# alanqrwang/keymorph

Hardware: AMD Instinct MI355X
Metric: volume-pairs/sec (fwd+bwd) at 256^3, 512 kp, TPS (higher is better)
Workload: dtype f32

## Files before the change

include/keymorph_hip.h:

```cpp
#ifndef KEYMORPH_HIP_H
#define KEYMORPH_HIP_H
#include <stddef.h>
#include <stdint.h>
#ifdef __cplusplus
extern "C" {
#endif

#define KMH_EINVAL (-22)
#define KMH_ABI_VERSION 1
int kmh_abi_version(void);

int kmh_grid_sample3d_fwd(const float* x, const float* grid, float* out, int N, int C, int D, int H,
                          int W, int Do, int Ho, int Wo, int mode, void* stream);
int kmh_grid_sample3d_bwd_grid(const float* x, const float* grid, const float* gout, float* dgrid,
                               int N, int C, int D, int H, int W, int Do, int Ho, int Wo, void* stream);
int kmh_grid_sample3d_bwd_input(const float* grid, const float* gout, float* dx, int N, int C, int D,
                                int H, int W, int Do, int Ho, int Wo, void* stream);

size_t kmh_reduce_ws_bytes(void);
int kmh_mse_fwd(const float* a, const float* b, long long n, float* out, void* ws, void* stream);
int kmh_mse_bwd(const float* a, const float* b, const float* gscale, long long n, float* da, void* stream);
int kmh_warp_mse_fwd(const float* x, const float* grid, const float* fixed, float* out, float* out_loss,
                     int N, int C, int D, int H, int W, int Do, int Ho, int Wo, void* ws, void* stream);
int kmh_warp_mse_fwd_grad(const float* x, const float* grid, const float* fixed, float* out, float* out_loss,
                          float* dgrid, int N, int C, int D, int H, int W, int Do, int Ho, int Wo, void* ws,
                          void* stream);
int kmh_scale_unless_one(float* a, long long n, const float* g, void* stream);

int kmh_dice_sums(const float* pred, const float* target, int R, long long V, float* sums, void* ws,
                  void* stream);
int kmh_rows_axpby(const float* t, const float* p, const float* ca, const float* cb, int R, long long V,
                   float* out, void* stream);
int kmh_warp_dice_ok(int N, int C, int D, int H, int W);
int kmh_warp_dice_sums(const float* x, const float* grid, const float* fixed, float* sums, int N, int C, int D, int H,
                       int W, int Do, int Ho, int Wo, const unsigned char* lab_x, const unsigned char* lab_fixed,
                       const int* gate, void* ws, void* stream);
int kmh_warp_dice_bwd_grid(const float* x, const float* grid, const float* fixed, const float* ca, const float* cb,
                           float* dgrid, int N, int C, int D, int H, int W, int Do, int Ho, int Wo,
                           const unsigned char* lab_x, const unsigned char* lab_fixed, const int* gate, void* stream);
int kmh_onehot_to_labels(const float* x, int N, int C, long long V, unsigned char* lab, int* ok, void* stream);
int kmh_argmax_onehot(const float* pred, int N, int C, long long V, float* out, void* stream);
int kmh_jacobian_det(const float* disp, long long cstride, long long vstride, int D, int H, int W, float* jd,
                     double* stats, void* ws, void* stream);

int kmh_label_presence(const long long* seg, long long n, int nflags, int* flags, void* stream);
int kmh_one_hot_select(const long long* seg, int N, long long V, const long long* labels, int C, void* out,
                       int out_i64, void* stream);

size_t kmh_hausdorff3d_ws_bytes(int D, int H, int W);
int kmh_hausdorff3d(const void* a, const void* b, int dtype_a, int dtype_b, long long sstride_a, long long sstride_b, int N,
                    int D, int H, int W, double sz, double sy, double sx, void* ws, double* out_sq, void* stream);
size_t kmh_edt3d_sq_ws_bytes(int D, int H, int W);
int kmh_edt3d_sq(const void* a, int dtype, int D, int H, int W, double sz, double sy, double sx, void* ws, double* out,
                 void* stream);
int kmh_label_counts(const void* x, const void* y, int dtype, int N, int C, long long V, unsigned long long* counts,
                     void* stream);

size_t kmh_lc2_ws_bytes(int num_patches, int num_radii);
int kmh_lc2_fwd(const float* us, const float* mr, int N, int S, int P, const int* radii, int R, double alpha, double beta,
                int reduce_mean, void* ws, float* out, void* stream);
int kmh_lc2_bwd(const float* us, const float* mr, const float* gout, int N, int S, int P, const int* radii, int R,
                int reduce_mean, const void* ws, float* dus, float* dmr, void* stream);

int kmh_affine_grid_fwd(const float* mat, float* out, int N, int D, int H, int W, void* stream);
int kmh_affine_grid_bwd(const float* dgrid, float* dmat, int N, int D, int H, int W, void* ws, void* stream);

int kmh_tps_grid_fwd(const float* theta, const float* ctrl, float* out, int N, int T, int D, int H, int W,
                     void* stream);
size_t kmh_tps_grid_bwd_ws_bytes(int N, int T, int D, int H, int W);
int kmh_tps_grid_bwd(const float* dgrid, const float* theta, const float* ctrl, float* dtheta,
                     float* dctrl, int N, int T, int D, int H, int W, void* ws, void* stream);
int kmh_tps_points_fwd(const float* theta, const float* ctrl, const float* pts, float* out, int N, int T,
                       int P, void* stream);
size_t kmh_tps_points_bwd_ws_bytes(int N, int T, int P);
int kmh_tps_points_bwd(const float* dout, const float* theta, const float* ctrl, const float* pts,
                       float* dtheta, float* dctrl, float* dpts, int N, int T, int P, void* ws,
                       void* stream);

size_t kmh_tps_fit_ws_bytes(int N, int T);
int kmh_tps_fit_fwd(const float* ctrl, const float* tgt, const float* lmbda, const float* w, float* theta,
                    int N, int T, void* ws, void* stream);
int kmh_tps_fit_force_retry(int count);
int kmh_tps_fit_bwd(const float* dtheta, const float* theta, const float* ctrl, const float* lmbda, const float* w,
                    float* dctrl, float* dtgt, float* dw, int N, int T, void* ws, void* stream);

int kmh_affine_fit_fwd(const float* x, const float* y, const float* w, float* M, int N, int K, void* stream);
int kmh_affine_fit_bwd(const float* dM, const float* x, const float* y, const float* w, const float* M,
                       float* dx, float* dy, float* dw, int N, int K, void* stream);
int kmh_rigid_fit_fwd(const float* x, const float* y, const float* w, float* M, int N, int K, void* stream);
int kmh_rigid_fit_bwd(const float* dM, const float* x, const float* y, const float* w, float* dx, float* dy,
                      float* dw, int N, int K, void* stream);
int kmh_affine_inverse_fwd(const float* M, float* Minv, int N, void* stream);
int kmh_affine_inverse_bwd(const float* dMinv, const float* Minv, float* dM, int N, void* stream);
int kmh_affine_points_fwd(const float* M, const float* pts, float* out, int N, int P, void* stream);
int kmh_affine_build_matrix(const float* scale, const float* offset, const float* theta, const float* shear,
                            float* out, int B, void* stream);
int kmh_affine_points_bwd(const float* dout, const float* M, const float* pts, float* dM, float* dpts,
                          int N, int P, void* stream);

int kmh_com3d_fwd(const float* feat, float* pts, float* sums, int N, int K, int D, int H, int W, void* ws,
                  void* stream);
int kmh_com3d_bwd(const float* dpts, const float* feat, const float* sums, float* dfeat, int N, int K,
                  int D, int H, int W, void* stream);



int kmh_conv3d_pack_weight(const float* w, float* packed, int Cout, int Cin, int transposed, void* stream);
int kmh_conv3d_fwd(const float* x, const float* scale, const float* shift, const float* mask,
                   const float* packed_w, const float* bias, float* y, int N, int D, int H, int W, int Cin,
                   int Cout, int relu_in, int relu_out, void* stream);
size_t kmh_conv3d_pack_bf_bytes(int Cout, int Cin, int transposed, int terms);
int kmh_conv3d_pack_weight_bf(const float* w, void* packed, int Cout, int Cin, int transposed, int terms,
                              const float* wscale, void* stream);
size_t kmh_conv3d_fwd_bf_stats_ws_bytes(int N, int D, int H, int W, int Cout, int rows_per_wave);
int kmh_conv3d_fwd_bf(const float* x, const float* scale, const float* shift, const float* mask, const void* packed,
                      const float* bias, float* y, int N, int D, int H, int W, int Cin, int Cout, int relu_in,
                      int relu_out, int terms, int rows_per_wave, const float* ascale, const float* wscale,
                      void* stats_ws, double* stats_out, int in_blocked, const float* addend, void* stream);
int kmh_conv3d_fwd_bf_set_dispatch(int mode);
int kmh_conv3d_fwd_bf_split_ok(int N, int D, int H, int W, int Cin, int Cout, int terms);
int kmh_conv3d_fwd_bf_variant(int N, int D, int H, int W, int Cin, int Cout, int terms, int has_mask, int has_addend);
int kmh_conv3d_fwd_bf_pool_ok(int N, int D, int H, int W, int Cin, int Cout, int terms);
int kmh_conv3d_fwd_bf_pool(const float* x, const float* scale, const float* shift, const void* packed, float* yp,
                           unsigned char* arg, int N, int D, int H, int W, int Cin, int Cout, int relu_in, int terms,
                           const float* ascale, const float* wscale, void* stats_ws, double* stats_out, int in_blocked,
                           void* stream);
size_t kmh_conv3d_up2_pack_bytes(int Cout, int Cl, int terms);
int kmh_conv3d_up2_pack_weight(const float* w, void* packed, int Cout, int Ctot, int cofs, int Cl, int terms,
                               const float* wscale, void* stream);
size_t kmh_conv3d_up2_dgrad_pack_bytes(int Cout, int Cl, int terms);
int kmh_conv3d_up2_dgrad_pack_weight(const float* w, void* packed, int Cout, int Ctot, int cofs, int Cl, int terms,
                                     const float* wscale, void* stream);
size_t kmh_conv3d_up2_dgrad_stats_ws_bytes(int N, int Dl, int Hl, int Wl, int Cl);
int kmh_conv3d_up2_dgrad(const float* dz, const void* packed, float* ds, int N, int Dl, int Hl, int Wl, int Cl, int Cout,
                         int terms, const float* dscale, const float* wscale, void* stats_ws, double* stats_out,
                         int in_blocked ,
                         void* stream);
int kmh_up2_boxsum(const float* dz, float* G, int N, int Dl, int Hl, int Wl, int Cout, int in_blocked ,
                   void* stream);
size_t kmh_up2_wgrad_gemm_ws_bytes(int N, int V, int Cl, int J);
int kmh_up2_wgrad_gemm(const float* A, const float* B, float* C, int N, int V, int Cl, int J, int terms,
                       const float* ascale, const float* bscale, const float* a_scale, const float* a_shift, void* ws,
                       void* stream);
int kmh_up2_wgrad_fold_ok(int Cl, int Cout, int terms);
size_t kmh_up2_wgrad_fold_ws_bytes(int N, int Dl, int Hl, int Wl, int Cl, int Cout);
int kmh_up2_wgrad_fold(const float* xl, const float* dz, float* C, int N, int Dl, int Hl, int Wl, int Cl, int Cout, int terms,
                       const float* ascale, const float* dscale, const float* a_scale, const float* a_shift, int dz_blocked,
                       void* ws, void* stream);
int kmh_conv3d_up2_fwd(const float* xl, const float* scale, const float* shift, int Ctot, int cofs, const void* packed,
                       float* y, int N, int Dl, int Hl, int Wl, int Cl, int Cout, int terms, const float* ascale,
                       const float* wscale, void* stream);
size_t kmh_conv3d_wgrad_bf_ws_bytes(int N, int D, int H, int W, int Cin, int Cout, int terms);
int kmh_conv3d_wgrad_bf_blocked_ok(int N, int D, int H, int W, int Cin, int Cout, int terms);
int kmh_conv3d_wgrad_bf(const float* x, const float* scale, const float* shift, const float* dz,
                        const float* dzmask, float* dw, int N, int D, int H, int W, int Cin, int Cout, int relu_in,
                        int accumulate, int terms, int append_ones, const float* xscale, const float* dscale, int dz_blocked, const float* w_fold, double* bhat,
                        void* ws, void* stream);
size_t kmh_conv3d_first_layer_fwd_ws_bytes(int N, int D, int H, int W, int Cout);
int kmh_conv3d_first_layer_fwd(const float* x, const float* scale, const float* shift, const float* w, float* y, int N,
                               int D, int H, int W, int Cout, void* ws, double* stats_out, void* stream);
size_t kmh_conv3d_first_layer_wgrad_ws_bytes(int N, int D, int H, int W, int Cout);
int kmh_conv3d_first_layer_wgrad(const float* x, const float* dz, const float* dzmask, const float* c123, double* rs, int N,
                                 int D, int H, int W, int Cout, void* ws, void* stream);
int kmh_conv3d_first_layer_fold(const void* rs, int rs_f64, const float* w, const float* scale_n, const float* shift_n, int Cout,
                                float* dw, double* ab_n, int accumulate, void* stream);
size_t kmh_conv3d_wgrad_ws_bytes(int N, int D, int H, int W, int Cin, int Cout);
int kmh_conv3d_wgrad(const float* x, const float* scale, const float* shift, const float* dz,
                     const float* dzmask, float* dw, int N, int D, int H, int W, int Cin, int Cout, int relu_in,
                     int accumulate, void* ws, void* stream);

size_t kmh_channel_stats_ws_bytes(int N, int C);
int kmh_channel_stats(const float* a, const float* b, int mode, int N, long long V, int C, double* out, void* ws,
                      const int* only_if, void* stream);
int kmh_gn_fwd_coeffs(const double* stats, const float* gamma, const float* beta, int N, int C, int G, double count,
                      float eps, float* scale, float* shift, float* mean_rstd, float* ascale, void* stream);
int kmh_absmax_scale(const float* x, long long n, float min_abs, float* out2, void* stream);
int kmh_gn_bwd_coeffs(const double* ab, const float* gamma, const float* mean_rstd, int N, int C, int G,
                      double count, float* c123, float* dgamma, float* dbeta, const int* only_if, void* stream);
int kmh_gn_bwd_coeffs_fold(const double* dstats, const double* bhat, const float* gamma, const float* beta,
                           const float* mean_rstd, int N, int C, int G, double count, float* c123, float* dgamma,
                           float* dbeta, int* fallback, void* stream);
int kmh_in_bwd_stats(const float* du, const float* z, const float* scale, const float* shift, int N, long long V, int C,
                     double* out, void* ws, void* stream);
int kmh_in_bwd_apply(const float* du, const float* z, const float* scale, const float* shift, const float* c123, int N,
                     long long V, int C, float* dz, float* dz_scale2, void* stream);
int kmh_in_bwd_apply_pool(const unsigned char* argmax, const float* du, const float* z, const float* scale,
                          const float* shift, const float* c123, int N, int D, int H, int W, int C, float* dz,
                          float* dz_scale2, void* stream);

int kmh_gn_bwd_apply(const float* dxn, const float* x, const float* c123, int N, long long V, int C,
                     int relu_mask, int accumulate, float* dx, float* dx_scale2, int out_blocked, void* stream);
int kmh_relu_mask(const float* dy, const float* y, long long n, float* dz, void* stream);
int kmh_norm_apply(const float* x, const float* scale, const float* shift, int N, long long V, int C, int relu,
                   float* y, void* stream);

int kmh_maxpool3d_fwd(const float* x, float* y, unsigned char* argmax, int N, int D, int H, int W, int C, void* stream);
int kmh_maxpool3d_bwd(const float* x, const unsigned char* argmax, const float* dy, const float* add, int add_cstride,
                      float* dx, int N, int D, int H, int W, int C, int out_blocked, void* stream);
size_t kmh_maxpool3d_bwd_split_bytes(int N, int D, int H, int W, int C);
int kmh_maxpool3d_bwd_split(const unsigned char* argmax, const float* dy, const float* dy_scale2, float* dxs, int N, int D,
                            int H, int W, int C, void* stream);
int kmh_maxpool3d_bwd_lazy(const unsigned char* argmax, const float* dy, const float* dxn, const float* x, const float* c123,
                           float* dx, int N, int D, int H, int W, int C, float* dx_scale2, void* stream);
int kmh_upcat_fwd(const float* skip, const float* low, float* out, int N, int D, int H, int W, int Cs, int Dl,
                  int Hl, int Wl, int Cl, void* stream);
int kmh_upcat_bwd(const float* dout, float* dskip, float* dlow, int N, int D, int H, int W, int Cs, int Dl, int Hl,
                  int Wl, int Cl, int accumulate_skip, void* stream);
int kmh_layout_convert(const float* in, float* out, int N, long long V, int C, int to_ncdhw, void* stream);

int kmh_pointwise_pack(const float* w, float* wt, int Cout, int Cin, void* stream);
int kmh_pointwise_fwd(const float* x, const float* wt, const float* bias, float* y, int N, long long V, int Cin,
                      int Cout, void* stream);
int kmh_pointwise_dgrad(const float* dy, const float* w, float* dx, int N, long long V, int Cin, int Cout,
                        void* stream);
size_t kmh_pointwise_wgrad_ws_bytes(int N, long long V, int Cin, int Cout);
int kmh_pointwise_wgrad(const float* dy, const float* x, float* dw, float* dbias, int N, long long V, int Cin,
                        int Cout, int accumulate, void* ws, void* stream);

size_t kmh_headcom_fwd_ws_bytes(int N, long long V, int Cout);
size_t kmh_headcom_bwd_ws_bytes(int N, long long V, int Cin, int Cout);
int kmh_headcom_fwd(const float* feat, const float* w, const float* bias, float* pts, float* sums, float* sq, int N, int D,
                    int H, int W, int Cin, int Cout, void* ws, void* stream);
int kmh_headcom_bwd(const float* dpts, const float* dpower, const float* feat, const float* w, const float* bias,
                    const float* sums, float* dfeat, float* dw, float* dbias, int N, int D, int H, int W, int Cin,
                    int Cout, int mask_dfeat, void* ws, void* stream);
size_t kmh_headcom_fwd_bf_ws_bytes(int N, long long V, int Cout, int terms);
size_t kmh_headcom_bwd_bf_ws_bytes(int N, long long V, int Cin, int Cout, int terms);
size_t kmh_headcom_mask_words(int N, int D, int H, int W, int Cout);
int kmh_headcom_fwd_bf(const float* feat, const float* w, const float* bias, float* pts, float* sums, float* sq,
                       float* scales_out, int N, int D, int H, int W, int Cin, int Cout, int terms, unsigned* mask, void* ws,
                       void* stream);
int kmh_headcom_bwd_bf(const float* dpts, const float* dpower, const float* feat, const float* w, const float* bias,
                       const float* sums, float* dfeat, float* dw, float* dbias, int N, int D, int H, int W, int Cin,
                       int Cout, int terms, int mask_dfeat, const float* scales_in, float* dfeat_scale2,
                       const unsigned* mask, void* ws, void* stream);

int kmh_adam_step(float* p, const float* g, float* m, float* v, long long n, float lr, float beta1, float beta2,
                  float eps, int step, float grad_scale, void* stream);

int kmh_resize_trilinear3d_fwd(const float* x, float* y, int N, int C, int D, int H, int W, int Do, int Ho, int Wo,
                               const int* tz, const int* ty, const int* tx, int channels_last, void* stream);
int kmh_resize_trilinear3d_bwd(const float* gy, float* gx, int N, int C, int D, int H, int W, int Do, int Ho, int Wo,
                               const int* tz, const int* ty, const int* tx, const int* rz, const int* ry, const int* rx,
                               int channels_last, void* stream);
size_t kmh_components3d_ws_bytes(int N, int D, int H, int W);
int kmh_components3d(const unsigned char* mask, int* labels, int N, int D, int H, int W, int* info, void* ws, void* stream);
int kmh_clean_mask3d(const unsigned char* mask, unsigned char* out, int N, int D, int H, int W, double threshold, int* info,
                     void* ws, void* stream);

int kmh_conv3d_thin_ok(int Cin, int Cout);
int kmh_conv3d_thin_wgrad_ok(int Cin, int Cout);
int kmh_conv3d_thin_fwd(const float* x, const float* w, const float* bias, float* y, int N, int D, int H, int W, int Cin,
                        int Cout, int relu_out, void* stream);
int kmh_conv3d_thin_dgrad(const float* dz, const float* dzmask, const float* w, float* dx, int N, int D, int H, int W, int Cin,
                          int Cout, void* stream);
size_t kmh_conv3d_thin_wgrad_ws_bytes(int N, int D, int H, int W, int Cin, int Cout);
int kmh_conv3d_thin_wgrad(const float* x, const float* dz, const float* dzmask, float* dw, float* db, int N, int D, int H,
                          int W, int Cin, int Cout, void* ws, void* stream);

#ifdef __cplusplus
}
#endif
#endif
```

keymorph_amd/_lib.py:

```python
from __future__ import annotations

import ctypes as C
import os

from .build import LIBPATH

_f = C.c_void_p
_i = C.c_int
_ll = C.c_longlong
_sz = C.c_size_t

PROTOS = {
    "kmh_abi_version": (_i, []),
    "kmh_grid_sample3d_fwd": (_i, [_f, _f, _f, _i, _i, _i, _i, _i, _i, _i, _i, _i, _f]),
    "kmh_grid_sample3d_bwd_grid": (_i, [_f, _f, _f, _f, _i, _i, _i, _i, _i, _i, _i, _i, _f]),
    "kmh_grid_sample3d_bwd_input": (_i, [_f, _f, _f, _i, _i, _i, _i, _i, _i, _i, _i, _f]),
    "kmh_reduce_ws_bytes": (_sz, []),
    "kmh_mse_fwd": (_i, [_f, _f, _ll, _f, _f, _f]),
    "kmh_mse_bwd": (_i, [_f, _f, _f, _ll, _f, _f]),
    "kmh_warp_mse_fwd": (_i, [_f, _f, _f, _f, _f, _i, _i, _i, _i, _i, _i, _i, _i, _f, _f]),
    "kmh_warp_mse_fwd_grad": (_i, [_f, _f, _f, _f, _f, _f, _i, _i, _i, _i, _i, _i, _i, _i, _f, _f]),
    "kmh_scale_unless_one": (_i, [_f, _ll, _f, _f]),
    "kmh_dice_sums": (_i, [_f, _f, _i, _ll, _f, _f, _f]),
    "kmh_rows_axpby": (_i, [_f, _f, _f, _f, _i, _ll, _f, _f]),
    "kmh_warp_dice_ok": (_i, [_i, _i, _i, _i, _i]),
    "kmh_warp_dice_sums": (_i, [_f, _f, _f, _f, _i, _i, _i, _i, _i, _i, _i, _i, _f, _f, _f, _f, _f]),
    "kmh_warp_dice_bwd_grid": (_i, [_f, _f, _f, _f, _f, _f, _i, _i, _i, _i, _i, _i, _i, _i, _f, _f, _f, _f]),
    "kmh_onehot_to_labels": (_i, [_f, _i, _i, _ll, _f, _f, _f]),
    "kmh_argmax_onehot": (_i, [_f, _i, _i, _ll, _f, _f]),
    "kmh_affine_grid_fwd": (_i, [_f, _f, _i, _i, _i, _i, _f]),
    "kmh_affine_grid_bwd": (_i, [_f, _f, _i, _i, _i, _i, _f, _f]),
    "kmh_tps_grid_fwd": (_i, [_f, _f, _f, _i, _i, _i, _i, _i, _f]),
    "kmh_tps_grid_bwd_ws_bytes": (_sz, [_i, _i, _i, _i, _i]),
    "kmh_tps_grid_bwd": (_i, [_f, _f, _f, _f, _f, _i, _i, _i, _i, _i, _f, _f]),
    "kmh_tps_points_fwd": (_i, [_f, _f, _f, _f, _i, _i, _i, _f]),
    "kmh_tps_points_bwd_ws_bytes": (_sz, [_i, _i, _i]),
    "kmh_tps_points_bwd": (_i, [_f, _f, _f, _f, _f, _f, _f, _i, _i, _i, _f, _f]),
    "kmh_tps_fit_ws_bytes": (_sz, [_i, _i]),
    "kmh_tps_fit_fwd": (_i, [_f, _f, _f, _f, _f, _i, _i, _f, _f]),
    "kmh_tps_fit_force_retry": (_i, [_i]),
    "kmh_tps_fit_bwd": (_i, [_f, _f, _f, _f, _f, _f, _f, _f, _i, _i, _f, _f]),
    "kmh_affine_fit_fwd": (_i, [_f, _f, _f, _f, _i, _i, _f]),
    "kmh_affine_fit_bwd": (_i, [_f, _f, _f, _f, _f, _f, _f, _f, _i, _i, _f]),
    "kmh_rigid_fit_fwd": (_i, [_f, _f, _f, _f, _i, _i, _f]),
    "kmh_rigid_fit_bwd": (_i, [_f, _f, _f, _f, _f, _f, _f, _i, _i, _f]),
    "kmh_affine_inverse_fwd": (_i, [_f, _f, _i, _f]),
    "kmh_affine_inverse_bwd": (_i, [_f, _f, _f, _i, _f]),
    "kmh_affine_points_fwd": (_i, [_f, _f, _f, _i, _i, _f]),
    "kmh_jacobian_det": (_i, [_f, _ll, _ll, _i, _i, _i, _f, _f, _f, _f]),
    "kmh_label_presence": (_i, [_f, _ll, _i, _f, _f]),
    "kmh_one_hot_select": (_i, [_f, _i, _ll, _f, _i, _f, _i, _f]),
    "kmh_hausdorff3d_ws_bytes": (_sz, [_i, _i, _i]),
    "kmh_hausdorff3d": (_i, [_f, _f, _i, _i, _ll, _ll, _i, _i, _i, _i, C.c_double, C.c_double, C.c_double, _f, _f, _f]),
    "kmh_edt3d_sq_ws_bytes": (_sz, [_i, _i, _i]),
    "kmh_edt3d_sq": (_i, [_f, _i, _i, _i, _i, C.c_double, C.c_double, C.c_double, _f, _f, _f]),
    "kmh_label_counts": (_i, [_f, _f, _i, _i, _i, _ll, _f, _f]),
    "kmh_lc2_ws_bytes": (_sz, [_i, _i]),
    "kmh_lc2_fwd": (_i, [_f, _f, _i, _i, _i, _f, _i, C.c_double, C.c_double, _i, _f, _f, _f]),
    "kmh_lc2_bwd": (_i, [_f, _f, _f, _i, _i, _i, _f, _i, _i, _f, _f, _f, _f]),
    "kmh_affine_build_matrix": (_i, [_f, _f, _f, _f, _f, _i, _f]),
    "kmh_affine_points_bwd": (_i, [_f, _f, _f, _f, _f, _i, _i, _f]),
    "kmh_com3d_fwd": (_i, [_f, _f, _f, _i, _i, _i, _i, _i, _f, _f]),
    "kmh_com3d_bwd": (_i, [_f, _f, _f, _f, _i, _i, _i, _i, _i, _f]),
    "kmh_conv3d_pack_weight": (_i, [_f, _f, _i, _i, _i, _f]),
    "kmh_conv3d_fwd": (_i, [_f, _f, _f, _f, _f, _f, _f, _i, _i, _i, _i, _i, _i, _i, _i, _f]),
    "kmh_conv3d_pack_bf_bytes": (_sz, [_i, _i, _i, _i]),
    "kmh_conv3d_pack_weight_bf": (_i, [_f, _f, _i, _i, _i, _i, _f, _f]),
    "kmh_conv3d_fwd_bf": (_i, [_f, _f, _f, _f, _f, _f, _f, _i, _i, _i, _i, _i, _i, _i, _i, _i, _i, _f, _f, _f, _f, _i, _f, _f]),
    "kmh_conv3d_fwd_bf_set_dispatch": (_i, [_i]),
    "kmh_conv3d_fwd_bf_variant": (_i, [_i, _i, _i, _i, _i, _i, _i, _i, _i]),
    "kmh_conv3d_fwd_bf_pool_ok": (_i, [_i, _i, _i, _i, _i, _i, _i]),
    "kmh_conv3d_fwd_bf_split_ok": (_i, [_i, _i, _i, _i, _i, _i, _i]),
    "kmh_conv3d_fwd_bf_pool": (_i, [_f, _f, _f, _f, _f, _f, _i, _i, _i, _i, _i, _i, _i, _i, _f, _f, _f, _f, _i, _f]),
    "kmh_conv3d_up2_dgrad_pack_bytes": (_sz, [_i, _i, _i]),
    "kmh_conv3d_up2_dgrad_pack_weight": (_i, [_f, _f, _i, _i, _i, _i, _i, _f, _f]),
    "kmh_conv3d_up2_dgrad_stats_ws_bytes": (_sz, [_i, _i, _i, _i, _i]),
    "kmh_conv3d_up2_dgrad": (_i, [_f, _f, _f, _i, _i, _i, _i, _i, _i, _i, _f, _f, _f, _f, _i, _f]),
    "kmh_up2_boxsum": (_i, [_f, _f, _i, _i, _i, _i, _i, _i, _f]),
    "kmh_up2_wgrad_gemm_ws_bytes": (_sz, [_i, _i, _i, _i]),
    "kmh_up2_wgrad_gemm": (_i, [_f, _f, _f, _i, _i, _i, _i, _i, _f, _f, _f, _f, _f, _f]),
    "kmh_up2_wgrad_fold_ok": (_i, [_i, _i, _i]),
    "kmh_up2_wgrad_fold_ws_bytes": (_sz, [_i, _i, _i, _i, _i, _i]),
    "kmh_up2_wgrad_fold": (_i, [_f, _f, _f, _i, _i, _i, _i, _i, _i, _i, _f, _f, _f, _f, _i, _f, _f]),
    "kmh_conv3d_up2_pack_bytes": (_sz, [_i, _i, _i]),
    "kmh_conv3d_up2_pack_weight": (_i, [_f, _f, _i, _i, _i, _i, _i, _f, _f]),
    "kmh_conv3d_up2_fwd": (_i, [_f, _f, _f, _i, _i, _f, _f, _i, _i, _i, _i, _i, _i, _i, _f, _f, _f]),
    "kmh_conv3d_fwd_bf_stats_ws_bytes": (_sz, [_i, _i, _i, _i, _i, _i]),
    "kmh_conv3d_first_layer_fwd_ws_bytes": (_sz, [_i, _i, _i, _i, _i]),
    "kmh_conv3d_first_layer_fwd": (_i, [_f, _f, _f, _f, _f, _i, _i, _i, _i, _i, _f, _f, _f]),
    "kmh_conv3d_wgrad_bf_ws_bytes": (_sz, [_i, _i, _i, _i, _i, _i, _i]),
    "kmh_conv3d_wgrad_bf": (_i, [_f, _f, _f, _f, _f, _f, _i, _i, _i, _i, _i, _i, _i, _i, _i, _i, _f, _f, _i, _f, _f, _f, _f]),
    "kmh_conv3d_wgrad_bf_blocked_ok": (_i, [_i, _i, _i, _i, _i, _i, _i]),
    "kmh_conv3d_first_layer_wgrad_ws_bytes": (_sz, [_i, _i, _i, _i, _i]),
    "kmh_conv3d_first_layer_wgrad": (_i, [_f, _f, _f, _f, _f, _i, _i, _i, _i, _i, _f, _f]),
    "kmh_conv3d_first_layer_fold": (_i, [_f, _i, _f, _f, _f, _i, _f, _f, _i, _f]),
    "kmh_conv3d_wgrad_ws_bytes": (_sz, [_i, _i, _i, _i, _i, _i]),
    "kmh_conv3d_wgrad": (_i, [_f, _f, _f, _f, _f, _f, _i, _i, _i, _i, _i, _i, _i, _i, _f, _f]),
    "kmh_channel_stats_ws_bytes": (_sz, [_i, _i]),
    "kmh_channel_stats": (_i, [_f, _f, _i, _i, _ll, _i, _f, _f, _f, _f]),
    "kmh_gn_fwd_coeffs": (_i, [_f, _f, _f, _i, _i, _i, C.c_double, C.c_float, _f, _f, _f, _f, _f]),
    "kmh_absmax_scale": (_i, [_f, _ll, C.c_float, _f, _f]),
    "kmh_gn_bwd_coeffs": (_i, [_f, _f, _f, _i, _i, _i, C.c_double, _f, _f, _f, _f, _f]),
    "kmh_gn_bwd_coeffs_fold": (_i, [_f, _f, _f, _f, _f, _i, _i, _i, C.c_double, _f, _f, _f, _f, _f]),
    "kmh_gn_bwd_apply": (_i, [_f, _f, _f, _i, _ll, _i, _i, _i, _f, _f, _i, _f]),
    "kmh_in_bwd_stats": (_i, [_f, _f, _f, _f, _i, _ll, _i, _f, _f, _f]),
    "kmh_in_bwd_apply": (_i, [_f, _f, _f, _f, _f, _i, _ll, _i, _f, _f, _f]),
    "kmh_in_bwd_apply_pool": (_i, [_f, _f, _f, _f, _f, _f, _i, _i, _i, _i, _i, _f, _f, _f]),
    "kmh_relu_mask": (_i, [_f, _f, _ll, _f, _f]),
    "kmh_norm_apply": (_i, [_f, _f, _f, _i, _ll, _i, _i, _f, _f]),
    "kmh_maxpool3d_fwd": (_i, [_f, _f, _f, _i, _i, _i, _i, _i, _f]),
    "kmh_maxpool3d_bwd": (_i, [_f, _f, _f, _f, _i, _f, _i, _i, _i, _i, _i, _i, _f]),
    "kmh_maxpool3d_bwd_split_bytes": (_sz, [_i, _i, _i, _i, _i]),
    "kmh_maxpool3d_bwd_split": (_i, [_f, _f, _f, _f, _i, _i, _i, _i, _i, _f]),
    "kmh_maxpool3d_bwd_lazy": (_i, [_f, _f, _f, _f, _f, _f, _i, _i, _i, _i, _i, _f, _f]),
    "kmh_upcat_fwd": (_i, [_f, _f, _f, _i, _i, _i, _i, _i, _i, _i, _i, _i, _f]),
    "kmh_upcat_bwd": (_i, [_f, _f, _f, _i, _i, _i, _i, _i, _i, _i, _i, _i, _i, _f]),
    "kmh_layout_convert": (_i, [_f, _f, _i, _ll, _i, _i, _f]),
    "kmh_pointwise_pack": (_i, [_f, _f, _i, _i, _f]),
    "kmh_pointwise_fwd": (_i, [_f, _f, _f, _f, _i, _ll, _i, _i, _f]),
    "kmh_pointwise_dgrad": (_i, [_f, _f, _f, _i, _ll, _i, _i, _f]),
    "kmh_pointwise_wgrad_ws_bytes": (_sz, [_i, _ll, _i, _i]),
    "kmh_pointwise_wgrad": (_i, [_f, _f, _f, _f, _i, _ll, _i, _i, _i, _f, _f]),
    "kmh_headcom_fwd_ws_bytes": (_sz, [_i, _ll, _i]),
    "kmh_headcom_bwd_ws_bytes": (_sz, [_i, _ll, _i, _i]),
    "kmh_headcom_fwd_bf_ws_bytes": (_sz, [_i, _ll, _i, _i]),
    "kmh_headcom_bwd_bf_ws_bytes": (_sz, [_i, _ll, _i, _i, _i]),
    "kmh_headcom_mask_words": (_sz, [_i, _i, _i, _i, _i]),
    "kmh_headcom_fwd_bf": (_i, [_f, _f, _f, _f, _f, _f, _f, _i, _i, _i, _i, _i, _i, _i, _f, _f, _f]),
    "kmh_headcom_bwd_bf": (_i, [_f, _f, _f, _f, _f, _f, _f, _f, _f, _i, _i, _i, _i, _i, _i, _i, _i, _f, _f, _f, _f, _f]),
    "kmh_headcom_fwd": (_i, [_f, _f, _f, _f, _f, _f, _i, _i, _i, _i, _i, _i, _f, _f]),
    "kmh_headcom_bwd": (_i, [_f, _f, _f, _f, _f, _f, _f, _f, _f, _i, _i, _i, _i, _i, _i, _i, _f, _f]),
    "kmh_adam_step": (_i, [_f, _f, _f, _f, _ll, C.c_float, C.c_float, C.c_float, C.c_float, _i, C.c_float, _f]),
    "kmh_resize_trilinear3d_fwd": (_i, [_f, _f, _i, _i, _i, _i, _i, _i, _i, _i, _f, _f, _f, _i, _f]),
    "kmh_resize_trilinear3d_bwd": (_i, [_f, _f, _i, _i, _i, _i, _i, _i, _i, _i, _f, _f, _f, _f, _f, _f, _i, _f]),
    "kmh_components3d_ws_bytes": (_sz, [_i, _i, _i, _i]),
    "kmh_components3d": (_i, [_f, _f, _i, _i, _i, _i, _f, _f, _f]),
    "kmh_clean_mask3d": (_i, [_f, _f, _i, _i, _i, _i, C.c_double, _f, _f, _f]),
    "kmh_conv3d_thin_ok": (_i, [_i, _i]),
    "kmh_conv3d_thin_wgrad_ok": (_i, [_i, _i]),
    "kmh_conv3d_thin_fwd": (_i, [_f, _f, _f, _f, _i, _i, _i, _i, _i, _i, _i, _f]),
    "kmh_conv3d_thin_dgrad": (_i, [_f, _f, _f, _f, _i, _i, _i, _i, _i, _i, _f]),
    "kmh_conv3d_thin_wgrad_ws_bytes": (_sz, [_i, _i, _i, _i, _i, _i]),
    "kmh_conv3d_thin_wgrad": (_i, [_f, _f, _f, _f, _f, _i, _i, _i, _i, _i, _i, _f, _f]),
}

_lib = None


class KeymorphHipError(RuntimeError):
    pass


class _Profiler:

    def __init__(self):
        self.enabled = False
        self.records = []
        self.meta = None

    def reset(self):
        self.records = []

    def summary(self):
        import torch
        torch.cuda.synchronize()
        out = {}
        for name, a, b, meta in self.records:
            d = out.setdefault(name, {"calls": 0, "ms": 0.0, "flops": 0.0, "bytes": 0.0})
            d["calls"] += 1
            d["ms"] += a.elapsed_time(b)
            if meta:
                d["flops"] += meta.get("flops", 0.0)
                d["bytes"] += meta.get("bytes", 0.0)
        return out


profiler = _Profiler()


class _Proxy:
    def __init__(self, lib):
        self._lib = lib

    def __getattr__(self, name):
        fn = getattr(self._lib, name)
        if not name.startswith("kmh_") or name.endswith("_bytes") or name == "kmh_abi_version":
            return fn

        def call(*args):
            if not profiler.enabled:
                return fn(*args)
            import torch
            a, b = torch.cuda.Event(enable_timing=True), torch.cuda.Event(enable_timing=True)
            a.record()
            rc = fn(*args)
            b.record()
            profiler.records.append((name, a, b, profiler.meta))
            profiler.meta = None
            return rc

        object.__setattr__(self, name, call)
        return call


_DEFAULT_LIBPATH = LIBPATH


def load():
    global _lib, LIBPATH
    if _lib is not None:
        return _lib
    if os.environ.get("KEYMORPH_HIP_LIB"):
        LIBPATH = os.environ["KEYMORPH_HIP_LIB"]
    if not os.path.exists(LIBPATH):
        raise KeymorphHipError(
            f"{LIBPATH} is missing: the HIP extension has not been built "
            "(run `python -m keymorph_amd.build`); there is no CPU/PyTorch fallback.")
    import torch
    rt = os.path.join(os.path.dirname(torch.__file__), "lib", "libamdhip64.so")
    if os.path.exists(rt):
        C.CDLL(rt, mode=C.RTLD_GLOBAL)
    else:
        C.CDLL("libamdhip64.so", mode=C.RTLD_GLOBAL)
    lib = C.CDLL(LIBPATH)
    ab_build = os.path.abspath(LIBPATH) != os.path.abspath(_DEFAULT_LIBPATH)
    for name, (res, args) in PROTOS.items():
        try:
            fn = getattr(lib, name)
        except AttributeError:
            if not ab_build:
                raise
            continue
        fn.restype = res
        fn.argtypes = args
    if lib.kmh_abi_version() != 1:
        raise KeymorphHipError("libkeymorph_hip.so ABI version mismatch")
    _lib = _Proxy(lib)
    return _lib


def check(rc: int, what: str):
    if rc != 0:
        raise KeymorphHipError(f"{what} failed with status {rc}")
```

keymorph_amd/backbone_ops.py:

```python
from __future__ import annotations

import os
from typing import Optional, Tuple

import torch

from . import _lib
from ._handoff import attach, expect, peek
from ._lib import check
from .ops import _p, _prep, _stream, workspace

Tensor = torch.Tensor
EPS = 1e-5

CONV_MODE = os.environ.get("KEYMORPH_HIP_CONV", "f16x3")
_TERMS = {"f16x3": 2, "bf16x6": 3}
_HEAD_TERMS = {"f16x3": 2, "bf16x6": 3}
BF_ROWS_PER_WAVE = int(os.environ.get("KEYMORPH_HIP_BF_ROWS", "4"))


def set_conv_mode(mode: str):
    global CONV_MODE
    assert mode in ("f32", "f16x3", "bf16x6"), mode
    CONV_MODE = mode


_SWITCHES = {
    "KEYMORPH_NO_EPILOGUE_STATS": "a separate statistics pass per layer instead of the convolution epilogue's",
    "KEYMORPH_NO_UPCONV": "materialise upsample+concat instead of the fused decoder operator, forward",
    "KEYMORPH_NO_UPCONV_BWD": "materialise upsample+concat instead of the fused decoder operator, backward",
    "KEYMORPH_NO_UPCONV_WGRAD": "the fused decoder operator rebuilds the upsampled half for the 27-tap weight gradient",
    "KEYMORPH_NO_UP2_FOLD": "the upsampled channels' weight gradient by the box-sum tensor + matrix product route",
    "KEYMORPH_NO_STATS_FOLD": "GroupNorm's backward statistics by a pass over the tensors",
    "KEYMORPH_NO_BLOCKED_GRADS": "every gradient in (N,D,H,W,C)",
    "KEYMORPH_NO_BLOCKED_UPCAT": "only the fused decoder operator's gradient in (N,D,H,W,C)",
    "KEYMORPH_NO_SPLIT_POOLGRAD": "the 256^3-level pooled gradient scattered as fp32 instead of pre-split records",
    "KEYMORPH_NO_CONV_POOL": "separate pooling pass instead of the conv epilogue's",
    "KEYMORPH_NO_LAZY_FIRST": "GroupNorm backward of the first block as its own pass",
    "KEYMORPH_NO_LAZY_SKIP": "GroupNorm's backward of a decoder skip applied in the decoder",
    "KEYMORPH_NO_LAZY_IN": "ConvNet block by block: separate norm / ReLU / pooling passes",
    "KEYMORPH_RANGE_AUDIT": "debug (ON = audit): per-sample dynamic range of every gradient operand, RANGE_AUDIT_LOG",
}


def _off(name: str) -> bool:
    if name not in _SWITCHES:
        raise KeyError(name)
    return bool(os.environ.get(name))


import contextlib
import functools
import threading

_AMP_DEFAULT = os.environ.get("KEYMORPH_AMP", "0") not in ("", "0")
_amp_tls = threading.local()


def amp_enabled() -> bool:
    return bool(getattr(_amp_tls, "on", _AMP_DEFAULT))


@contextlib.contextmanager
def amp_scope(on: bool):
    prev = amp_enabled()
    _amp_tls.on = bool(on)
    try:
        yield
    finally:
        _amp_tls.on = prev


def set_amp(on: bool) -> bool:
    prev = amp_enabled()
    _amp_tls.on = bool(on)
    return prev


def _t(terms: int) -> int:
    return 1 if (terms == 2 and amp_enabled()) else terms


def _binds_amp(cls):
    fwd, bwd = cls.forward, cls.backward

    @staticmethod
    @functools.wraps(fwd)
    def forward(ctx, *a, **k):
        ctx._kmh_amp = amp_enabled()
        return fwd(ctx, *a, **k)

    @staticmethod
    @functools.wraps(bwd)
    def backward(ctx, *g):
        with amp_scope(ctx._kmh_amp):
            return bwd(ctx, *g)

    cls.forward, cls.backward = forward, backward
    return cls


FIRST_BLOCK_DGRAD = os.environ.get("KEYMORPH_FIRST_BLOCK_DGRAD", "")


def set_first_block_dgrad(mode: str) -> str:
    global FIRST_BLOCK_DGRAD
    assert mode in ("", "bf16x6"), mode
    prev, FIRST_BLOCK_DGRAD = FIRST_BLOCK_DGRAD, mode
    return prev


def first_block_dgrad_terms() -> int:
    return 3 if (FIRST_BLOCK_DGRAD == "bf16x6" and CONV_MODE == "f16x3") else 0


def _f32(shape, dev):
    return torch.empty(shape, dtype=torch.float32, device=dev)


def channel_stats(a: Tensor, b: Optional[Tensor], N: int, V: int, C: int, only_if: Optional[Tensor] = None) -> Tensor:
    lib = _lib.load()
    out = torch.empty((N, C, 2), dtype=torch.float64, device=a.device)
    ws = workspace(int(lib.kmh_channel_stats_ws_bytes(N, C)), a.device, "stats")
    check(lib.kmh_channel_stats(_p(a), _p(b), 0 if b is None else 1, N, V, C, _p(out), _p(ws), _p(only_if), _stream()),
          "kmh_channel_stats")
    return out


def _needs_range_scales() -> bool:
    return _TERMS.get(CONV_MODE, 0) == 2


_CONSTS = {}


def _const(device, *values) -> Tensor:
    key = (str(device), values)
    t = _CONSTS.get(key)
    if t is None:
        t = _CONSTS[key] = torch.tensor(values, dtype=torch.float32, device=device)
    return t


def absmax_scale(x: Tensor, min_abs: float = 0.0) -> Tensor:
    lib = _lib.load()
    out = _f32((2,), x.device)
    check(lib.kmh_absmax_scale(_p(x), x.numel(), float(min_abs), _p(out), _stream()), "kmh_absmax_scale")
    return out


def conv_emits_stats() -> bool:
    return CONV_MODE != "f32" and not _off("KEYMORPH_NO_EPILOGUE_STATS")


def _tag_stats(t: Tensor, stats: Optional[Tensor]) -> None:
    if stats is not None:
        attach(t, "stats", stats)


def _peek_stats(t: Tensor) -> Optional[Tensor]:
    return peek(t, "stats")


STATS_STATS = {"carried": 0, "measured": 0}


def input_stats(x: Tensor, N: int, V: int, C: int) -> Tensor:
    s = _peek_stats(x)
    if s is not None and tuple(s.shape) == (N, C, 2):
        STATS_STATS["carried"] += 1
        return s
    STATS_STATS["measured"] += 1
    return channel_stats(x, None, N, V, C)


def _tag_grad_scale(t: Optional[Tensor], scale2: Optional[Tensor], loosen: float = 1.0) -> None:
    if t is None or scale2 is None:
        return
    if loosen != 1.0:
        scale2 = torch.stack([scale2[0] * (1.0 / loosen), scale2[1] * loosen])
    attach(t, "grad_scale", scale2)


def _sum_bound(a: Optional[Tensor], b: Optional[Tensor]) -> Optional[Tensor]:
    if a is None or b is None:
        return None
    return torch.stack([torch.minimum(a[0], b[0]) * 0.5, torch.maximum(a[1], b[1]) * 2.0])


GRAD_SCALE_STATS = {"carried": 0, "measured": 0}
RANGE_AUDIT_LOG = []


def range_audit(t: Tensor) -> dict:
    with torch.no_grad():
        a = t.detach().abs().reshape(t.shape[0], -1).float()
        m_n = a.amax(dim=1).double()
        M = float(m_n.max())
        if M == 0.0:
            return {"max": 0.0, "per_sample_log2_below_max": [0.0] * t.shape[0], "worst_relative_precision": 2.0 ** -22,
                    "flushed_fraction": 0.0}
        S = 2.0 ** (14 - int(torch.floor(torch.log2(torch.tensor(M))).item()))
        nz = a > 0
        flushed = float(((a * S < 2.0 ** -25) & nz).sum()) / max(1.0, float(nz.sum()))
        below = [float(torch.log2(torch.tensor(M) / m)) if float(m) > 0 else float("inf") for m in m_n]
        prec = max(max(2.0 ** -22, 2.0 ** (b - 39)) for b in below if b != float("inf"))
        return {"max": M, "per_sample_log2_below_max": below, "worst_relative_precision": prec,
                "flushed_fraction": flushed}


def grad_scale(dy: Tensor) -> Tensor:
    if _off("KEYMORPH_RANGE_AUDIT") and not _blocked_kind(dy):
        RANGE_AUDIT_LOG.append(dict(range_audit(dy), shape=tuple(dy.shape)))
    s = peek(dy, "grad_scale")
    if s is not None:
        GRAD_SCALE_STATS["carried"] += 1
        return s
    GRAD_SCALE_STATS["measured"] += 1
    return absmax_scale(dy)


def norm_coeffs(stats: Tensor, gamma: Optional[Tensor], beta: Optional[Tensor], N: int, C: int, G: int, V: int,
                want_ascale: bool = False):
    lib = _lib.load()
    dev = stats.device
    scale, shift, mr = _f32((N, C), dev), _f32((N, C), dev), _f32((N, G, 2), dev)
    ascale = _f32((2,), dev) if (want_ascale and _needs_range_scales()) else None
    check(lib.kmh_gn_fwd_coeffs(_p(stats), _p(gamma), _p(beta), N, C, G, float(V), EPS, _p(scale), _p(shift),
                                _p(mr), _p(ascale), _stream()), "kmh_gn_fwd_coeffs")
    return (scale, shift, mr, ascale) if want_ascale else (scale, shift, mr)


def pack_weight(w: Tensor, transposed: bool, wscale: Optional[Tensor] = None, terms: int = 0) -> Tensor:
    lib = _lib.load()
    Cout, Cin = w.shape[:2]
    if CONV_MODE != "f32":
        terms = terms or _TERMS[CONV_MODE]
        out = torch.empty(int(lib.kmh_conv3d_pack_bf_bytes(Cout, Cin, int(transposed), terms)), dtype=torch.uint8,
                          device=w.device)
        wscale = (wscale if wscale is not None else absmax_scale(w)) if terms == 2 else None
        attach(out, "packed", (terms, wscale))
        check(lib.kmh_conv3d_pack_weight_bf(_p(w), _p(out), Cout, Cin, int(transposed), terms, _p(wscale), _stream()),
              "kmh_conv3d_pack_weight_bf")
        return out
    out = _f32((27, Cout, Cin) if transposed else (27, Cin, Cout), w.device)
    check(lib.kmh_conv3d_pack_weight(_p(w), _p(out), Cout, Cin, int(transposed), _stream()), "kmh_conv3d_pack_weight")
    return out


def _packed(pk: Tensor):
    return peek(pk, "packed") or (0, None)


def _conv_meta(N, D, H, W, Cin, Cout, taps=27) -> None:
    if _lib.profiler.enabled:
        _lib.profiler.meta = {"flops": 2.0 * taps * Cin * Cout * N * D * H * W, "shape": (N, D, H, W, Cin, Cout)}


def conv3_raw(x, scale, shift, packed, bias, N, D, H, W, Cin, Cout, relu_in, relu_out, mask=None,
              ascale=None, stats_out: Optional[Tensor] = None, in_blocked: bool = False,
              addend: Optional[Tensor] = None) -> Tensor:
    lib = _lib.load()
    y = _f32((N, D, H, W, Cout), x.device)
    _conv_meta(N, D, H, W, Cin, Cout)
    terms, wscale = _packed(packed)
    if terms:
        if terms == 2 and ascale is None:
            assert scale is None, "a normalised input needs the range scale of the NORMALISED tensor (norm_coeffs)"
            ascale = absmax_scale(x)
        sws = None
        if stats_out is not None:
            sws = workspace(int(lib.kmh_conv3d_fwd_bf_stats_ws_bytes(N, D, H, W, Cout, BF_ROWS_PER_WAVE)), x.device,
                            "convstats")
        check(lib.kmh_conv3d_fwd_bf(_p(x), _p(scale), _p(shift), _p(mask), _p(packed), _p(bias), _p(y), N, D, H, W,
                                    Cin, Cout, int(relu_in), int(relu_out), _t(terms), BF_ROWS_PER_WAVE,
                                    _p(ascale if terms == 2 else None), _p(wscale), _p(sws), _p(stats_out),
                                    int(in_blocked), _p(addend), _stream()), "kmh_conv3d_fwd_bf")
        return y
    assert stats_out is None and addend is None, "only the split-operand kernels emit output statistics / take an addend"
    assert not in_blocked, "the channel-blocked input layout belongs to the split-operand kernels"
    check(lib.kmh_conv3d_fwd(_p(x), _p(scale), _p(shift), _p(mask), _p(packed), _p(bias), _p(y), N, D, H, W, Cin,
                             Cout, int(relu_in), int(relu_out), _stream()), "kmh_conv3d_fwd")
    return y


def conv3_wgrad(x, scale, shift, dz, N, D, H, W, Cin, Cout, relu_in, dzmask=None, xscale=None, dscale=None,
                dz_blocked: bool = False, fold: Optional[Tuple[Tensor, Tensor]] = None) -> Tensor:
    lib = _lib.load()
    dw = _f32((Cout, Cin, 3, 3, 3), x.device)
    _conv_meta(N, D, H, W, Cin, Cout)
    if CONV_MODE != "f32":
        terms = _TERMS[CONV_MODE]
        ws = workspace(int(lib.kmh_conv3d_wgrad_bf_ws_bytes(N, D, H, W, Cin, Cout, terms)), x.device, "wgrad")
        if terms == 2:
            if xscale is None:
                assert scale is None, "a normalised input needs the range scale of the NORMALISED tensor"
                xscale = absmax_scale(x)
            if dscale is None:
                dscale = absmax_scale(dz)
        else:
            xscale = dscale = None
        check(lib.kmh_conv3d_wgrad_bf(_p(x), _p(scale), _p(shift), _p(dz), _p(dzmask), _p(dw), N, D, H, W, Cin, Cout,
                                      int(relu_in), 0, _t(terms), 0, _p(xscale), _p(dscale), int(dz_blocked),
                                      _p(fold[0] if fold else None), _p(fold[1] if fold else None), _p(ws),
                                      _stream()), "kmh_conv3d_wgrad_bf")
        return dw
    assert fold is None, "the per-sample fold belongs to the split-operand kernels"
    assert not dz_blocked, "the channel-blocked gradient layout belongs to the split-operand kernels"
    ws = workspace(int(lib.kmh_conv3d_wgrad_ws_bytes(N, D, H, W, Cin, Cout)), x.device, "wgrad")
    check(lib.kmh_conv3d_wgrad(_p(x), _p(scale), _p(shift), _p(dz), _p(dzmask), _p(dw), N, D, H, W, Cin, Cout,
                               int(relu_in), 0, _p(ws), _stream()), "kmh_conv3d_wgrad")
    return dw


def first_layer_grads(x, scale, shift, mr, gamma, weight, dy, ymask, N, D, H, W, Cout, G, dscale=None, lazy_c123=None):
    lib = _lib.load()
    V = D * H * W
    dw = _f32((Cout, 1, 3, 3, 3), x.device)
    ab = torch.empty((N, 1, 2), dtype=torch.float64, device=x.device)
    if Cout <= 16:
        rs = torch.empty((N, Cout, 2, 27), dtype=torch.float64, device=x.device)
        ws = workspace(int(lib.kmh_conv3d_first_layer_wgrad_ws_bytes(N, D, H, W, Cout)), x.device, "wgrad")
        if _lib.profiler.enabled:
            _lib.profiler.meta = {"flops": 2.0 * 27 * 2 * Cout * V * N, "shape": (N, D, H, W, 1, Cout)}
        check(lib.kmh_conv3d_first_layer_wgrad(_p(x), _p(dy), _p(ymask), _p(lazy_c123), _p(rs), N, D, H, W, Cout, _p(ws),
                                               _stream()), "kmh_conv3d_first_layer_wgrad")
        for n in range(N):
            check(lib.kmh_conv3d_first_layer_fold(_p(rs[n]), 1, _p(weight), _p(scale[n]), _p(shift[n]), Cout, _p(dw),
                                                  _p(ab[n]), int(n > 0), _stream()), "kmh_conv3d_first_layer_fold")
    else:
        assert lazy_c123 is None
        terms = _TERMS[CONV_MODE]
        rs = _f32((Cout, 2, 3, 3, 3), x.device)
        ws = workspace(int(lib.kmh_conv3d_wgrad_bf_ws_bytes(1, D, H, W, 2, Cout, terms)), x.device, "wgrad")
        xscale = absmax_scale(x, 1.0) if terms == 2 else None
        dscale = (dscale if dscale is not None else absmax_scale(dy)) if terms == 2 else None
        for n in range(N):
            if _lib.profiler.enabled:
                _lib.profiler.meta = {"flops": 2.0 * 27 * 1 * Cout * V, "shape": (1, D, H, W, 1, Cout)}
            check(lib.kmh_conv3d_wgrad_bf(_p(x[n]), None, None, _p(dy[n]), _p(None if ymask is None else ymask[n]),
                                          _p(rs), 1, D, H, W, 2, Cout, 0, 0, _t(terms), 1, _p(xscale), _p(dscale), 0, None, None,
                                          _p(ws), _stream()), "kmh_conv3d_wgrad_bf")
            check(lib.kmh_conv3d_first_layer_fold(_p(rs), 0, _p(weight), _p(scale[n]), _p(shift[n]), Cout, _p(dw),
                                                  _p(ab[n]), int(n > 0), _stream()), "kmh_conv3d_first_layer_fold")
    _, dgamma, dbeta = _gn_bwd_coeffs(ab, gamma, mr, N, 1, G, V)
    return dw, dgamma, dbeta


def conv3_up2_dgrad(dz: Tensor, weight: Tensor, Cs: int, Cl: int, dscale: Optional[Tensor] = None,
                    stats_out: Optional[Tensor] = None, dz_blocked: bool = False) -> Tensor:
    lib = _lib.load()
    N, D, H, W, Cout = dz.shape
    terms = _TERMS[CONV_MODE]
    wsu = None
    if terms == 2:
        wsu = absmax_scale(weight[:, Cs:].contiguous()) * _const(dz.device, 0.125, 8.0)
        if dscale is None:
            dscale = absmax_scale(dz)
    pk = torch.empty(int(lib.kmh_conv3d_up2_dgrad_pack_bytes(Cout, Cl, terms)), dtype=torch.uint8, device=dz.device)
    check(lib.kmh_conv3d_up2_dgrad_pack_weight(_p(weight), _p(pk), Cout, Cs + Cl, Cs, Cl, terms, _p(wsu), _stream()),
          "kmh_conv3d_up2_dgrad_pack_weight")
    ds = _f32((N, D // 2, H // 2, W // 2, Cl), dz.device)
    _conv_meta(N, D, H, W, Cout, Cl, taps=8)
    sws = None
    if stats_out is not None:
        sws = workspace(int(lib.kmh_conv3d_up2_dgrad_stats_ws_bytes(N, D // 2, H // 2, W // 2, Cl)), dz.device, "convstats")
    check(lib.kmh_conv3d_up2_dgrad(_p(dz), _p(pk), _p(ds), N, D // 2, H // 2, W // 2, Cl, Cout, _t(terms),
                                   _p(dscale if terms == 2 else None), _p(wsu), _p(sws), _p(stats_out), int(dz_blocked),
                                   _stream()), "kmh_conv3d_up2_dgrad")
    return ds


UPCONV_STATS = {"calls": 0}


def _up_sources(x):
    tag = peek(x, "up_sources")
    return tag[:2] if (tag is not None and tag[0]._version == tag[2] and tag[1]._version == tag[3]) else None


def grad_blocked_ok(N, D, H, W, Cin, Cout) -> bool:
    if CONV_MODE != "f16x3" or _off("KEYMORPH_NO_BLOCKED_GRADS"):
        return False
    return bool(_lib.load().kmh_conv3d_wgrad_bf_blocked_ok(N, D, H, W, Cin, Cout, 2))


BLOCKED_STATS = {"handoffs": 0}
SPLIT_STATS = {"handoffs": 0}


UP2_STATS = {"fold": 0, "boxsum": 0}


def up2_wgrad_fold_ok(Cl, Cout, terms):
    if _off("KEYMORPH_NO_UP2_FOLD"):
        return False
    return bool(_lib.load().kmh_up2_wgrad_fold_ok(int(Cl), int(Cout), int(terms)))


def pool_grad_split_ok(N, D, H, W, Cin, Cout) -> bool:
    if CONV_MODE != "f16x3" or _off("KEYMORPH_NO_SPLIT_POOLGRAD") or Cout % 8:
        return False
    lib = _lib.load()
    return bool(lib.kmh_conv3d_fwd_bf_split_ok(N, D, H, W, Cout, Cin, 2)) and \
        bool(lib.kmh_conv3d_wgrad_bf_blocked_ok(N, D, H, W, Cin, Cout, 2))


def _blocked_kind(t) -> int:
    return peek(t, "layout") or 0


def _gn_bwd_coeffs(ab, gamma, mr, N, C, G, V, fold=None):
    lib = _lib.load()
    c123 = _f32((N, C, 3), mr.device)
    dgamma = dbeta = flag = None
    if gamma is not None:
        dgamma, dbeta = torch.zeros_like(gamma), torch.zeros_like(gamma)
    if fold is not None:
        dstats, bhat, beta = fold
        flag = torch.empty(1, dtype=torch.int32, device=mr.device)
        check(lib.kmh_gn_bwd_coeffs_fold(_p(dstats), _p(bhat), _p(gamma), _p(beta), _p(mr), N, C, G, float(V), _p(c123),
                                         _p(dgamma), _p(dbeta), _p(flag), _stream()), "kmh_gn_bwd_coeffs_fold")
        STATS_STATS["folded"] = STATS_STATS.get("folded", 0) + 1
    if callable(ab):
        ab = ab(flag)
    check(lib.kmh_gn_bwd_coeffs(_p(ab), _p(gamma), _p(mr), N, C, G, float(V), _p(c123), _p(dgamma), _p(dbeta), _p(flag),
                                _stream()), "kmh_gn_bwd_coeffs")
    return c123, dgamma, dbeta


def _gn_bwd_apply(dxn, x, c123, N, V, C, sc2, from_relu=True, out=None, blocked=False):
    out = dxn if out is None else out
    check(_lib.load().kmh_gn_bwd_apply(_p(dxn), _p(x), _p(c123), N, V, C, int(from_relu), 0, _p(out), _p(sc2), int(blocked),
                                       _stream()), "kmh_gn_bwd_apply")
    _tag_grad_scale(out, sc2)
    if blocked:
        attach(out, "layout", 1)
        BLOCKED_STATS["handoffs"] += 1
    return out


@_binds_amp
class _SingleConvGCR(torch.autograd.Function):

    @staticmethod
    def forward(ctx, x, gamma, beta, weight, num_groups, x_from_relu, dy_premasked, dy_blocked=False, dx_blocked=False,
                pool=False, dy_lazy=False, dx_lazy=False, dgrad_terms=0):
        ctx.dgrad_terms = int(dgrad_terms) if (CONV_MODE == "f16x3" and int(dgrad_terms) == 3) else 0
        upsrc = _up_sources(x)
        x, gamma, beta, weight = _prep(x), _prep(gamma), _prep(beta), _prep(weight)
        N, D, H, W, Cin = x.shape
        Cout = weight.shape[0]
        V = D * H * W
        if upsrc is not None and not (CONV_MODE in _TERMS and _TERMS[CONV_MODE] in (2, 3) and Cout > 16
                                       and upsrc[1].shape[-1] % 8 == 0 and upsrc[0].shape[-1] % 8 == 0
                                       and not _off("KEYMORPH_NO_UPCONV")):
            upsrc = None
        stats = input_stats(x, N, V, Cin)
        scale, shift, mr, ascale = norm_coeffs(stats, gamma, beta, N, Cin, num_groups, V, want_ascale=True)
        ystats = (torch.empty((N, Cout, 2), dtype=torch.float64, device=x.device) if conv_emits_stats() else None)
        lib = _lib.load()
        if Cin == 1 and Cout <= 16:
            y = _f32((N, D, H, W, Cout), x.device)
            ws = workspace(int(lib.kmh_conv3d_first_layer_fwd_ws_bytes(N, D, H, W, Cout)), x.device, "convstats")
            _conv_meta(N, D, H, W, Cin, Cout)
            check(lib.kmh_conv3d_first_layer_fwd(_p(x), _p(scale), _p(shift), _p(weight), _p(y), N, D, H, W, Cout, _p(ws),
                                                 _p(ystats), _stream()), "kmh_conv3d_first_layer_fwd")
        elif upsrc is not None:
            skip, low = upsrc
            y = _up2_forward(skip, low, scale, shift, ascale, weight, N, D, H, W, skip.shape[-1], low.shape[-1], Cout,
                             ystats)
        elif pool:
            assert dy_premasked and ystats is not None and conv_pool_ok(N, D, H, W, Cin, Cout)
            pk = pack_weight(weight, False)
            ctx.wscale = _packed(pk)[1]
            y = _f32((N, D // 2, H // 2, W // 2, Cout), x.device)
            arg = torch.empty((N, D // 2, H // 2, W // 2, Cout), dtype=torch.uint8, device=x.device)
            sws = workspace(int(lib.kmh_conv3d_fwd_bf_stats_ws_bytes(N, D, H, W, Cout, BF_ROWS_PER_WAVE)), x.device,
                            "convstats")
            _conv_meta(N, D, H, W, Cin, Cout)
            check(lib.kmh_conv3d_fwd_bf_pool(_p(x), _p(scale), _p(shift), _p(pk), _p(y), _p(arg), N, D, H, W, Cin, Cout, 0,
                                             _t(2), _p(ascale), _p(ctx.wscale), _p(sws), _p(ystats), 0, _stream()),
                  "kmh_conv3d_fwd_bf_pool")
            ctx.pool_arg = arg
            POOL_STATS["fused"] += 1
        else:
            pk = pack_weight(weight, False)
            ctx.wscale = _packed(pk)[1]
            y = conv3_raw(x, scale, shift, pk, None, N, D, H, W, Cin, Cout, False, True, ascale=ascale,
                          stats_out=ystats)
        ctx.pool = bool(pool)
        ctx.save_for_backward(x, y, scale, shift, mr, gamma, weight, beta)
        ctx.ascale = ascale
        ctx.cfg = (num_groups, bool(x_from_relu), bool(dy_premasked))
        ctx.blocked = (bool(dy_blocked), bool(dx_blocked))
        ctx.lazy = (bool(dy_lazy), bool(dx_lazy))
        assert not dy_blocked or dy_premasked, "a channel-blocked gradient comes from a SingleConv, i.e. already masked"
        if ystats is None:
            return y, None
        ctx.mark_non_differentiable(ystats)
        return y, ystats

    @staticmethod
    def backward(ctx, dy, _dstats=None):
        lib = _lib.load()
        x, y, scale, shift, mr, gamma, weight, beta = ctx.saved_tensors
        G, x_from_relu, dy_premasked = ctx.cfg
        N, D, H, W, Cin = x.shape
        Cout = weight.shape[0]
        V = D * H * W
        dy_blocked, dx_blocked = ctx.blocked
        expect(dy, "layout", dy_blocked and not ctx.pool, "gradient between two SingleConvs", "KEYMORPH_NO_BLOCKED_GRADS")
        sd_in = peek(dy, "grad_scale")
        dy_lazy, dx_lazy = ctx.lazy
        expect(dy, "lazy_gn", dy_lazy, "the first encoder block's pending GroupNorm backward", "KEYMORPH_NO_LAZY_FIRST")
        lazy_tag = peek(dy, "lazy_gn")
        dy = _prep(dy)
        dy_split = False
        if ctx.pool:
            odd = (D | H | W) & 1
            dy_split = (dy_blocked and not odd and _needs_range_scales() and pool_grad_split_ok(N, D, H, W, Cin, Cout)
                        and not (Cin == 1 and not ctx.needs_input_grad[0])
                        and not ctx.dgrad_terms)
            if dy_split:
                sd_in = sd_in if sd_in is not None else absmax_scale(dy)
                full = torch.empty((N, Cout // 8, D * H * W + 1, 8), dtype=torch.float32, device=dy.device)
                check(lib.kmh_maxpool3d_bwd_split(_p(ctx.pool_arg), _p(dy), _p(sd_in), _p(full), N, D, H, W, Cout, _stream()),
                      "kmh_maxpool3d_bwd_split")
                SPLIT_STATS["handoffs"] += 1
            else:
                full = torch.empty((N, D, H, W, Cout), dtype=torch.float32, device=dy.device)
                if odd:
                    full.zero_()
                check(lib.kmh_maxpool3d_bwd(None, _p(ctx.pool_arg), _p(dy), None, 0, _p(full), N, D, H, W, Cout,
                                            int(dy_blocked), _stream()), "kmh_maxpool3d_bwd")
            _tag_grad_scale(full, sd_in)
            dy = full
            if dy_blocked:
                attach(dy, "layout", 2 if dy_split else 1)
                BLOCKED_STATS["handoffs"] += 1
        kind = 2 if dy_split else int(dy_blocked)
        if _blocked_kind(dy) != kind:
            raise RuntimeError("keymorph_amd: gradient layout kind %d where %d was expected (1 = fp32 channel-blocked, 2 = pre-split"
                               " records); a hook or an in-place op between two operators changed the tensor" % (_blocked_kind(dy), kind))
        ymask = None if dy_premasked else y
        first = Cin == 1 and not ctx.needs_input_grad[0] and (Cout <= 16 or CONV_MODE != "f32")
        dscale = (grad_scale(dy) if (_needs_range_scales() and not (first and Cout <= 16)) else None)
        if first:
            lazy_c123, ymask = lazy_tag if dy_lazy else (None, ymask)
            dw, dgamma, dbeta = first_layer_grads(x, scale, shift, mr, gamma, weight, dy, ymask, N, D, H, W, Cout, G,
                                                  dscale=dscale, lazy_c123=lazy_c123)
            return (None, dgamma, dbeta, dw) + (None,) * 9
        assert not dy_lazy, "only the first layer's correlation kernel applies a pending GroupNorm backward"
        need_affine = ctx.needs_input_grad[1] or ctx.needs_input_grad[2]
        need_dxn = ctx.needs_input_grad[0] or need_affine
        fold = need_dxn and ctx.needs_input_grad[3] and conv_emits_stats() and not _off("KEYMORPH_NO_STATS_FOLD")
        bhat = torch.zeros((N, Cin), dtype=torch.float64, device=x.device) if fold else None
        dw = (conv3_wgrad(x, scale, shift, dy, N, D, H, W, Cin, Cout, False, dzmask=ymask, xscale=ctx.ascale,
                          dscale=dscale, dz_blocked=kind, fold=(weight, bhat) if fold else None)
              if ctx.needs_input_grad[3] else None)
        dx = dgamma = dbeta = None
        if need_dxn:
            dstats = torch.empty((N, Cin, 2), dtype=torch.float64, device=x.device) if fold else None
            if ctx.dgrad_terms:
                FIRST_BLOCK_STATS["exact_dgrads"] += 1
            dxn = conv3_raw(dy, None, None,
                            pack_weight(weight, True, None if ctx.dgrad_terms else getattr(ctx, "wscale", None), terms=ctx.dgrad_terms),
                            None, N, D, H, W, Cout, Cin, False, False,
                            mask=ymask, ascale=dscale, in_blocked=kind, stats_out=dstats)
            sc2 = torch.zeros(2, dtype=torch.float32, device=x.device) if (_needs_range_scales() and ctx.needs_input_grad[0]) else None
            c123, dgamma, dbeta = _gn_bwd_coeffs(lambda flag: channel_stats(dxn, x, N, V, Cin, only_if=flag), gamma, mr,
                                                 N, Cin, G, V, fold=(dstats, bhat, beta) if fold else None)
            if ctx.needs_input_grad[0] and dx_lazy:
                assert x_from_relu and not dx_blocked
                dx = dxn
                attach(dx, "lazy_gn", (c123, x))
                LAZY_STATS["handoffs"] += 1
            elif ctx.needs_input_grad[0]:
                dx = _gn_bwd_apply(dxn, x, c123, N, V, Cin, sc2, from_relu=x_from_relu,
                                   out=torch.empty_like(dxn) if dx_blocked else None, blocked=dx_blocked)
        return (dx, dgamma, dbeta, dw) + (None,) * 9


def _up2_forward(skip, low, scale, shift, ascale, weight, N, D, H, W, Cs, Cl, Cout, ystats):
    lib = _lib.load()
    terms = _TERMS[CONV_MODE]
    dev = skip.device
    pk_s = pack_weight(weight[:, :Cs].contiguous(), False)
    wsu = None
    if terms == 2:
        wsu = absmax_scale(weight[:, Cs:].contiguous()) * _const(dev, 0.125, 8.0)
    pku = torch.empty(int(lib.kmh_conv3d_up2_pack_bytes(Cout, Cl, terms)), dtype=torch.uint8, device=dev)
    check(lib.kmh_conv3d_up2_pack_weight(_p(weight), _p(pku), Cout, Cs + Cl, Cs, Cl, terms, _p(wsu), _stream()),
          "kmh_conv3d_up2_pack_weight")
    part = _f32((N, D, H, W, Cout), dev)
    _conv_meta(N, D, H, W, Cl, Cout, taps=8)
    check(lib.kmh_conv3d_up2_fwd(_p(low), _p(scale), _p(shift), Cs + Cl, Cs, _p(pku), _p(part), N, D // 2, H // 2,
                                 W // 2, Cl, Cout, _t(terms), _p(ascale if terms == 2 else None), _p(wsu), _stream()),
          "kmh_conv3d_up2_fwd")
    y = conv3_raw(skip, scale[:, :Cs].contiguous(), shift[:, :Cs].contiguous(), pk_s, None, N, D, H, W, Cs, Cout,
                  False, True, ascale=ascale, stats_out=ystats, addend=part)
    UPCONV_STATS["calls"] += 1
    return y


def upcat_conv_ok(skip, low, Cout) -> bool:
    return (CONV_MODE in _TERMS and conv_emits_stats() and Cout > 16 and Cout % 4 == 0 and skip.shape[-1] % 8 == 0
            and low.shape[-1] % 8 == 0 and all(a == 2 * b for a, b in zip(skip.shape[1:4], low.shape[1:4]))
            and not _off("KEYMORPH_NO_UPCONV") and not _off("KEYMORPH_NO_UPCONV_BWD"))


@_binds_amp
class _UpCatConvGCR(torch.autograd.Function):

    @staticmethod
    def forward(ctx, skip, low, gamma, beta, weight, num_groups, dy_premasked, dskip_lazy=False, dy_blocked=False):
        ctx.dskip_lazy = bool(dskip_lazy)
        ctx.dy_blocked = bool(dy_blocked)
        assert not dy_blocked or dy_premasked, "a channel-blocked gradient comes from a SingleConv, i.e. already masked"
        skip, low, gamma, beta, weight = _prep(skip), _prep(low), _prep(gamma), _prep(beta), _prep(weight)
        N, D, H, W, Cs = skip.shape
        Cl, Cout = low.shape[-1], weight.shape[0]
        V = D * H * W
        stats = torch.cat([input_stats(skip, N, V, Cs), input_stats(low, N, V // 8, Cl) * 8.0], dim=1)
        scale, shift, mr, ascale = norm_coeffs(stats, gamma, beta, N, Cs + Cl, num_groups, V, want_ascale=True)
        ystats = torch.empty((N, Cout, 2), dtype=torch.float64, device=skip.device)
        y = _up2_forward(skip, low, scale, shift, ascale, weight, N, D, H, W, Cs, Cl, Cout, ystats)
        ctx.save_for_backward(skip, low, y, scale, shift, mr, gamma, weight, beta)
        ctx.ascale = ascale
        ctx.cfg = (num_groups, bool(dy_premasked))
        ctx.mark_non_differentiable(ystats)
        return y, ystats

    @staticmethod
    def backward(ctx, dy, _dstats=None):
        lib = _lib.load()
        skip, low, y, scale, shift, mr, gamma, weight, beta = ctx.saved_tensors
        G, dy_premasked = ctx.cfg
        N, D, H, W, Cs = skip.shape
        Cl, Cout = low.shape[-1], weight.shape[0]
        C, V = Cs + Cl, D * H * W
        blk = ctx.dy_blocked
        expect(dy, "layout", blk, "gradient of the fused upsample+concat convolution's output", "KEYMORPH_NO_BLOCKED_GRADS")
        dy = _prep(dy)
        if not dy_premasked:
            dzm = torch.empty_like(dy)
            check(lib.kmh_relu_mask(_p(dy), _p(y), dy.numel(), _p(dzm), _stream()), "kmh_relu_mask")
            dy = dzm
        dscale = grad_scale(dy) if _needs_range_scales() else None
        bhat_s = torch.zeros((N, Cs), dtype=torch.float64, device=dy.device)
        dw_s = conv3_wgrad(skip, scale[:, :Cs].contiguous(), shift[:, :Cs].contiguous(), dy, N, D, H, W, Cs, Cout, False,
                           xscale=ctx.ascale, dscale=dscale, dz_blocked=blk, fold=(weight[:, :Cs].contiguous(), bhat_s))
        if Cout % 4 == 0 and not _off("KEYMORPH_NO_UPCONV_WGRAD"):
            Vl = V // 8
            sc_l, sh_l = scale[:, Cs:].contiguous(), shift[:, Cs:].contiguous()
            terms = _TERMS[CONV_MODE]
            dwn = _f32((N, Cl, 27, Cout), dy.device)
            if _lib.profiler.enabled:
                _lib.profiler.meta = {"flops": 2.0 * 27 * Cl * Cout * N * Vl, "shape": (N, Vl, Cl, 27 * Cout)}
            if up2_wgrad_fold_ok(Cl, Cout, terms):
                UP2_STATS["fold"] += 1
                gws = workspace(int(lib.kmh_up2_wgrad_fold_ws_bytes(N, D // 2, H // 2, W // 2, Cl, Cout)), dy.device, "wgrad")
                check(lib.kmh_up2_wgrad_fold(_p(low), _p(dy), _p(dwn), N, D // 2, H // 2, W // 2, Cl, Cout, _t(terms), _p(ctx.ascale),
                                             _p(dscale), _p(sc_l), _p(sh_l), int(blk), _p(gws), _stream()), "kmh_up2_wgrad_fold")
            else:
                UP2_STATS["boxsum"] += 1
                boxes = _f32((N, Vl, 27 * Cout), dy.device)
                check(lib.kmh_up2_boxsum(_p(dy), _p(boxes), N, D // 2, H // 2, W // 2, Cout, int(blk), _stream()), "kmh_up2_boxsum")
                gws = workspace(int(lib.kmh_up2_wgrad_gemm_ws_bytes(N, Vl, Cl, 27 * Cout)), dy.device, "wgrad")
                bsc = (dscale * _const(dy.device, 0.125, 8.0)) if terms == 2 else None
                check(lib.kmh_up2_wgrad_gemm(_p(low), _p(boxes), _p(dwn), N, Vl, Cl, 27 * Cout, _t(terms),
                                             _p(ctx.ascale if terms == 2 else None), _p(bsc), _p(sc_l), _p(sh_l), _p(gws),
                                             _stream()), "kmh_up2_wgrad_gemm")
                del boxes
            dw_l = dwn.sum(0).permute(2, 0, 1).reshape(Cout, Cl, 3, 3, 3)
            wl = weight[:, Cs:].reshape(Cout, Cl, 27).permute(1, 2, 0)
            bhat_l = (dwn.double() * wl.double().unsqueeze(0)).sum(dim=(2, 3))
        else:
            xu = _f32((N, D, H, W, Cl), dy.device)
            check(lib.kmh_upcat_fwd(_p(skip), _p(low), _p(xu), N, D, H, W, 0, D // 2, H // 2, W // 2, Cl, _stream()),
                  "kmh_upcat_fwd")
            bhat_l = torch.zeros((N, Cl), dtype=torch.float64, device=dy.device)
            dw_l = conv3_wgrad(xu, scale[:, Cs:].contiguous(), shift[:, Cs:].contiguous(), dy, N, D, H, W, Cl, Cout,
                               False, xscale=ctx.ascale, dscale=dscale, dz_blocked=blk,
                               fold=(weight[:, Cs:].contiguous(), bhat_l))
            del xu
        dw = torch.cat([dw_s, dw_l], dim=1)
        bhat = torch.cat([bhat_s, bhat_l], dim=1)
        dst_s = torch.empty((N, Cs, 2), dtype=torch.float64, device=dy.device)
        dxn_s = conv3_raw(dy, None, None, pack_weight(weight[:, :Cs].contiguous(), True), None, N, D, H, W, Cout, Cs,
                          False, False, ascale=dscale, stats_out=dst_s, in_blocked=blk)
        dst_l = torch.empty((N, Cl, 2), dtype=torch.float64, device=dy.device)
        dsum_l = conv3_up2_dgrad(dy, weight, Cs, Cl, dscale, stats_out=dst_l, dz_blocked=blk)
        dstats = torch.cat([dst_s, dst_l], dim=1)
        ab = lambda flag: torch.cat([channel_stats(dxn_s, skip, N, V, Cs, only_if=flag),
                                     channel_stats(dsum_l, low, N, V // 8, Cl, only_if=flag)], dim=1)
        c123, dgamma, dbeta = _gn_bwd_coeffs(ab, gamma, mr, N, C, G, V, fold=(dstats, bhat, beta))
        c_s = c123[:, :Cs].contiguous()
        c_l = (c123[:, Cs:] * _const(dy.device, 1.0, 8.0, 8.0)).contiguous()
        sc_s = torch.zeros(2, dtype=torch.float32, device=dy.device) if _needs_range_scales() else None
        sc_l = torch.zeros(2, dtype=torch.float32, device=dy.device) if _needs_range_scales() else None
        dskip = dlow = None
        if ctx.needs_input_grad[0] and ctx.dskip_lazy:
            dskip = dxn_s
            attach(dskip, "lazy_gn", (c_s, skip))
            LAZY_STATS["handoffs"] += 1
        elif ctx.needs_input_grad[0]:
            dskip = _gn_bwd_apply(dxn_s, skip, c_s, N, V, Cs, sc_s)
        if ctx.needs_input_grad[1]:
            dlow = _gn_bwd_apply(dsum_l, low, c_l, N, V // 8, Cl, sc_l)
        return (dskip, dlow, dgamma, dbeta, dw) + (None,) * 4


def upcat_blocked_ok(skip, low, Cout) -> bool:
    N, D, H, W, Cs = skip.shape
    return (torch.is_grad_enabled() and Cout % 8 == 0 and not _off("KEYMORPH_NO_UPCONV_WGRAD")
            and not _off("KEYMORPH_NO_BLOCKED_UPCAT") and grad_blocked_ok(N, D, H, W, Cs, Cout))


def upcat_conv_gcr(skip, low, gamma, beta, weight, num_groups: int, dy_premasked: bool = False,
                   dskip_lazy: bool = False, dy_blocked: bool = False) -> Tensor:
    if dskip_lazy:
        node = skip.grad_fn
        if node is not None and type(node).__name__ == "_PoolForkBackward":
            node._kmh_expect_lazy = True
        else:
            dskip_lazy = False
    y, ystats = _UpCatConvGCR.apply(skip, low, gamma, beta, weight, num_groups, dy_premasked, dskip_lazy, dy_blocked)
    _tag_stats(y, ystats)
    return y


def single_conv_gcr(x, gamma, beta, weight, num_groups: int, x_from_relu: bool = True,
                    dy_premasked: bool = False, dy_blocked: bool = False, dx_blocked: bool = False,
                    pool: bool = False, dy_lazy: bool = False, dx_lazy: bool = False, dgrad_terms: int = 0) -> Tensor:
    y, ystats = _SingleConvGCR.apply(x, gamma, beta, weight, num_groups, x_from_relu, dy_premasked, dy_blocked,
                                     dx_blocked, pool, dy_lazy, dx_lazy, dgrad_terms)
    _tag_stats(y, ystats)
    return y


POOL_STATS = {"fused": 0}
FIRST_BLOCK_STATS = {"exact_dgrads": 0}
LAZY_STATS = {"handoffs": 0}


def lazy_skip_ok(skip) -> bool:
    return (torch.is_grad_enabled() and skip.shape[1] % 2 == 0 and skip.shape[2] % 2 == 0 and skip.shape[3] % 2 == 0
            and skip.shape[4] % 4 == 0 and not _off("KEYMORPH_NO_LAZY_SKIP"))


def lazy_first_layer_ok(x, cout1: int) -> bool:
    return (x.shape[-1] == 1 and cout1 <= 16 and not x.requires_grad and torch.is_grad_enabled()
            and not _off("KEYMORPH_NO_LAZY_FIRST"))


def conv_pool_ok(N, D, H, W, Cin, Cout) -> bool:
    if CONV_MODE != "f16x3" or not conv_emits_stats() or _off("KEYMORPH_NO_CONV_POOL"):
        return False
    return bool(_lib.load().kmh_conv3d_fwd_bf_pool_ok(N, D, H, W, Cin, Cout, 2))


_NO_ADD = object()


def _maxpool_fwd(ctx, x):
    lib = _lib.load()
    x = _prep(x)
    N, D, H, W, C = x.shape
    y = _f32((N, D // 2, H // 2, W // 2, C), x.device)
    arg = torch.empty(y.shape, dtype=torch.uint8, device=x.device) if ctx.needs_input_grad[0] else None
    check(lib.kmh_maxpool3d_fwd(_p(x), _p(y), _p(arg), N, D, H, W, C, _stream()), "kmh_maxpool3d_fwd")
    ctx.xshape = tuple(x.shape)
    if arg is not None:
        ctx.save_for_backward(arg)
    return x, y


def _maxpool_bwd(ctx, dy, add, out_blocked=False):
    lib = _lib.load()
    (arg,) = ctx.saved_tensors
    N, D, H, W, C = ctx.xshape
    odd = (D % 2) or (H % 2) or (W % 2)
    acs = 0
    add_tag = _NO_ADD if add is None else peek(add, "grad_scale")
    if add is not None:
        acs = add.stride(3)
        dense_voxels = add.stride() == (D * H * W * acs, H * W * acs, W * acs, acs, 1)
        if odd or add.dtype != torch.float32 or not dense_voxels:
            add, acs = add.contiguous().float().clone(), C
    if add is not None and acs == C and odd:
        dx = add
    else:
        dx = (torch.zeros if odd else torch.empty)((N, D, H, W, C), dtype=torch.float32, device=arg.device)
    dy_c = _prep(dy)
    check(lib.kmh_maxpool3d_bwd(None, _p(arg), _p(dy_c), _p(add), acs, _p(dx), N, D, H, W, C, int(out_blocked),
                                _stream()), "kmh_maxpool3d_bwd")
    if out_blocked:
        attach(dx, "layout", 1)
        BLOCKED_STATS["handoffs"] += 1
    sd = peek(dy, "grad_scale")
    _tag_grad_scale(dx, sd if add_tag is _NO_ADD else _sum_bound(sd, add_tag))
    return dx


class _MaxPool2(torch.autograd.Function):
    @staticmethod
    def forward(ctx, x, blocked_grad):
        ctx.blocked_grad = bool(blocked_grad)
        return _maxpool_fwd(ctx, x)[1]

    @staticmethod
    def backward(ctx, dy):
        return _maxpool_bwd(ctx, dy, None, ctx.blocked_grad), None


def maxpool2(x: Tensor, blocked_grad: bool = False) -> Tensor:
    return _MaxPool2.apply(x, blocked_grad)


class _PoolFork(torch.autograd.Function):

    @staticmethod
    def forward(ctx, x):
        x, y = _maxpool_fwd(ctx, x)
        ctx.set_materialize_grads(False)
        return y, x.view_as(x)

    @staticmethod
    def backward(ctx, dy, dskip):
        if dskip is not None and getattr(ctx, "_kmh_expect_lazy", False):
            expect(dskip, "lazy_gn", True, "pool_fork's skip gradient with its GroupNorm backward pending", "KEYMORPH_NO_LAZY_SKIP")
        lazy = peek(dskip, "lazy_gn") if dskip is not None else None
        if lazy is not None:
            lib = _lib.load()
            c123, x = lazy
            N, D, H, W, C = ctx.xshape
            dxn = _prep(dskip)
            sc2 = torch.zeros(2, dtype=torch.float32, device=dxn.device) if _needs_range_scales() else None
            if dy is None:
                return _gn_bwd_apply(dxn, x, c123, N, D * H * W, C, sc2)
            (arg,) = ctx.saved_tensors
            dx = torch.empty((N, D, H, W, C), dtype=torch.float32, device=dxn.device)
            check(lib.kmh_maxpool3d_bwd_lazy(_p(arg), _p(_prep(dy)), _p(dxn), _p(x), _p(c123), _p(dx), N, D, H, W, C, _p(sc2),
                                             _stream()), "kmh_maxpool3d_bwd_lazy")
            _tag_grad_scale(dx, sc2)
            return dx
        if dy is None:
            return dskip
        return _maxpool_bwd(ctx, dy, dskip)


def pool_fork(x: Tensor):
    y, skip = _PoolFork.apply(x)
    _tag_stats(skip, _peek_stats(x))
    return y, skip


class _UpCat(torch.autograd.Function):
    @staticmethod
    def forward(ctx, skip, low, lazy_skip_grad):
        lib = _lib.load()
        skip, low = _prep(skip), _prep(low)
# ... 233 lines not shown
    ws = workspace(int(lib.kmh_channel_stats_ws_bytes(N, C)), g.device, "stats")
    check(lib.kmh_in_bwd_stats(_p(g), _p(u), _p(scale), _p(shift), N, u.shape[1] * u.shape[2] * u.shape[3], C, _p(ab), _p(ws),
                               _stream()), "kmh_in_bwd_stats")
    c123, _, _ = _gn_bwd_coeffs(ab, None, mr, N, C, C, Dp * Hp * Wp)
    out = g if in_place else torch.empty_like(zprev)
    sc2 = torch.zeros(2, dtype=torch.float32, device=g.device) if _needs_range_scales() else None
    if arg is not None:
        check(lib.kmh_in_bwd_apply_pool(_p(arg), _p(g), _p(zprev), _p(scale), _p(shift), _p(c123), N, Dp, Hp, Wp, C, _p(out),
                                        _p(sc2), _stream()), "kmh_in_bwd_apply_pool")
    else:
        check(lib.kmh_in_bwd_apply(_p(g), _p(zprev), _p(scale), _p(shift), _p(c123), N, Dp * Hp * Wp, C, _p(out), _p(sc2),
                                   _stream()), "kmh_in_bwd_apply")
    _tag_grad_scale(out, sc2)
    return out


@_binds_amp
class _ConvINUnit(torch.autograd.Function):

    @staticmethod
    def forward(ctx, zprev, st, weight, bias, pool, first):
        lib = _lib.load()
        zprev, weight, bias = _prep(zprev), _prep(weight), _prep(bias)
        N, Dp, Hp, Wp, Cin = zprev.shape
        Cout = weight.shape[0]
        ctx.first, ctx.pool = bool(first), bool(pool)
        scale = shift = mr = ascale = arg = None
        u = zprev
        if not first:
            scale, shift, mr, ascale = norm_coeffs(st, None, None, N, Cin, Cin, Dp * Hp * Wp, want_ascale=True)
            if pool:
                u = _f32((N, Dp // 2, Hp // 2, Wp // 2, Cin), zprev.device)
                arg = torch.empty(u.shape, dtype=torch.uint8, device=zprev.device)
                check(lib.kmh_maxpool3d_fwd(_p(zprev), _p(u), _p(arg), N, Dp, Hp, Wp, Cin, _stream()), "kmh_maxpool3d_fwd")
        D, H, W = u.shape[1:4]
        pk = pack_weight(weight, False)
        ctx.wscale = _packed(pk)[1]
        zst = torch.empty((N, Cout, 2), dtype=torch.float64, device=zprev.device)
        z = conv3_raw(u, scale, shift, pk, bias, N, D, H, W, Cin, Cout, not first, False, ascale=ascale, stats_out=zst)
        ctx.ascale = ascale
        ctx.dims = (N, Dp, Hp, Wp, D, H, W, Cin, Cout)
        saved = [zprev, weight] + ([] if first else [scale, shift, mr]) + ([u, arg] if (pool and not first) else [])
        ctx.save_for_backward(*saved)
        ctx.mark_non_differentiable(zst)
        LAZY_IN_STATS["units"] += 1
        return z, zst

    @staticmethod
    def backward(ctx, dz, _dst):
        N, Dp, Hp, Wp, D, H, W, Cin, Cout = ctx.dims
        saved = ctx.saved_tensors
        zprev, weight = saved[0], saved[1]
        dscale = peek(dz, "grad_scale")
        dz = _prep(dz)
        if _needs_range_scales() and dscale is None:
            dscale = absmax_scale(dz)
        db = torch.zeros(Cout, dtype=torch.float32, device=dz.device)
        if ctx.first:
            xs = absmax_scale(zprev) if _needs_range_scales() else None
            dw = conv3_wgrad(zprev, None, None, dz, N, D, H, W, Cin, Cout, False, xscale=xs, dscale=dscale)
            return (None, None, dw, db) + (None,) * 2
        scale, shift, mr = saved[2:5]
        u, arg = (saved[5], saved[6]) if ctx.pool else (zprev, None)
        dw = conv3_wgrad(u, scale, shift, dz, N, D, H, W, Cin, Cout, True, xscale=ctx.ascale, dscale=dscale)
        du = conv3_raw(dz, None, None, pack_weight(weight, True, wscale=ctx.wscale), None, N, D, H, W, Cout, Cin, False, False,
                       ascale=dscale)
        dzp = _in_bwd(du, u, zprev, scale, shift, mr, arg=arg, in_place=not ctx.pool)
        return (dzp, None, dw, db) + (None,) * 2


class _INReluOut(torch.autograd.Function):

    @staticmethod
    def forward(ctx, z, st):
        lib = _lib.load()
        z = _prep(z)
        N, D, H, W, C = z.shape
        V = D * H * W
        scale, shift, mr = norm_coeffs(st, None, None, N, C, C, V)
        y = torch.empty_like(z)
        check(lib.kmh_norm_apply(_p(z), _p(scale), _p(shift), N, V, C, 1, _p(y), _stream()), "kmh_norm_apply")
        ctx.save_for_backward(z, scale, shift, mr)
        return y

    @staticmethod
    def backward(ctx, dy):
        z, scale, shift, mr = ctx.saved_tensors
        return _in_bwd(_prep(dy), z, z, scale, shift, mr), None


def convnet_instance_lazy(x: Tensor, blocks) -> Tensor:
    z = st = None
    pool_prev = False
    for b, (w, bias, down) in enumerate(blocks):
        if b == 0:
            z, st = _ConvINUnit.apply(x, None, w, bias, False, True)
        else:
            z, st = _ConvINUnit.apply(z, st, w, bias, pool_prev, False)
        pool_prev = bool(down)
    y = _INReluOut.apply(z, st)
    return maxpool2(y) if pool_prev else y


HEAD_MASK = os.environ.get("KEYMORPH_HEAD_MASK", "1") != "0"
HEAD_STATS = {"mask": 0, "recompute": 0}


def _headcom_fwd(feat, w, b, sq=None, scales=False, mask=False):
    lib = _lib.load()
    N, D, H, W, Cin = feat.shape
    Cout = w.shape[0]
    pts, sums = _f32((N, Cout, 3), feat.device), _f32((N, Cout, 4), feat.device)
    hsc = hmask = None
    if CONV_MODE != "f32" and Cin % 4 == 0:
        terms = _HEAD_TERMS[CONV_MODE]
        ws = workspace(int(lib.kmh_headcom_fwd_bf_ws_bytes(N, D * H * W, Cout, terms)), feat.device, "head")
        if scales and terms == 2:
            hsc = _f32((4,), feat.device)
        nmask = int(lib.kmh_headcom_mask_words(N, D, H, W, Cout)) if mask else 0
        if nmask:
            hmask = torch.empty(nmask, dtype=torch.int32, device=feat.device)
        check(lib.kmh_headcom_fwd_bf(_p(feat), _p(w), _p(b), _p(pts), _p(sums), _p(sq), _p(hsc), N, D, H, W, Cin, Cout,
                                     _t(terms), _p(hmask), _p(ws), _stream()), "kmh_headcom_fwd_bf")
    else:
        ws = workspace(int(lib.kmh_headcom_fwd_ws_bytes(N, D * H * W, Cout)), feat.device, "head")
        check(lib.kmh_headcom_fwd(_p(feat), _p(w), _p(b), _p(pts), _p(sums), _p(sq), N, D, H, W, Cin, Cout, _p(ws),
                                  _stream()), "kmh_headcom_fwd")
    return pts, sums, hsc, hmask


@_binds_amp
class _HeadCoM(torch.autograd.Function):

    @staticmethod
    def forward(ctx, feat, w, b, feat_from_relu=False):
        ctx.set_materialize_grads(False)
        ctx.mask_dfeat = int(bool(feat_from_relu))
        feat, w = _prep(feat), _prep(w)
        b = None if b is None else _prep(b)
        pts, sums, ctx.hsc, ctx.hmask = _headcom_fwd(feat, w, b, scales=True, mask=HEAD_MASK and any(ctx.needs_input_grad[:3]))
        if CONV_MODE != "f32" and feat.shape[-1] % 4 == 0:
            HEAD_STATS["mask" if ctx.hmask is not None else "recompute"] += 1
        ctx.save_for_backward(feat, w, sums) if b is None else ctx.save_for_backward(feat, w, sums, b)
        return pts, sums[:, :, 0].contiguous()

    @staticmethod
    def backward(ctx, dpts, dpower):
        lib = _lib.load()
        saved = ctx.saved_tensors
        feat, w, sums = saved[:3]
        b = saved[3] if len(saved) > 3 else None
        N, D, H, W, Cin = feat.shape
        Cout = w.shape[0]
        dpts = torch.zeros((N, Cout, 3), dtype=torch.float32, device=feat.device) if dpts is None else _prep(dpts)
        dpower = None if dpower is None else _prep(dpower)
        dfeat = torch.empty_like(feat) if ctx.needs_input_grad[0] else None
        need_w = ctx.needs_input_grad[1] or (b is not None and ctx.needs_input_grad[2])
        dw = torch.empty_like(w) if need_w else None
        db = _f32((Cout,), feat.device) if (need_w and b is not None) else None
        if CONV_MODE != "f32" and Cin % 4 == 0:
            terms = _HEAD_TERMS[CONV_MODE]
            ws = workspace(int(lib.kmh_headcom_bwd_bf_ws_bytes(N, D * H * W, Cin, Cout, terms)), feat.device, "head")
            dsc = (torch.zeros(2, dtype=torch.float32, device=feat.device)
                   if (terms == 2 and dfeat is not None) else None)
            check(lib.kmh_headcom_bwd_bf(_p(dpts), _p(dpower), _p(feat), _p(w), _p(b), _p(sums), _p(dfeat), _p(dw), _p(db), N, D, H,
                                         W, Cin, Cout, _t(terms), ctx.mask_dfeat, _p(ctx.hsc), _p(dsc), _p(ctx.hmask), _p(ws), _stream()),
                  "kmh_headcom_bwd_bf")
            _tag_grad_scale(dfeat, dsc)
        else:
            ws = workspace(int(lib.kmh_headcom_bwd_ws_bytes(N, D * H * W, Cin, Cout)), feat.device, "head")
            check(lib.kmh_headcom_bwd(_p(dpts), _p(dpower), _p(feat), _p(w), _p(b), _p(sums), _p(dfeat), _p(dw), _p(db), N, D, H,
                                      W, Cin, Cout, ctx.mask_dfeat, _p(ws), _stream()), "kmh_headcom_bwd")
        return dfeat, dw, db, None


HEAD_FUSED_MAX_CIN = 64


def head_moments(feat: Tensor, w: Tensor, b: Optional[Tensor]):
    with torch.no_grad():
        feat, w = _prep(feat), _prep(w)
        b = None if b is None else _prep(b)
        sq = _f32((feat.shape[0], w.shape[0]), feat.device)
        pts, sums, _, _ = _headcom_fwd(feat, w, b, sq=sq)
        return pts, sums[:, :, 0].contiguous(), sq


def head_com(feat: Tensor, w: Tensor, b: Optional[Tensor], feat_from_relu: bool = False) -> Tensor:
    return _HeadCoM.apply(feat, w, b, feat_from_relu)[0]


def head_com_power(feat: Tensor, w: Tensor, b: Optional[Tensor], feat_from_relu: bool = False):
    return _HeadCoM.apply(feat, w, b, feat_from_relu)
```

keymorph_amd/csrc/conv_bf.hip:

```cpp
#include <atomic>
#include <cstdio>
#include <cstdlib>
#include "conv_split.h"
#include "stats_final.h"
#include <type_traits>

namespace {

constexpr int TX = 32, TZ = 2;
constexpr int HX = TX + 2, HZ = TZ + 2;
constexpr int NSTEP = 14;
constexpr int BF_TPB = 256;

constexpr int NSTEP_Z = 18;
template <int TERMS>
__global__ __launch_bounds__(256) void pack_weight_bf_kernel(const float* __restrict__ w, __bf16* __restrict__ out,
                                                             int Cout, int Cin, int CoutP, int nchunk,
                                                             int transposed, int zpair,
                                                             const float* __restrict__ wscale ) {
  const int Co = transposed ? Cin : Cout, Ci = transposed ? Cout : Cin;
  const int nstep = zpair ? NSTEP_Z : NSTEP;
  const long long total = (long long)nchunk * nstep * 2 * CoutP * 8;
  for (long long e = (long long)blockIdx.x * 256 + threadIdx.x; e < total; e += (long long)gridDim.x * 256) {
    const int c = (int)(e & 7);
    long long r = e >> 3;
    const int col = (int)(r % CoutP); r /= CoutP;
    const int h = (int)(r & 1); r >>= 1;
    const int s = (int)(r % nstep);
    const int chunk = (int)(r / nstep);
    const int ci = chunk * 8 + c;
    int tap = 2 * s + h, co = col;
    bool ok = tap < 27;
    if (zpair) {
      const int kz = tap / 9 - (col >> 4);
      co = col & 15;
      ok = (col < 32) && kz >= 0 && kz <= 2;
      tap = kz * 9 + tap % 9;
    }
    float v = 0.f;
    if (ok && ci < Ci && co < Co)
      v = transposed ? w[((long long)ci * Cin + co) * 27 + (26 - tap)] : w[((long long)co * Cin + ci) * 27 + tap];
    float rem = wscale ? v * wscale[0] : v;
#pragma unroll
    for (int t = 0; t < TERMS; ++t) {
      float back;
      const unsigned short hb = to16<TERMS>(rem, back);
      reinterpret_cast<unsigned short*>(out)[((((long long)chunk * TERMS + t) * nstep + s) * 2 + h) * CoutP * 8 +
                                             (long long)col * 8 + c] = hb;
      rem -= back;
    }
  }
}

template <int NT, int TERMS, int MR, bool ZP = false, int ZT = 1>
__global__ __launch_bounds__(BF_TPB, ((MR == 2 && NT == 2 && TERMS == 3) ? 3 : 2)) void conv3_fwd_bf_kernel(
    const float* __restrict__ x, const float* __restrict__ scale, const float* __restrict__ shift,
    const float* __restrict__ mask, const bf16x8* __restrict__ wp, const float* __restrict__ bias,
    float* __restrict__ y, int D, int H, int W, int Cin, int Cout, int CoutP, int relu_in, int relu_out,
    int tiles_x, int tiles_y, int tiles_z, int tiles_zp, const float* __restrict__ ascale ,
    const float* __restrict__ wscale ,
    double* __restrict__ stats_partial ,
    int in_blocked ,
    const float* __restrict__ addend ) {
  constexpr int TZv = 2 * ZT, HZv = TZv + 2;
  constexpr int TY = (ZP ? 4 : 2) * MR, HY = TY + 2, PL = HX * HY * HZv;
  constexpr int NST = ZP ? NSTEP_Z : NSTEP;
  static_assert(!ZP || NT == 1, "z-paired tiles are for Cout <= 16");
  __shared__ bf16x8 sIn[TERMS][PL];
  const int tid = threadIdx.x, lane = tid & 63, wv = tid >> 6;
  const int li = lane & 31, lh = lane >> 5;
  const int n = blockIdx.z;
  const int ncog = ZP ? 1 : (Cout + 32 * NT - 1) / (32 * NT);
  const int item = xcd_remap(blockIdx.x, gridDim.x);
  const int cog = item % ncog, brick = item / ncog;
  const int tyz = (tiles_y + 7) >> 3;
  const int lz8 = brick & 7, ly8 = (brick >> 3) & 7, patch = brick >> 6;
  const int pyi = patch % tyz, rest = patch / tyz;
  const int pzi = rest % tiles_zp, bx = rest / tiles_zp;
  const int by = pyi * 8 + ly8, bz = pzi * 8 + lz8;
  if (by >= tiles_y || bz >= tiles_z) return;
  const int x0 = bx * TX, y0 = by * TY, z0 = bz * TZv;
  const int co0 = cog * (32 * NT);
  const int wz = ZP ? 0 : wv >> 1, wy = (ZP ? wv : (wv & 1)) * MR;

  f32x16 acc[ZT][MR][NT];
#pragma unroll
  for (int p = 0; p < ZT; ++p)
#pragma unroll
    for (int m = 0; m < MR; ++m)
#pragma unroll
      for (int t = 0; t < NT; ++t)
#pragma unroll
        for (int r = 0; r < 16; ++r) acc[p][m][t][r] = 0.f;

  const float sA = ascale ? ascale[0] : 1.f;
  const float desc = (ascale ? ascale[1] : 1.f) * (wscale ? wscale[1] : 1.f);
  const bool vec4 = (Cin & 3) == 0;
  const int nchunk = (Cin + KC - 1) / KC;
  const int vrow = (wz * HY + wy) * HX + li;

  constexpr int NV = (PL + BF_TPB - 1) / BF_TPB;
  int sv_rel[NV];
  bool sv_in[NV];
  const long long origin = ((((long long)n * D + z0) * H + y0) * W + x0) * Cin;
#pragma unroll
  for (int i = 0; i < NV; ++i) {
    const int v = tid + i * BF_TPB;
    const int lx = v % HX, ly = (v / HX) % HY, lz = v / (HX * HY);
    const int gx = x0 + lx - 1, gy = y0 + ly - 1, gz = z0 + lz - 1;
    sv_in[i] = (v < PL) && ((unsigned)gx < (unsigned)W) && ((unsigned)gy < (unsigned)H) && ((unsigned)gz < (unsigned)D);
    sv_rel[i] = (((lz - 1) * H + (ly - 1)) * W + (lx - 1)) * (in_blocked ? KC : Cin);
  }
  const long long chunk_stride = in_blocked ? (long long)D * H * W * KC : KC;
  const float* xb = in_blocked ? x + ((long long)n * nchunk * D * H * W + (((long long)z0 * H + y0) * W + x0)) * KC : x + origin;
  const float* mb = mask ? mask + origin : nullptr;
  const int boff = lh * CoutP + co0 + li;

  constexpr bool PF = false;
  constexpr int NPRE = PF ? NV : 1;
  float pv[NPRE][8], pm[NPRE][8];
  auto fetch_one = [&](int ch, int i, float (&v8)[8], float (&m8)[8]) {
    const int c0 = ch * KC;
#pragma unroll
    for (int j = 0; j < 8; ++j) { v8[j] = 0.f; m8[j] = 1.f; }
    if (sv_in[i]) {
      const float* p = xb + sv_rel[i] + ch * chunk_stride;
      if (vec4) {
#pragma unroll
        for (int q = 0; q < 2; ++q) {
          if (c0 + 4 * q < Cin) {
            const float4 t4 = *reinterpret_cast<const float4*>(p + 4 * q);
            v8[4 * q] = t4.x; v8[4 * q + 1] = t4.y; v8[4 * q + 2] = t4.z; v8[4 * q + 3] = t4.w;
            if (mb) {
              const float4 m4 = *reinterpret_cast<const float4*>(mb + sv_rel[i] + c0 + 4 * q);
              m8[4 * q] = m4.x; m8[4 * q + 1] = m4.y; m8[4 * q + 2] = m4.z; m8[4 * q + 3] = m4.w;
            }
          }
        }
      } else {
#pragma unroll
        for (int j = 0; j < 8; ++j)
          if (c0 + j < Cin) {
            v8[j] = p[j];
            if (mb) m8[j] = mb[sv_rel[i] + c0 + j];
          }
      }
    }
  };
  auto commit_one = [&](int ch, int i, const float (&v8)[8], const float (&m8)[8], const float (&csc)[8],
                        const float (&csh)[8]) {
    const int c0 = ch * KC;
    const int v = tid + i * BF_TPB;
    if (v < PL) {
      float val[8];
#pragma unroll
      for (int j = 0; j < 8; ++j) {
        float t = (m8[j] > 0.f) ? v8[j] : 0.f;
        t = t * csc[j] + csh[j];
        if (relu_in) t = fmaxf(t, 0.f);
        val[j] = (sv_in[i] && c0 + j < Cin) ? t : 0.f;
      }
      bf16x8 parts[TERMS];
      split8<TERMS>(val, parts);
#pragma unroll
      for (int t = 0; t < TERMS; ++t) sIn[t][v] = parts[t];
    }
  };

  if (PF) {
#pragma unroll
    for (int i = 0; i < NV; ++i) fetch_one(0, i, pv[PF ? i : 0], pm[PF ? i : 0]);
  }
  for (int ch = 0; ch < nchunk; ++ch) {
    float csc[8], csh[8];
#pragma unroll
    for (int j = 0; j < 8; ++j) {
      const bool ok = scale && (ch * KC + j < Cin);
      csc[j] = (ok ? scale[n * Cin + ch * KC + j] : 1.f) * sA;
      csh[j] = (ok ? shift[n * Cin + ch * KC + j] : 0.f) * sA;
    }
    const bf16x8* wc = wp + (long long)ch * TERMS * NST * 2 * CoutP + boff;
    constexpr int BD = NT == 4 ? 1 : NT == 3 ? 2 : (ZP ? 4 : (TERMS == 2 ? 4 : (NT == 1 ? 2 : 1))) / ZT;
    constexpr int BPRE = BD >= 2 ? BD / 2 : BD;
    bf16x8 bq[BD][NT][TERMS];
#pragma unroll
    for (int d = 0; d < BPRE; ++d)
#pragma unroll
      for (int t = 0; t < NT; ++t)
#pragma unroll
        for (int q = 0; q < TERMS; ++q) bq[d][t][q] = wc[(q * NST + d) * 2 * CoutP + 32 * t];
    __syncthreads();
#pragma unroll
    for (int i = 0; i < NV; ++i) {
      if (!PF) fetch_one(ch, i, pv[0], pm[0]);
      commit_one(ch, i, pv[PF ? i : 0], pm[PF ? i : 0], csc, csh);
    }
    __syncthreads();
    if (PF && ch + 1 < nchunk) {
#pragma unroll
      for (int i = 0; i < NV; ++i) fetch_one(ch + 1, i, pv[PF ? i : 0], pm[PF ? i : 0]);
    }
#pragma unroll
    for (int d = BPRE; d < BD; ++d)
#pragma unroll
// ... 1305 lines not shown
```

keymorph_amd/csrc/conv_up2.hip:

```cpp
#include <cstdlib>
#include "conv_split.h"
#include "stats_final.h"

namespace {

constexpr int UX = 32, UY = 4;
constexpr int UHX = UX + 2, UHY = UY + 2, UPL = UHX * UHY * 3;
constexpr int UP_TPB = 512;
constexpr int UP_NST = 32;

template <int TERMS>
__global__ __launch_bounds__(256) void pack_weight_up_kernel(const float* __restrict__ w, __bf16* __restrict__ out,
                                                             int Cout, int Ctot, int cofs, int Cl, int CoutP, int nchunk,
                                                             const float* __restrict__ wscale) {
  const long long total = (long long)nchunk * UP_NST * 2 * CoutP * 8;
  for (long long e = (long long)blockIdx.x * 256 + threadIdx.x; e < total; e += (long long)gridDim.x * 256) {
    const int c = (int)(e & 7);
    long long r = e >> 3;
    const int col = (int)(r % CoutP); r /= CoutP;
    const int h = (int)(r & 1); r >>= 1;
    const int su = (int)(r % UP_NST);
    const int chunk = (int)(r / UP_NST);
    const int ci = chunk * 8 + c, p = su >> 2, st = su & 3;
    const int par[3] = {p >> 2, (p >> 1) & 1, p & 1}, j[3] = {st >> 1, st & 1, h};
    int lo[3], hi[3];
#pragma unroll
    for (int a = 0; a < 3; ++a) {
      lo[a] = par[a] == 0 ? (j[a] == 0 ? 0 : 1) : (j[a] == 0 ? 0 : 2);
      hi[a] = par[a] == 0 ? (j[a] == 0 ? 0 : 2) : (j[a] == 0 ? 1 : 2);
    }
    float v = 0.f;
    if (ci < Cl && col < Cout) {
      const float* wr = w + ((long long)col * Ctot + cofs + ci) * 27;
      for (int kz = lo[0]; kz <= hi[0]; ++kz)
        for (int ky = lo[1]; ky <= hi[1]; ++ky)
          for (int kx = lo[2]; kx <= hi[2]; ++kx) v += wr[kz * 9 + ky * 3 + kx];
    }
    float rem = wscale ? v * wscale[0] : v;
#pragma unroll
    for (int t = 0; t < TERMS; ++t) {
      float back;
      const unsigned short hb = to16<TERMS>(rem, back);
      reinterpret_cast<unsigned short*>(out)[((((long long)chunk * TERMS + t) * UP_NST + su) * 2 + h) * CoutP * 8 +
                                             (long long)col * 8 + c] = hb;
      rem -= back;
    }
  }
}

template <int TERMS, bool AMP = false>
__global__ __launch_bounds__(UP_TPB, 2) void conv3_up2_fwd_kernel(
    const float* __restrict__ xl, const float* __restrict__ scale, const float* __restrict__ shift, int Ctot, int cofs,
    const bf16x8* __restrict__ wp, float* __restrict__ y, int Dl, int Hl, int Wl, int Cl, int Cout, int CoutP,
    int tiles_x, int tiles_y, const float* __restrict__ ascale, const float* __restrict__ wscale) {
  __shared__ bf16x8 sIn[2][TERMS][UPL];
  const int tid = threadIdx.x, lane = tid & 63, wv = tid >> 6, li = lane & 31, lh = lane >> 5;
  const int n = blockIdx.z;
  const int ncog = (Cout + 63) / 64;
  const int item = xcd_remap(blockIdx.x, gridDim.x);
  const int cog = item % ncog, brick = item / ncog;
  const int bx = brick % tiles_x, by = (brick / tiles_x) % tiles_y, zl = brick / (tiles_x * tiles_y);
  const int x0 = bx * UX, y0 = by * UY;
  const int pz = (wv >> 1) & 1, py = wv & 1, nt = wv >> 2;
  const int co = cog * 64 + 32 * nt + li;

  f32x16 acc[2][UY];
#pragma unroll
  for (int pl = 0; pl < 2; ++pl)
#pragma unroll
    for (int m = 0; m < UY; ++m)
#pragma unroll
      for (int r = 0; r < 16; ++r) acc[pl][m][r] = 0.f;
  const float sA = ascale ? ascale[0] : 1.f;
  const float desc = (ascale ? ascale[1] : 1.f) * (wscale ? wscale[1] : 1.f);
  const int nchunk = Cl / KC;

  constexpr int NV = (UPL + UP_TPB - 1) / UP_TPB;
  int sv_rel[NV];
  bool sv_in[NV];
#pragma unroll
  for (int i = 0; i < NV; ++i) {
    const int v = tid + i * UP_TPB;
    const int lx = v % UHX, ly = (v / UHX) % UHY, lz = v / (UHX * UHY);
    const int gx = x0 + lx - 1, gy = y0 + ly - 1, gz = zl + lz - 1;
    sv_in[i] = (v < UPL) && ((unsigned)gx < (unsigned)Wl) && ((unsigned)gy < (unsigned)Hl) && ((unsigned)gz < (unsigned)Dl);
    sv_rel[i] = sv_in[i] ? ((gz * Hl + gy) * Wl + gx) * Cl : 0;
  }
  const float* xn = xl + (long long)n * Dl * Hl * Wl * Cl;
  float pv[NV][8];
  auto fetch = [&](int ch) {
#pragma unroll
    for (int i = 0; i < NV; ++i) {
      const float* p = xn + sv_rel[i] + ch * KC;
      const float4 a = *reinterpret_cast<const float4*>(p), b = *reinterpret_cast<const float4*>(p + 4);
      pv[i][0] = a.x; pv[i][1] = a.y; pv[i][2] = a.z; pv[i][3] = a.w;
      pv[i][4] = b.x; pv[i][5] = b.y; pv[i][6] = b.z; pv[i][7] = b.w;
    }
  };
  auto commit = [&](int ch, int stage) {
    float csc[8], csh[8];
#pragma unroll
    for (int j = 0; j < 8; ++j) {
      csc[j] = (scale ? scale[(long long)n * Ctot + cofs + ch * KC + j] : 1.f) * sA;
      csh[j] = (scale ? shift[(long long)n * Ctot + cofs + ch * KC + j] : 0.f) * sA;
    }
#pragma unroll
    for (int i = 0; i < NV; ++i) {
      const int v = tid + i * UP_TPB;
      if (v < UPL) {
        float val[8];
#pragma unroll
        for (int j = 0; j < 8; ++j) val[j] = sv_in[i] ? pv[i][j] * csc[j] + csh[j] : 0.f;
        bf16x8 parts[TERMS];
        split8<TERMS>(val, parts);
#pragma unroll
        for (int t = 0; t < TERMS; ++t) sIn[stage][t][v] = parts[t];
      }
    }
  };

  const int wbase = (pz * UHY + py) * UHX + li + lh;
  const int subase = (pz * 4 + py * 2) * 4;
  fetch(0);
  commit(0, 0);
  __syncthreads();
  for (int ch = 0; ch < nchunk; ++ch) {
    const int stage = ch & 1;
    if (ch + 1 < nchunk) fetch(ch + 1);
    const bf16x8* wc = wp + (long long)ch * TERMS * UP_NST * 2 * CoutP + lh * CoutP + co;
    constexpr int BD = 4;
    bf16x8 bq[BD][TERMS];
#pragma unroll
    for (int d = 0; d < BD; ++d)
#pragma unroll
      for (int q = 0; q < TERMS; ++q)
        bq[d][q] = wc[((long long)(q * UP_NST + subase + d)) * 2 * CoutP];
#pragma unroll
    for (int k = 0; k < 8; ++k) {
      const int pl = k >> 2, st = k & 3;
      bf16x8 b[TERMS];
#pragma unroll
      for (int q = 0; q < TERMS; ++q) b[q] = bq[k % BD][q];
      if (k + BD < 8) {
#pragma unroll
        for (int q = 0; q < TERMS; ++q)
          bq[k % BD][q] = wc[((long long)(q * UP_NST + subase + k + BD)) * 2 * CoutP];
      }
      const int off = wbase + ((st >> 1) * UHY + (st & 1)) * UHX + pl;
#pragma unroll
      for (int m = 0; m < UY; ++m) {
        bf16x8 a[TERMS];
#pragma unroll
        for (int q = 0; q < TERMS; ++q) a[q] = sIn[stage][q][off + m * UHX];
        if (TERMS == 3) {
          acc[pl][m] = mfma16<TERMS>(a[2], b[0], acc[pl][m]);
          acc[pl][m] = mfma16<TERMS>(a[1], b[1], acc[pl][m]);
          acc[pl][m] = mfma16<TERMS>(a[0], b[2], acc[pl][m]);
        }
        if constexpr (!AMP) {
          acc[pl][m] = mfma16<TERMS>(a[1], b[0], acc[pl][m]);
          acc[pl][m] = mfma16<TERMS>(a[0], b[1], acc[pl][m]);
        }
        acc[pl][m] = mfma16<TERMS>(a[0], b[0], acc[pl][m]);
      }
    }
    if (ch + 1 < nchunk) commit(ch + 1, stage ^ 1);
    __syncthreads();
  }
  const int D = 2 * Dl, H = 2 * Hl, W = 2 * Wl;
  const int gz = 2 * zl + pz;
  float* tile = reinterpret_cast<float*>(&sIn[0][0][0]) + wv * (32 * 32);
  const int c4 = lane & 7, vx = lane >> 3;
  const int cq = cog * 64 + 32 * nt + 4 * c4;
  const bool cq_ok = cq < Cout;
#pragma unroll
  for (int pl = 0; pl < 2; ++pl)
#pragma unroll
    for (int m = 0; m < UY; ++m) {
#pragma unroll
      for (int r = 0; r < 16; ++r) tile[((r & 3) + 8 * (r >> 2) + 4 * lh) * 32 + li] = acc[pl][m][r] * desc;
      const bool row_ok = cq_ok && y0 + m < Hl;
      const int gy = 2 * (y0 + m) + py;
      float* yp = y + ((((long long)n * D + gz) * H + gy) * W) * Cout + cq;
#pragma unroll
      for (int k = 0; k < 4; ++k) {
        const int xx = vx + 8 * k, xlw = x0 + xx;
        const float4 v = *reinterpret_cast<const float4*>(tile + xx * 32 + 4 * c4);
        if (row_ok && xlw < Wl) *reinterpret_cast<float4*>(yp + (long long)(2 * xlw + pl) * Cout) = v;
      }
    }
}

constexpr int DUX = 16, DUY = 4;
constexpr int DHX = 2 * DUX + 2, DHY = 2 * DUY + 2, DPL = DHX * DHY * 4;
constexpr int DUP_NST = 32;
constexpr int DUP_TPB = 256;

template <int TERMS>
__global__ __launch_bounds__(256) void pack_weight_upt_kernel(const float* __restrict__ w, __bf16* __restrict__ out,
                                                              int Cout, int Ctot, int cofs, int Cl, int CiP, int nchunk,
                                                              const float* __restrict__ wscale) {
  const long long total = (long long)nchunk * DUP_NST * 2 * CiP * 8;
  for (long long e = (long long)blockIdx.x * 256 + threadIdx.x; e < total; e += (long long)gridDim.x * 256) {
    const int c = (int)(e & 7);
    long long r = e >> 3;
    const int col = (int)(r % CiP); r /= CiP;
    const int h = (int)(r & 1); r >>= 1;
    const int s = (int)(r % DUP_NST);
    const int chunk = (int)(r / DUP_NST);
    const int co = chunk * 8 + c;
    const int idx[3] = {s >> 3, (s >> 1) & 3, 2 * (s & 1) + h};
    int lo[3], hi[3];
#pragma unroll
    for (int a = 0; a < 3; ++a) {
      const int par = (idx[a] + 1) & 1, j = idx[a] <= 1 ? 1 : 0;
      lo[a] = par == 0 ? (j == 0 ? 0 : 1) : (j == 0 ? 0 : 2);
      hi[a] = par == 0 ? (j == 0 ? 0 : 2) : (j == 0 ? 1 : 2);
    }
    float v = 0.f;
    if (co < Cout && col < Cl) {
      const float* wr = w + ((long long)co * Ctot + cofs + col) * 27;
      for (int kz = lo[0]; kz <= hi[0]; ++kz)
        for (int ky = lo[1]; ky <= hi[1]; ++ky)
          for (int kx = lo[2]; kx <= hi[2]; ++kx) v += wr[kz * 9 + ky * 3 + kx];
    }
    float rem = wscale ? v * wscale[0] : v;
#pragma unroll
    for (int t = 0; t < TERMS; ++t) {
      float back;
      const unsigned short hb = to16<TERMS>(rem, back);
      reinterpret_cast<unsigned short*>(out)[((((long long)chunk * TERMS + t) * DUP_NST + s) * 2 + h) * CiP * 8 +
                                             (long long)col * 8 + c] = hb;
      rem -= back;
    }
  }
}

template <int TERMS, bool AMP = false>
__global__ __launch_bounds__(DUP_TPB, TERMS == 2 ? 2 : 3) void conv3_up2_dgrad_kernel(
    const float* __restrict__ dz , const bf16x8* __restrict__ wp,
    float* __restrict__ ds , int Dl, int Hl, int Wl, int Cl, int CiP, int Cout, int tiles_x,
    int tiles_y, const float* __restrict__ dscale, const float* __restrict__ wscale,
    double* __restrict__ stats_partial ,
    int in_blocked ) {
  __shared__ bf16x8 sIn[TERMS][DPL];
  const int tid = threadIdx.x, lane = tid & 63, wv = tid >> 6, li = lane & 31, lh = lane >> 5;
  const int n = blockIdx.z;
  const int ncig = (Cl + 127) / 128;
  const int item = xcd_remap(blockIdx.x, gridDim.x);
  const int cig = item % ncig, brick = item / ncig;
  const int bx = brick % tiles_x, by = (brick / tiles_x) % tiles_y, zl = brick / (tiles_x * tiles_y);
  const int x0 = bx * DUX, y0 = by * DUY;
  const int ci = cig * 128 + 32 * wv + li;
  const int D = 2 * Dl, H = 2 * Hl, W = 2 * Wl;

  f32x16 acc[2];
#pragma unroll
  for (int m = 0; m < 2; ++m)
#pragma unroll
    for (int r = 0; r < 16; ++r) acc[m][r] = 0.f;
  const float sD = dscale ? dscale[0] : 1.f;
  const float desc = (dscale ? dscale[1] : 1.f) * (wscale ? wscale[1] : 1.f);
  const int nchunk = (Cout + KC - 1) / KC;
  const float* dn = dz + (long long)n * D * H * W * Cout;
  constexpr int NV = (DPL + DUP_TPB - 1) / DUP_TPB;
  const int abase = (2 * (li >> 4)) * DHX + 2 * (li & 15) + lh;

  float4 pre[NV][2];
  auto fetch = [&](int ch) {
#pragma unroll
    for (int i = 0; i < NV; ++i) {
      const int v = tid + i * DUP_TPB;
      pre[i][0] = pre[i][1] = make_float4(0.f, 0.f, 0.f, 0.f);
      if (v < DPL) {
        const int lx = v % DHX, ly = (v / DHX) % DHY, lz = v / (DHX * DHY);
        const int gx = 2 * x0 - 1 + lx, gy = 2 * y0 - 1 + ly, gz = 2 * zl - 1 + lz;
        if ((unsigned)gx < (unsigned)W && (unsigned)gy < (unsigned)H && (unsigned)gz < (unsigned)D) {
          const long long vox = ((long long)gz * H + gy) * W + gx;
          const float* p = in_blocked ? dn + ((long long)ch * D * H * W + vox) * KC : dn + vox * Cout + ch * KC;
          if ((Cout & 3) == 0) {
#pragma unroll
            for (int q = 0; q < 2; ++q)
              if (ch * KC + 4 * q < Cout) pre[i][q] = *reinterpret_cast<const float4*>(p + 4 * q);
          } else {
            float t8[8] = {0.f, 0.f, 0.f, 0.f, 0.f, 0.f, 0.f, 0.f};
#pragma unroll
            for (int j = 0; j < 8; ++j)
              if (ch * KC + j < Cout) t8[j] = p[j];
            pre[i][0] = make_float4(t8[0], t8[1], t8[2], t8[3]);
            pre[i][1] = make_float4(t8[4], t8[5], t8[6], t8[7]);
          }
        }
      }
    }
  };
  constexpr bool PF = TERMS == 2;
  if (PF) fetch(0);
  for (int ch = 0; ch < nchunk; ++ch) {
    __syncthreads();
    if (!PF) fetch(ch);
#pragma unroll
    for (int i = 0; i < NV; ++i) {
      const int v = tid + i * DUP_TPB;
      if (v < DPL) {
        const float val[8] = {pre[i][0].x * sD, pre[i][0].y * sD, pre[i][0].z * sD, pre[i][0].w * sD,
                              pre[i][1].x * sD, pre[i][1].y * sD, pre[i][1].z * sD, pre[i][1].w * sD};
        bf16x8 parts[TERMS];
        split8<TERMS>(val, parts);
#pragma unroll
        for (int t = 0; t < TERMS; ++t) sIn[t][v] = parts[t];
      }
    }
    __syncthreads();
    if (PF && ch + 1 < nchunk) fetch(ch + 1);
    const bf16x8* wc = wp + (long long)ch * TERMS * DUP_NST * 2 * CiP + lh * CiP + ci;
    constexpr int BD = 4;
    bf16x8 bq[BD][TERMS];
#pragma unroll
    for (int d = 0; d < BD; ++d)
#pragma unroll
      for (int q = 0; q < TERMS; ++q) bq[d][q] = wc[((long long)(q * DUP_NST + d)) * 2 * CiP];
#pragma unroll 1
    for (int tz = 0; tz < 4; ++tz) {
#pragma unroll
      for (int s8 = 0; s8 < 8; ++s8) {
        const int s = tz * 8 + s8;
        bf16x8 b[TERMS];
#pragma unroll
        for (int q = 0; q < TERMS; ++q) b[q] = bq[s8 % BD][q];
        if (s + BD < DUP_NST) {
#pragma unroll
          for (int q = 0; q < TERMS; ++q) bq[s8 % BD][q] = wc[((long long)(q * DUP_NST + s + BD)) * 2 * CiP];
        }
        const int off = abase + (tz * DHY + (s8 >> 1)) * DHX + 2 * (s8 & 1);
#pragma unroll
        for (int m = 0; m < 2; ++m) {
          bf16x8 a[TERMS];
#pragma unroll
          for (int q = 0; q < TERMS; ++q) a[q] = sIn[q][off + 4 * m * DHX];
          if (TERMS == 3) {
            acc[m] = mfma16<TERMS>(a[2], b[0], acc[m]);
            acc[m] = mfma16<TERMS>(a[1], b[1], acc[m]);
            acc[m] = mfma16<TERMS>(a[0], b[2], acc[m]);
          }
          if constexpr (!AMP) {
            acc[m] = mfma16<TERMS>(a[1], b[0], acc[m]);
            acc[m] = mfma16<TERMS>(a[0], b[1], acc[m]);
          }
          acc[m] = mfma16<TERMS>(a[0], b[0], acc[m]);
        }
      }
    }
  }
  if (ci >= Cl) return;
  float s1 = 0.f, s2 = 0.f;
#pragma unroll
  for (int m = 0; m < 2; ++m) {
#pragma unroll
    for (int r = 0; r < 16; ++r) {
      const int row = (r & 3) + 8 * (r >> 2) + 4 * lh;
      const int gx = x0 + (row & 15), gy = y0 + 2 * m + (row >> 4);
      if (gx < Wl && gy < Hl) {
        const float v = acc[m][r] * desc;
        ds[((((long long)n * Dl + zl) * Hl + gy) * Wl + gx) * Cl + ci] = v;
        s1 += v;
        s2 = fmaf(v, v, s2);
      }
    }
  }
  if (stats_partial) {
    double d1 = (double)s1, d2 = (double)s2;
    d1 += __shfl_xor(d1, 32, 64);
    d2 += __shfl_xor(d2, 32, 64);
    if (lh == 0) {
      double* o = stats_partial + (((long long)n * gridDim.x / ncig + brick) * Cl + ci) * 2;
      o[0] = d1; o[1] = d2;
    }
  }
}

constexpr int GK = 32;
constexpr int GPITCH = GK * 2 + 16;
template <int TERMS, bool AMP = false>
__global__ __launch_bounds__(256, 3) void up2_wgrad_gemm_kernel(const float* __restrict__ A, const float* __restrict__ B,
                                                                float* __restrict__ Cp, int V, int Cl, int J, int kslab,
                                                                int ntn, int ntm, const float* __restrict__ ascale,
                                                                const float* __restrict__ bscale,
                                                                const float* __restrict__ a_scale ,
// ... 548 lines not shown
```

keymorph_amd/csrc/firstlayer.hip:

```cpp
#include <cstdlib>
#include "common.h"
#include "stats_final.h"

namespace {

constexpr int FL_XS = 2;
constexpr int FL_TPB = 320;
constexpr int FL_YR = 8;
constexpr int FL_CO = 16;

__global__ __launch_bounds__(FL_TPB) void first_wgrad_kernel(const float* __restrict__ x, const float* __restrict__ dz,
                                                            const float* __restrict__ dzmask,
                                                            float* __restrict__ partial , int D,
                                                            int H, int W, int Cout, int ytiles,
                                                            const float* __restrict__ c123) {
  extern __shared__ __attribute__((aligned(16))) float fsm[];
  const int WP = (W + 3) & ~3;
  const int XP = WP + 8;
  const int DP = WP + 4;
  float* xs = fsm;
  float* ds = fsm + 3 * (FL_YR + 2) * XP;
  const int tid = threadIdx.x;
  const int n = blockIdx.z, z = blockIdx.y, y0 = blockIdx.x * FL_YR;
  const float* xn = x + (long long)n * D * H * W;
// ... 392 lines not shown
  store_tile(0);
  __syncthreads();
  const int gx = x0 + vx;
  float s1[2] = {0.f, 0.f}, s2[2] = {0.f, 0.f};
  float* yn = y + (long long)n * D * H * W * Cout;
  const int zend = (zc + FF_Z < D) ? zc + FF_Z : D;
  for (int z = zc; z < zend; ++z) {
    const float* t = sx[(z - zc) & 1];
    if (z + 1 < zend) load_tile(z + 1);
    float win[3][3][3];
#pragma unroll
    for (int kz = 0; kz < 3; ++kz)
#pragma unroll
      for (int ky = 0; ky < 2; ++ky)
#pragma unroll
        for (int kx = 0; kx < 3; ++kx) win[kz][ky + 1][kx] = t[(kz * (FF_Y + 2) + ky) * FF_P + vx + kx];
    static_assert(FF_Y % 3 == 0, "row blocks of three");
#pragma unroll 1
    for (int yb = 0; yb < FF_Y; yb += 3)
#pragma unroll
    for (int yj = 0; yj < 3; ++yj) {
      const int yy = yb + yj;
#pragma unroll
      for (int kz = 0; kz < 3; ++kz)
#pragma unroll
        for (int kx = 0; kx < 3; ++kx) {
          win[kz][0][kx] = win[kz][1][kx];
          win[kz][1][kx] = win[kz][2][kx];
          win[kz][2][kx] = t[(kz * (FF_Y + 2) + yy + 2) * FF_P + vx + kx];
        }
      kmh_f2 a01 = {0.f, 0.f};
#pragma unroll
      for (int kz = 0; kz < 3; ++kz)
#pragma unroll
        for (int ky = 0; ky < 3; ++ky)
#pragma unroll
          for (int kx = 0; kx < 3; ++kx) {
            const float v = win[kz][ky][kx];
            a01 = __builtin_elementwise_fma(kmh_f2{v, v}, w01[(kz * 3 + ky) * 3 + kx], a01);
          }
      const int gy = y0 + yy;
      if (gx < W && gy < H) {
        const float o[2] = {fmaxf(a01.x, 0.f), fmaxf(a01.y, 0.f)};
        float* dst = yn + (((long long)z * H + gy) * W + gx) * Cout + FF_CPT * q;
        if ((Cout & 1) == 0) {
          if (FF_CPT * q < Cout) *reinterpret_cast<float2*>(dst) = make_float2(o[0], o[1]);
        } else {
#pragma unroll
          for (int j = 0; j < 2; ++j)
            if (FF_CPT * q + j < Cout) dst[j] = o[j];
        }
#pragma unroll
        for (int j = 0; j < 2; ++j) { s1[j] += o[j]; s2[j] += o[j] * o[j]; }
      }
    }
    if (z + 1 < zend) store_tile((z + 1 - zc) & 1);
    __syncthreads();
  }
  if (stats_partial) {
    const int lane = tid & 63, wv = tid >> 6;
#pragma unroll
    for (int j = 0; j < 2; ++j) {
      double d1 = (double)s1[j], d2 = (double)s2[j];
#pragma unroll
      for (int o = FF_SUB; o < kWave; o <<= 1) { d1 += __shfl_xor(d1, o, kWave); d2 += __shfl_xor(d2, o, kWave); }
      if (lane < FF_SUB) { sred[wv][FF_CPT * lane + j][0] = d1; sred[wv][FF_CPT * lane + j][1] = d2; }
    }
    __syncthreads();
    if (tid < 2 * Cout) {
      const int c = tid >> 1, k = tid & 1;
      const long long blk = ((long long)n * gridDim.y + blockIdx.y) * gridDim.x + blockIdx.x;
      double s = 0;
#pragma unroll
      for (int wq = 0; wq < FF_TPB / kWave; ++wq) s += sred[wq][c][k];
      stats_partial[(blk * Cout + c) * 2 + k] = s;
    }
  }
}

}

KMH_API size_t kmh_conv3d_first_layer_fwd_ws_bytes(int N, int D, int H, int W, int Cout) {
  return (size_t)N * ceil_div(D, FF_Z) * ceil_div(W, FF_X) * ceil_div(H, FF_Y) * Cout * 2 * sizeof(double);
}

KMH_API int kmh_conv3d_first_layer_fwd(const float* x, const float* scale, const float* shift, const float* w, float* y,
                                       int N, int D, int H, int W, int Cout, void* ws, double* stats_out, void* stream) {
  if (Cout > 16 || Cout < 1) return -22;
  hipStream_t s = (hipStream_t)stream;
  const int xt = ceil_div(W, FF_X), yt = ceil_div(H, FF_Y);
  const int zt = ceil_div(D, FF_Z);
  first_fwd_kernel<<<dim3(xt * yt, zt, N), FF_TPB, 0, s>>>(x, scale, shift, w, y, stats_out ? (double*)ws : nullptr, D, H,
                                                          W, Cout, xt, yt);
  if (stats_out)
    kmh_stats::final_kernel<<<dim3(ceil_div(Cout * 2, 256 / kWave), N), 256, 0, s>>>((const double*)ws, zt * xt * yt,
                                                                                  Cout, stats_out);
  return KMH_LAUNCH_CHECK();
}

KMH_API size_t kmh_conv3d_first_layer_wgrad_ws_bytes(int N, int D, int H, int W, int Cout) {
  (void)W;
  return (size_t)N * D * ceil_div(H, FL_YR) * FL_XS * Cout * 54 * sizeof(float);
}

KMH_API int kmh_conv3d_first_layer_wgrad(const float* x, const float* dz, const float* dzmask, const float* c123, double* rs,
                                         int N, int D, int H, int W, int Cout, void* ws, void* stream) {
  if (Cout > FL_CO || Cout < 1 || W < 1 || (c123 && !dzmask)) return -22;
  hipStream_t s = (hipStream_t)stream;
  const int WP = (W + 3) & ~3, XP = WP + 8;
  const size_t lds = ((size_t)3 * (FL_YR + 2) * XP + (size_t)2 * FL_CO * (WP + 4)) * sizeof(float);
  if (lds > 160 * 1024) return -22;
  hipError_t e = hipFuncSetAttribute((const void*)first_wgrad_kernel, hipFuncAttributeMaxDynamicSharedMemorySize, (int)lds);
  if (e != hipSuccess) return (int)e;
  const int yt = ceil_div(H, FL_YR);
  const int per = Cout * 54;
  static const bool valu_only = getenv("KEYMORPH_FIRST_WGRAD_VALU") != nullptr;
  size_t ds_floats = (size_t)2 * WP * 16;
  if (ds_floats < 2 * 4 * 2 * 64 * 4) ds_floats = 2 * 4 * 2 * 64 * 4;
  const size_t lds_m = ((size_t)3 * (FM_YR + 2) * XP + ds_floats + 2 * 4 * 16 + 2 * 2 * 16) * sizeof(float);
  if (!valu_only && lds_m <= 160 * 1024 && FM_YR == FL_YR) {
    hipError_t e2 = hipFuncSetAttribute((const void*)first_wgrad_mfma_kernel, hipFuncAttributeMaxDynamicSharedMemorySize, (int)lds_m);
    if (e2 != hipSuccess) return (int)e2;
    first_wgrad_mfma_kernel<<<dim3(yt, D, N), FM_TPB, lds_m, s>>>(x, dz, dzmask, (float*)ws, D, H, W, Cout, yt, c123);
    first_wgrad_reduce_kernel<<<dim3(ceil_div(per, 4), N), 256, 0, s>>>((const float*)ws, D * yt, per, rs);
    return KMH_LAUNCH_CHECK();
  }
  first_wgrad_kernel<<<dim3(yt, D, N), FL_TPB, lds, s>>>(x, dz, dzmask, (float*)ws, D, H, W, Cout, yt, c123);
  first_wgrad_reduce_kernel<<<dim3(ceil_div(per, 4), N), 256, 0, s>>>((const float*)ws, D * yt * FL_XS, per, rs);
  return KMH_LAUNCH_CHECK();
}

namespace {
template <typename RS>
__global__ __launch_bounds__(256) void first_layer_fold_kernel(const RS* __restrict__ rs, const float* __restrict__ w,
                                                               const float* __restrict__ scale,
                                                               const float* __restrict__ shift, int Cout,
                                                               float* __restrict__ dw, double* __restrict__ ab,
                                                               int accumulate) {
  const float sc = scale[0], sh = shift[0];
  double a = 0, b = 0;
  for (int e = threadIdx.x; e < Cout * 27; e += 256) {
    const int co = e / 27, tap = e % 27;
    const RS R = rs[(co * 2 + 0) * 27 + tap], S = rs[(co * 2 + 1) * 27 + tap];
    const float g = (float)((RS)sc * R + (RS)sh * S);
    dw[e] = accumulate ? dw[e] + g : g;
    a += (double)w[e] * (double)S;
    b += (double)w[e] * (double)R;
  }
  __shared__ double red[4];
  a = block_sum<double>(a, red);
  b = block_sum<double>(b, red);
  if (threadIdx.x == 0) { ab[0] = a; ab[1] = b; }
}
}

KMH_API int kmh_conv3d_first_layer_fold(const void* rs, int rs_f64, const float* w, const float* scale_n, const float* shift_n,
                                        int Cout, float* dw, double* ab_n, int accumulate, void* stream) {
  if (rs_f64)
    first_layer_fold_kernel<double><<<1, 256, 0, (hipStream_t)stream>>>((const double*)rs, w, scale_n, shift_n, Cout, dw, ab_n, accumulate);
  else
    first_layer_fold_kernel<float><<<1, 256, 0, (hipStream_t)stream>>>((const float*)rs, w, scale_n, shift_n, Cout, dw, ab_n, accumulate);
  return KMH_LAUNCH_CHECK();
}
```

keymorph_amd/parallel.py:

```python
from __future__ import annotations

import os
from typing import Iterable, List

import torch
import torch.distributed as dist

from . import _lib
from ._lib import check
from .ops import _p, _stream


def init_distributed():
    world = int(os.environ.get("WORLD_SIZE", "1"))
    rank = int(os.environ.get("RANK", "0"))
    local = int(os.environ.get("LOCAL_RANK", "0"))
    if os.environ.get("KEYMORPH_SHARE_GPU") == "1":
        local = 0
    if world > 1 and not dist.is_initialized():
        os.environ.setdefault("MASTER_ADDR", "127.0.0.1")
        os.environ.setdefault("MASTER_PORT", "29500")
        backend = os.environ.get("KEYMORPH_DIST_BACKEND") or ("nccl" if torch.cuda.is_available() else "gloo")
        if torch.cuda.is_available():
            torch.cuda.set_device(local)
        dist.init_process_group(backend=backend, rank=rank, world_size=world)
    return rank, local, world


def shard_indices(num_items: int, rank: int, world: int) -> List[int]:
    base, rem = divmod(num_items, world)
    start = rank * base + min(rank, rem)
    return list(range(start, start + base + (1 if rank < rem else 0)))


class FlatParams:

    def __init__(self, params: Iterable[torch.nn.Parameter]):
        self.params = [p for p in params if p.requires_grad]
        n = sum(p.numel() for p in self.params)
        dev = self.params[0].device
        self.flat = torch.empty(n, dtype=torch.float32, device=dev)
        self._grad = torch.zeros(n, dtype=torch.float32, device=dev)
        self._views = []
        o = 0
        for p in self.params:
            k = p.numel()
            self.flat[o:o + k].copy_(p.data.reshape(-1))
            p.data = self.flat[o:o + k].view_as(p.data)
            v = self._grad[o:o + k].view_as(p.data)
            p.grad = v
            self._views.append(v)
            o += k
        self.numel = n

    def zero_grad(self):
        for p in self.params:
            p.grad = None

    def gather(self) -> torch.Tensor:
        src, dst, zero = [], [], []
        for p, v in zip(self.params, self._views):
            g = p.grad
            if g is None:
                zero.append(v)
            elif g.data_ptr() != v.data_ptr():
                src.append(g.detach().reshape(v.shape).to(v.dtype))
                dst.append(v)
            p.grad = v
        with torch.no_grad():
            if zero:
                torch._foreach_zero_(zero)
            if dst:
                torch._foreach_copy_(dst, src)
        return self._grad

    @property
    def grad(self) -> torch.Tensor:
        return self.gather()

    def broadcast(self, src: int = 0):
        if dist.is_initialized() and dist.get_world_size() > 1:
            dist.broadcast(self.flat, src)

    def allreduce_grads(self) -> float:
        g = self.gather()
        if dist.is_initialized() and dist.get_world_size() > 1:
            dist.all_reduce(g, op=dist.ReduceOp.SUM)
            return 1.0 / dist.get_world_size()
        return 1.0


class FusedAdam:

    def __init__(self, flat: FlatParams, lr=1e-3, betas=(0.9, 0.999), eps=1e-8):
        self.flat, self.lr, self.betas, self.eps = flat, lr, betas, eps
        self.m = torch.zeros_like(flat.flat)
        self.v = torch.zeros_like(flat.flat)
        self.t = 0

    def state_dict(self):
        state, o = {}, 0
        for i, p in enumerate(self.flat.params):
            k = p.numel()
            state[i] = {"step": torch.tensor(float(self.t)), "exp_avg": self.m[o:o + k].view_as(p).clone(),
                        "exp_avg_sq": self.v[o:o + k].view_as(p).clone()}
            o += k
        group = {"lr": self.lr, "betas": tuple(self.betas), "eps": self.eps, "weight_decay": 0, "amsgrad": False,
                 "maximize": False, "foreach": None, "capturable": False, "differentiable": False, "fused": None,
                 "params": list(range(len(self.flat.params)))}
        return {"state": state, "param_groups": [group]}

    def load_state_dict(self, sd):
        groups = sd["param_groups"]
        assert len(groups) == 1 and len(groups[0]["params"]) == len(self.flat.params), "parameter list mismatch"
        g = groups[0]
        assert not g.get("amsgrad", False) and not g.get("weight_decay", 0), "plain Adam only"
        self.lr, self.betas, self.eps = g["lr"], tuple(g["betas"]), g["eps"]
        o, steps = 0, set()
        for i, p in zip(g["params"], self.flat.params):
            k = p.numel()
            st = sd["state"].get(i)
            if st is None:
                self.m[o:o + k].zero_(); self.v[o:o + k].zero_()
            else:
                self.m[o:o + k].copy_(st["exp_avg"].reshape(-1))
                self.v[o:o + k].copy_(st["exp_avg_sq"].reshape(-1))
                steps.add(int(st["step"]))
            o += k
        assert len(steps) <= 1, "per-parameter step counts differ"
        self.t = steps.pop() if steps else 0

    def step(self, grad_scale: float = 1.0):
        self.t += 1
        lib = _lib.load()
        check(lib.kmh_adam_step(_p(self.flat.flat), _p(self.flat.gather()), _p(self.m), _p(self.v), self.flat.numel,
                                self.lr, self.betas[0], self.betas[1], self.eps, self.t, grad_scale, _stream()),
              "kmh_adam_step")


def gather_group_points(local_points: torch.Tensor, num_subjects: int) -> torch.Tensor:
    if not (dist.is_initialized() and dist.get_world_size() > 1):
        assert local_points.shape[0] == num_subjects
        return local_points
    world, rank = dist.get_world_size(), dist.get_rank()
    counts = [len(shard_indices(num_subjects, r, world)) for r in range(world)]
    assert local_points.shape[0] == counts[rank], "this rank's block does not match shard_indices()"
    m = max(counts)
    pad = local_points.new_zeros((m,) + tuple(local_points.shape[1:]))
    pad[: counts[rank]] = local_points
    outs = [torch.empty_like(pad) for _ in range(world)]
    dist.all_gather(outs, pad.contiguous())
    return torch.cat([o[:c] for o, c in zip(outs, counts)], dim=0)


def allgather_points(points: torch.Tensor) -> torch.Tensor:
    if not (dist.is_initialized() and dist.get_world_size() > 1):
        return points
    outs = [torch.empty_like(points) for _ in range(dist.get_world_size())]
    dist.all_gather(outs, points.contiguous())
    return torch.cat(outs, dim=0)
```

keymorph_amd/unet3d/model.py:

```python
from __future__ import annotations

import torch
import torch.nn as nn

from .. import backbone_ops as B


def number_of_features_per_level(init_channel_number, num_levels):
    return [init_channel_number * 2 ** k for k in range(num_levels)]


class SingleConv(nn.Module):

    def __init__(self, in_channels, out_channels, num_groups=8, first_layer=False):
        super().__init__()
        g = 1 if in_channels < num_groups else num_groups
        assert in_channels % g == 0, (
            f"Expected number of channels in input to be divisible by num_groups. "
            f"num_channels={in_channels}, num_groups={g}")
        self.groupnorm = nn.GroupNorm(num_groups=g, num_channels=in_channels)
        self.conv = nn.Conv3d(in_channels, out_channels, 3, padding=1, bias=False)
        self._groups = g
        self._first = first_layer
        self._dy_premasked = False

    def forward(self, x, dy_premasked=None, dy_blocked=False, dx_blocked=False, pool=False, dy_lazy=False,
                dx_lazy=False, dgrad_terms=0):
        return B.single_conv_gcr(x, self.groupnorm.weight, self.groupnorm.bias, self.conv.weight, self._groups,
                                 x_from_relu=not self._first,
                                 dy_premasked=self._dy_premasked if dy_premasked is None else dy_premasked,
                                 dy_blocked=dy_blocked, dx_blocked=dx_blocked, pool=pool, dy_lazy=dy_lazy, dx_lazy=dx_lazy,
                                 dgrad_terms=dgrad_terms)


class DoubleConv(nn.Module):
    def __init__(self, in_channels, out_channels, encoder, num_groups=8, first_layer=False):
        super().__init__()
        if encoder:
            c1_out = max(out_channels // 2, in_channels)
            c1 = (in_channels, c1_out)
            c2 = (c1_out, out_channels)
        else:
            c1 = (in_channels, out_channels)
            c2 = (out_channels, out_channels)
        self.SingleConv1 = SingleConv(*c1, num_groups=num_groups, first_layer=first_layer)
        self.SingleConv2 = SingleConv(*c2, num_groups=num_groups)
        self.SingleConv1._dy_premasked = True

    def forward(self, x, out_premasked=None, out_dy_blocked=False, out_pool=False):
        n, d, h, w, cin = x.shape
        blk = (torch.is_grad_enabled() and self.SingleConv1._dy_premasked
               and B.grad_blocked_ok(n, d, h, w, cin, self.SingleConv1.conv.out_channels))
        lazy = (self.SingleConv1._first and self.SingleConv1._dy_premasked and not blk
                and B.lazy_first_layer_ok(x, self.SingleConv1.conv.out_channels))
        return self.SingleConv2(self.SingleConv1(x, dy_blocked=blk, dy_lazy=lazy), out_premasked,
                                dy_blocked=out_dy_blocked, dx_blocked=blk, pool=out_pool, dx_lazy=lazy,
                                dgrad_terms=B.first_block_dgrad_terms() if self.SingleConv1._first else 0)


class Encoder(nn.Module):
    def __init__(self, in_channels, out_channels, apply_pooling=True, num_groups=8, first_layer=False):
        super().__init__()
        self.apply_pooling = apply_pooling
        self.basic_module = DoubleConv(in_channels, out_channels, True, num_groups, first_layer)

    def forward(self, x):
        if self.apply_pooling:
            x = B.maxpool2(x)
        return self.basic_module(x)


class Decoder(nn.Module):
    def __init__(self, in_channels, out_channels, num_groups=8):
        super().__init__()
        self.basic_module = DoubleConv(in_channels, out_channels, False, num_groups)

    def forward(self, encoder_features, x, lazy_skip_grad=False, out_premasked=None):
        dc = self.basic_module
        c1 = dc.SingleConv1
        if B.upcat_conv_ok(encoder_features, x, c1.conv.out_channels):
            blk = B.upcat_blocked_ok(encoder_features, x, c1.conv.out_channels)
            h = B.upcat_conv_gcr(encoder_features, x, c1.groupnorm.weight, c1.groupnorm.bias, c1.conv.weight,
                                 c1._groups, dy_premasked=True,
                                 dskip_lazy=bool(lazy_skip_grad) and B.lazy_skip_ok(encoder_features), dy_blocked=blk)
            return dc.SingleConv2(h, out_premasked, dx_blocked=blk)
        return dc(B.upcat(encoder_features, x, lazy_skip_grad), out_premasked)


class AbstractUNet(nn.Module):
    def __init__(self, in_channels, out_channels, final_sigmoid=True, f_maps=64, layer_order="gcr", num_groups=8,
                 num_levels=4, is_segmentation=True, conv_padding=1, num_truncated_layers=0, use_checkpoint=False, **kwargs):
        super().__init__()
        self.use_checkpoint = bool(use_checkpoint)
        if layer_order != "gcr" or conv_padding != 1:
            raise NotImplementedError("keymorph_amd implements the 'gcr', padding=1 U-Net of scripts/run.py")
        if isinstance(f_maps, int):
            f_maps = number_of_features_per_level(f_maps, num_levels=num_levels)
        assert isinstance(f_maps, (list, tuple)) and len(f_maps) > 1, "Required at least 2 levels in the U-Net"
        self.f_maps = list(f_maps)
        self.encoders = nn.ModuleList(
            Encoder(in_channels if i == 0 else f_maps[i - 1], f, apply_pooling=i > 0, num_groups=num_groups,
                    first_layer=i == 0)
            for i, f in enumerate(f_maps))
        rf = list(reversed(f_maps))
        decs = [Decoder(rf[i] + rf[i + 1], rf[i + 1], num_groups) for i in range(len(rf) - 1)]
        if num_truncated_layers > 0:
            decs = decs[:-num_truncated_layers]
        self.decoders = nn.ModuleList(decs)
        self.final_conv = nn.Conv3d(f_maps[num_truncated_layers], out_channels, 1)
        convs = [m for m in self.modules() if isinstance(m, SingleConv)]
        last_block = (self.decoders[-1] if len(self.decoders) else self.encoders[-1]).basic_module
        for m in convs:
            m._dy_premasked = m is not last_block.SingleConv2
        if is_segmentation:
            self.final_activation = nn.Sigmoid() if final_sigmoid else nn.Softmax(dim=1)
        else:
            self.final_activation = None

    def features(self, x, head_masks_gradient=False):
        last_pm = True if head_masks_gradient else None
        x = B.to_ndhwc(x)
        feats = []
        L, nd = len(self.encoders), len(self.decoders)
        forked = {L - 2 - j for j in range(nd)}
        pooled = None
        prev_blk = False
        for i, enc in enumerate(self.encoders):
            opm = last_pm if (nd == 0 and i == L - 1) else None
            nxt_pools = i + 1 < L and self.encoders[i + 1].apply_pooling and i not in forked
            c2 = enc.basic_module.SingleConv2
            blk_out = (nxt_pools and torch.is_grad_enabled() and c2._dy_premasked and opm is None
                       and c2.conv.out_channels % 8 == 0)
            if i == 0 or not enc.apply_pooling:
                xin = x
            else:
                xin = pooled if pooled is not None else B.maxpool2(x, blocked_grad=prev_blk)
            if blk_out:
                n_, d_, h_, w_ = xin.shape[0], xin.shape[1], xin.shape[2], xin.shape[3]
                blk_out = (d_ % 2 == 0 and h_ % 2 == 0 and w_ % 2 == 0 and
                           B.grad_blocked_ok(n_, d_, h_, w_, c2.conv.in_channels, c2.conv.out_channels))
            fuse_pool = (nxt_pools and opm is None and c2._dy_premasked
                         and B.conv_pool_ok(xin.shape[0], xin.shape[1], xin.shape[2], xin.shape[3], c2.conv.in_channels,
                                            c2.conv.out_channels))
            x = self._block(enc.basic_module, xin, opm, out_dy_blocked=blk_out, out_pool=fuse_pool)
            prev_blk = blk_out
            pooled = x if fuse_pool else None
            if fuse_pool:
                feats.insert(0, (None, False))
                continue
            if i in forked and i + 1 < L and self.encoders[i + 1].apply_pooling:
                pooled, x = B.pool_fork(x)
                feats.insert(0, (x, True))
            else:
                feats.insert(0, (x, False))
        x = feats[0][0]
        for j, (dec, (skip, lazy)) in enumerate(zip(self.decoders, feats[1:])):
            x = self._block(dec, skip, x, lazy, last_pm if j == nd - 1 else None)
        return x

    def _block(self, fn, *args, **kwargs):
        if self.use_checkpoint and torch.is_grad_enabled():
            from torch.utils import checkpoint
            return checkpoint.checkpoint(lambda *a: fn(*a, **kwargs), *args, use_reentrant=False)
        return fn(*args, **kwargs)

    def keypoints_ij(self, x):
        assert self.final_activation is None or self.training
        fused = self.final_conv.in_channels <= B.HEAD_FUSED_MAX_CIN
        feat = self.features(x, head_masks_gradient=fused)
        if not fused:
            from .. import ops
            return ops.com3d(B.pointwise(feat, self.final_conv.weight, self.final_conv.bias))
        return B.head_com(feat, self.final_conv.weight, self.final_conv.bias, feat_from_relu=True)

    def keypoints_and_power(self, x):
        assert self.final_activation is None or self.training
        if self.final_conv.in_channels > B.HEAD_FUSED_MAX_CIN:
            raise NotImplementedError("keypoint weighting needs the fused head (final conv with <= 64 input channels)")
        feat = self.features(x, head_masks_gradient=True)
        return B.head_com_power(feat, self.final_conv.weight, self.final_conv.bias, feat_from_relu=True)

    def keypoints_and_moments(self, x):
        assert self.final_activation is None or self.training
        feat = self.features(x)
        if feat.shape[-1] > B.HEAD_FUSED_MAX_CIN:
            raise NotImplementedError("keypoint weighting needs the fused head (final conv with <= 64 input channels)")
        pts, power, sq = B.head_moments(feat, self.final_conv.weight, self.final_conv.bias)
        return pts, power, sq, feat.shape[1] * feat.shape[2] * feat.shape[3]

    def forward(self, x):
        y = B.pointwise(self.features(x), self.final_conv.weight, self.final_conv.bias)
        if not self.training and self.final_activation is not None:
            y = self.final_activation(y)
        return y


class UNet3D(AbstractUNet):

    def __init__(self, in_channels, out_channels, final_sigmoid=True, f_maps=64, layer_order="gcr", num_groups=8,
                 num_levels=4, is_segmentation=True, conv_padding=1, use_checkpoint=False, **kwargs):
        super().__init__(in_channels, out_channels, final_sigmoid, f_maps, layer_order, num_groups, num_levels,
                         is_segmentation, conv_padding, 0, use_checkpoint=use_checkpoint)


class TruncatedUNet3D(AbstractUNet):

    def __init__(self, in_channels, out_channels, num_truncated_layers, final_sigmoid=True, f_maps=64,
                 layer_order="gcr", num_groups=8, num_levels=4, is_segmentation=True, conv_padding=1,
                 use_checkpoint=False, **kwargs):
        super().__init__(in_channels, out_channels, final_sigmoid, f_maps, layer_order, num_groups, num_levels,
                         is_segmentation, conv_padding, num_truncated_layers, use_checkpoint=use_checkpoint)


from .._absent import absent_class as _absent_class, absent_function as _absent_function

UNet2D = _absent_class("UNet2D", "keymorph/unet3d/model.py:266", nn.Module)
ResidualUNet3D = _absent_class("ResidualUNet3D", "keymorph/unet3d/model.py:192", nn.Module)
ResidualUNetSE3D = _absent_class("ResidualUNetSE3D", "keymorph/unet3d/model.py:228", nn.Module)
AbstractTruncatedUNet = AbstractUNet
get_model = _absent_function("get_model", "keymorph/unet3d/model.py:300")
```

Before: 15.55.

## Batch weight packing into a cached per-model weight bank with multi-segment kernels

Adds a WeightBank that packs every conv weight image (forward, backward, up and up-transposed) in a single multi-descriptor kernel launch, preceded by one batched absmax-scale launch, and reuses those images across the forward and backward passes. Refills are triggered by tensor version counters; the optimizer step now bumps those versions. The per-sample first-layer fold loop is replaced by one batched fold call, and several small zero allocations are merged into a single buffer. This targets the many small launches and repeated per-call weight repacking, at the cost of extra persistent memory and cache-invalidation logic that relies on version tracking.

```diff
diff --git a/include/keymorph_hip.h b/include/keymorph_hip.h
--- a/include/keymorph_hip.h
+++ b/include/keymorph_hip.h
@@ -164,6 +164,8 @@
                                  int D, int H, int W, int Cout, void* ws, void* stream);
 int kmh_conv3d_first_layer_fold(const void* rs, int rs_f64, const float* w, const float* scale_n, const float* shift_n, int Cout,
                                 float* dw, double* ab_n, int accumulate, void* stream);
+int kmh_conv3d_first_layer_fold_batch(const double* rs, const float* w, const float* scale, const float* shift, int N, int Cout,
+                                      float* dw, double* ab, void* stream);
 size_t kmh_conv3d_wgrad_ws_bytes(int N, int D, int H, int W, int Cin, int Cout);
 int kmh_conv3d_wgrad(const float* x, const float* scale, const float* shift, const float* dz,
                      const float* dzmask, float* dw, int N, int D, int H, int W, int Cin, int Cout, int relu_in,
@@ -175,6 +177,9 @@
 int kmh_gn_fwd_coeffs(const double* stats, const float* gamma, const float* beta, int N, int C, int G, double count,
                       float eps, float* scale, float* shift, float* mean_rstd, float* ascale, void* stream);
 int kmh_absmax_scale(const float* x, long long n, float min_abs, float* out2, void* stream);
+int kmh_absmax_scale_multi(const void* segs, int count, float* out, void* stream);
+int kmh_conv3d_pack_multi_geometry(int kind, int Cout, int C, int transposed, int* pad, int* zpair, long long* total, int* nblk);
+int kmh_conv3d_pack_multi(const void* descs, int count, int total_blocks, int terms, void* stream);
 int kmh_gn_bwd_coeffs(const double* ab, const float* gamma, const float* mean_rstd, int N, int C, int G,
                       double count, float* c123, float* dgamma, float* dbeta, const int* only_if, void* stream);
 int kmh_gn_bwd_coeffs_fold(const double* dstats, const double* bhat, const float* gamma, const float* beta,
diff --git a/keymorph_amd/_lib.py b/keymorph_amd/_lib.py
--- a/keymorph_amd/_lib.py
+++ b/keymorph_amd/_lib.py
@@ -94,12 +94,16 @@
     "kmh_conv3d_first_layer_wgrad_ws_bytes": (_sz, [_i, _i, _i, _i, _i]),
     "kmh_conv3d_first_layer_wgrad": (_i, [_f, _f, _f, _f, _f, _i, _i, _i, _i, _i, _f, _f]),
     "kmh_conv3d_first_layer_fold": (_i, [_f, _i, _f, _f, _f, _i, _f, _f, _i, _f]),
+    "kmh_conv3d_first_layer_fold_batch": (_i, [_f, _f, _f, _f, _i, _i, _f, _f, _f]),
     "kmh_conv3d_wgrad_ws_bytes": (_sz, [_i, _i, _i, _i, _i, _i]),
     "kmh_conv3d_wgrad": (_i, [_f, _f, _f, _f, _f, _f, _i, _i, _i, _i, _i, _i, _i, _i, _f, _f]),
     "kmh_channel_stats_ws_bytes": (_sz, [_i, _i]),
     "kmh_channel_stats": (_i, [_f, _f, _i, _i, _ll, _i, _f, _f, _f, _f]),
     "kmh_gn_fwd_coeffs": (_i, [_f, _f, _f, _i, _i, _i, C.c_double, C.c_float, _f, _f, _f, _f, _f]),
     "kmh_absmax_scale": (_i, [_f, _ll, C.c_float, _f, _f]),
+    "kmh_absmax_scale_multi": (_i, [_f, _i, _f, _f]),
+    "kmh_conv3d_pack_multi_geometry": (_i, [_i, _i, _i, _i, C.POINTER(_i), C.POINTER(_i), C.POINTER(_ll), C.POINTER(_i)]),
+    "kmh_conv3d_pack_multi": (_i, [_f, _i, _i, _i, _f]),
     "kmh_gn_bwd_coeffs": (_i, [_f, _f, _f, _i, _i, _i, C.c_double, _f, _f, _f, _f, _f]),
     "kmh_gn_bwd_coeffs_fold": (_i, [_f, _f, _f, _f, _f, _i, _i, _i, C.c_double, _f, _f, _f, _f, _f]),
     "kmh_gn_bwd_apply": (_i, [_f, _f, _f, _i, _ll, _i, _i, _i, _f, _f, _i, _f]),
diff --git a/keymorph_amd/backbone_ops.py b/keymorph_amd/backbone_ops.py
--- a/keymorph_amd/backbone_ops.py
+++ b/keymorph_amd/backbone_ops.py
@@ -1,6 +1,8 @@
 from __future__ import annotations
 
+import math
 import os
+import struct
 from typing import Optional, Tuple
 
 import torch
@@ -52,6 +54,7 @@
 import contextlib
 import functools
 import threading
+import weakref
 
 _AMP_DEFAULT = os.environ.get("KEYMORPH_AMP", "0") not in ("", "0")
 _amp_tls = threading.local()
@@ -248,8 +251,135 @@
     return out
 
 
+def _fwd_image(weight: Tensor) -> Tensor:
+    img = _bank_images(weight)
+    return img["fwd"] if img is not None else pack_weight(weight, False)
+
+
+def _bwd_image(weight: Tensor, wscale: Optional[Tensor] = None, terms: int = 0) -> Tensor:
+    img = None if terms else _bank_images(weight)
+    return img["bwd"] if img is not None else pack_weight(weight, True, wscale, terms=terms)
+
+
 def _packed(pk: Tensor):
     return peek(pk, "packed") or (0, None)
+
+
+def _zeros(dev, *specs):
+    cut, nbytes = [], 0
+    for sp in specs:
+        n = 0 if sp is None else math.prod(sp[0]) * sp[1].itemsize
+        cut.append((nbytes, n))
+        nbytes += -(-n // 16) * 16
+    buf = torch.zeros(nbytes, dtype=torch.uint8, device=dev)
+    return [None if sp is None else buf[o:o + n].view(sp[1]).view(sp[0]) for sp, (o, n) in zip(specs, cut)]
+
+
+def _absmax_seg(ptr: int, n: int, row_len: int, row_stride: int, col_ofs: int = 0, min_abs: float = 0.0, mul: float = 1.0,
+                inv_mul: float = 1.0) -> bytes:
+    return struct.pack("<Qqqqqfffi", ptr, n, row_len, row_stride, col_ofs, min_abs, mul, inv_mul, 0)
+
+
+def _device_table(records: bytes, dev) -> Tensor:
+    return torch.frombuffer(bytearray(records), dtype=torch.uint8).to(dev)
+
+
+_BANK_OF = {}
+BANK_STATS = {"fills": 0, "hits": 0, "misses": 0}
+
+
+class WeightBank:
+    def __init__(self, specs):
+        self.specs = [(w, int(cs)) for w, cs in specs]
+        self._layout = self._state = None
+        self.entries = []
+
+    def __reduce__(self):
+        return (WeightBank, (self.specs,))
+
+    def _build_layout(self, mode, dev):
+        import ctypes
+        lib = _lib.load()
+        terms = _TERMS[mode]
+        segs, images = [], []
+        self.entries = []
+        for w, cs in self.specs:
+            Cout, Ctot = w.shape[:2]
+            ent = {}
+            if cs:
+                Cl = Ctot - cs
+                segs.append((w, Cout * cs * 27, cs * 27, Ctot * 27, 0, 1.0, 1.0))
+                segs.append((w, Cout * Cl * 27, Cl * 27, Ctot * 27, cs * 27, 0.125, 8.0))
+                ss, sl = len(segs) - 2, len(segs) - 1
+                for key, kind, C, cofs, tr, sg in (("fwd_s", 0, cs, 0, 0, ss), ("bwd_s", 0, cs, 0, 1, ss),
+                                                   ("up", 1, Cl, cs, 0, sl), ("upt", 2, Cl, cs, 0, sl)):
+                    images.append((ent, key, kind, w, Cout, C, Ctot, cofs, tr, sg))
+            else:
+                segs.append((w, w.numel(), w.numel(), w.numel(), 0, 1.0, 1.0))
+                for key, tr in (("fwd", 0), ("bwd", 1)):
+                    images.append((ent, key, 0, w, Cout, Ctot, Ctot, 0, tr, len(segs) - 1))
+            self.entries.append(ent)
+        self.scales = _f32((len(segs), 2), dev)
+        geo, nbytes = [], 0
+        for (_, _, kind, w, Cout, C, _, _, tr, _) in images:
+            pad, zp, total, nblk = ctypes.c_int(), ctypes.c_int(), ctypes.c_longlong(), ctypes.c_int()
+            check(lib.kmh_conv3d_pack_multi_geometry(kind, Cout, C, tr, ctypes.byref(pad), ctypes.byref(zp), ctypes.byref(total),
+                                                     ctypes.byref(nblk)), "kmh_conv3d_pack_multi_geometry")
+            geo.append((pad.value, zp.value, total.value, nblk.value, nbytes))
+            nbytes += -(-(total.value * terms * 2) // 256) * 256
+        self.images = torch.empty(nbytes, dtype=torch.uint8, device=dev)
+        seg_tab = b"".join(_absmax_seg(w.data_ptr(), n, rl, rs, co, 0.0, mul, inv) for (w, n, rl, rs, co, mul, inv) in segs)
+        img_tab, blk0 = b"", 0
+        for (ent, key, kind, w, Cout, C, Ctot, cofs, tr, sg), (pad, zp, total, nblk, ofs) in zip(images, geo):
+            wscale = self.scales[sg] if terms == 2 else None
+            out = self.images[ofs:ofs + total * terms * 2]
+            attach(out, "packed", (terms, wscale))
+            ent[key] = out
+            if kind:
+                ent["wsu"] = wscale
+            img_tab += struct.pack("<QQQ10iq", w.data_ptr(), out.data_ptr(), _p(wscale) or 0, kind, Cout, C, Ctot, cofs, pad, tr, zp,
+                                   blk0, nblk, total)
+            blk0 += nblk
+        self.nseg, self.nimg, self.nblk, self.terms = len(segs), len(images), blk0, terms
+        self.seg_tab, self.img_tab = _device_table(seg_tab, dev), _device_table(img_tab, dev)
+        for i, (w, _) in enumerate(self.specs):
+            _BANK_OF[w.data_ptr()] = (weakref.ref(self), i)
+
+    def ensure(self):
+        mode = CONV_MODE
+        if mode not in _TERMS or not self.specs or not self.specs[0][0].is_cuda:
+            return
+        if self.specs[0][0].device.index != torch.cuda.current_device():
+            return
+        ws = [w for w, _ in self.specs]
+        layout = (mode, tuple((w.data_ptr(), tuple(w.shape), w.dtype, w.is_contiguous()) for w in ws))
+        if any(k[2] != torch.float32 or not k[3] for k in layout[1]):
+            return
+        state = tuple(w._version for w in ws)
+        if layout == self._layout and state == self._state:
+            return
+        if layout != self._layout:
+            self._build_layout(mode, ws[0].device)
+            self._layout = layout
+        lib = _lib.load()
+        if self.terms == 2:
+            check(lib.kmh_absmax_scale_multi(_p(self.seg_tab), self.nseg, _p(self.scales), _stream()), "kmh_absmax_scale_multi")
+        check(lib.kmh_conv3d_pack_multi(_p(self.img_tab), self.nimg, self.nblk, self.terms, _stream()), "kmh_conv3d_pack_multi")
+        self._state = state
+        BANK_STATS["fills"] += 1
+
+
+def _bank_images(weight: Tensor, cs: int = 0):
+    hit = _BANK_OF.get(weight.data_ptr())
+    if hit is not None:
+        bank, i = hit[0](), hit[1]
+        w, wcs = bank.specs[i] if bank is not None else (None, -1)
+        if (wcs == cs and bank._state is not None and bank._layout[0] == CONV_MODE and w.data_ptr() == weight.data_ptr()
+                and w.shape == weight.shape and bank._state[i] == weight._version == w._version):
+            BANK_STATS["hits"] += 1
+            return bank.entries[i]
+    BANK_STATS["misses"] += 1
+    return None
 
 
 def _conv_meta(N, D, H, W, Cin, Cout, taps=27) -> None:
@@ -325,9 +455,8 @@
             _lib.profiler.meta = {"flops": 2.0 * 27 * 2 * Cout * V * N, "shape": (N, D, H, W, 1, Cout)}
         check(lib.kmh_conv3d_first_layer_wgrad(_p(x), _p(dy), _p(ymask), _p(lazy_c123), _p(rs), N, D, H, W, Cout, _p(ws),
                                                _stream()), "kmh_conv3d_first_layer_wgrad")
-        for n in range(N):
-            check(lib.kmh_conv3d_first_layer_fold(_p(rs[n]), 1, _p(weight), _p(scale[n]), _p(shift[n]), Cout, _p(dw),
-                                                  _p(ab[n]), int(n > 0), _stream()), "kmh_conv3d_first_layer_fold")
+        check(lib.kmh_conv3d_first_layer_fold_batch(_p(rs), _p(weight), _p(scale), _p(shift), N, Cout, _p(dw), _p(ab),
+                                                    _stream()), "kmh_conv3d_first_layer_fold_batch")
     else:
         assert lazy_c123 is None
         terms = _TERMS[CONV_MODE]
@@ -352,14 +481,16 @@
     lib = _lib.load()
     N, D, H, W, Cout = dz.shape
     terms = _TERMS[CONV_MODE]
-    wsu = None
-    if terms == 2:
-        wsu = absmax_scale(weight[:, Cs:].contiguous()) * _const(dz.device, 0.125, 8.0)
-        if dscale is None:
-            dscale = absmax_scale(dz)
-    pk = torch.empty(int(lib.kmh_conv3d_up2_dgrad_pack_bytes(Cout, Cl, terms)), dtype=torch.uint8, device=dz.device)
-    check(lib.kmh_conv3d_up2_dgrad_pack_weight(_p(weight), _p(pk), Cout, Cs + Cl, Cs, Cl, terms, _p(wsu), _stream()),
-          "kmh_conv3d_up2_dgrad_pack_weight")
+    if terms == 2 and dscale is None:
+        dscale = absmax_scale(dz)
+    img = _bank_images(weight, Cs)
+    if img is not None:
+        pk, wsu = img["upt"], img["wsu"]
+    else:
+        wsu = absmax_scale(weight[:, Cs:].contiguous()) * _const(dz.device, 0.125, 8.0) if terms == 2 else None
+        pk = torch.empty(int(lib.kmh_conv3d_up2_dgrad_pack_bytes(Cout, Cl, terms)), dtype=torch.uint8, device=dz.device)
+        check(lib.kmh_conv3d_up2_dgrad_pack_weight(_p(weight), _p(pk), Cout, Cs + Cl, Cs, Cl, terms, _p(wsu), _stream()),
+              "kmh_conv3d_up2_dgrad_pack_weight")
     ds = _f32((N, D // 2, H // 2, W // 2, Cl), dz.device)
     _conv_meta(N, D, H, W, Cout, Cl, taps=8)
     sws = None
@@ -410,12 +541,12 @@
     return peek(t, "layout") or 0
 
 
-def _gn_bwd_coeffs(ab, gamma, mr, N, C, G, V, fold=None):
+def _gn_bwd_coeffs(ab, gamma, mr, N, C, G, V, fold=None, dgb=None):
     lib = _lib.load()
     c123 = _f32((N, C, 3), mr.device)
     dgamma = dbeta = flag = None
     if gamma is not None:
-        dgamma, dbeta = torch.zeros_like(gamma), torch.zeros_like(gamma)
+        dgamma, dbeta = dgb if dgb is not None else _zeros(gamma.device, (gamma.shape, gamma.dtype), (gamma.shape, gamma.dtype))
     if fold is not None:
         dstats, bhat, beta = fold
         flag = torch.empty(1, dtype=torch.int32, device=mr.device)
@@ -472,7 +603,7 @@
                              ystats)
         elif pool:
             assert dy_premasked and ystats is not None and conv_pool_ok(N, D, H, W, Cin, Cout)
-            pk = pack_weight(weight, False)
+            pk = _fwd_image(weight)
             ctx.wscale = _packed(pk)[1]
             y = _f32((N, D // 2, H // 2, W // 2, Cout), x.device)
             arg = torch.empty((N, D // 2, H // 2, W // 2, Cout), dtype=torch.uint8, device=x.device)
@@ -485,7 +616,7 @@
             ctx.pool_arg = arg
             POOL_STATS["fused"] += 1
         else:
-            pk = pack_weight(weight, False)
+            pk = _fwd_image(weight)
             ctx.wscale = _packed(pk)[1]
             y = conv3_raw(x, scale, shift, pk, None, N, D, H, W, Cin, Cout, False, True, ascale=ascale,
                           stats_out=ystats)
@@ -555,7 +686,10 @@
         need_affine = ctx.needs_input_grad[1] or ctx.needs_input_grad[2]
         need_dxn = ctx.needs_input_grad[0] or need_affine
         fold = need_dxn and ctx.needs_input_grad[3] and conv_emits_stats() and not _off("KEYMORPH_NO_STATS_FOLD")
-        bhat = torch.zeros((N, Cin), dtype=torch.float64, device=x.device) if fold else None
+        want_sc2 = need_dxn and _needs_range_scales() and ctx.needs_input_grad[0]
+        f32g = gamma is not None and gamma.dtype == torch.float32 and need_dxn
+        bhat, sc2, dg0, db0 = _zeros(x.device, ((N, Cin), torch.float64) if fold else None, ((2,), torch.float32) if want_sc2 else None,
+                                     (gamma.shape, torch.float32) if f32g else None, (gamma.shape, torch.float32) if f32g else None)
         dw = (conv3_wgrad(x, scale, shift, dy, N, D, H, W, Cin, Cout, False, dzmask=ymask, xscale=ctx.ascale,
                           dscale=dscale, dz_blocked=kind, fold=(weight, bhat) if fold else None)
               if ctx.needs_input_grad[3] else None)
@@ -565,12 +699,12 @@
             if ctx.dgrad_terms:
                 FIRST_BLOCK_STATS["exact_dgrads"] += 1
             dxn = conv3_raw(dy, None, None,
-                            pack_weight(weight, True, None if ctx.dgrad_terms else getattr(ctx, "wscale", None), terms=ctx.dgrad_terms),
+                            _bwd_image(weight, None if ctx.dgrad_terms else getattr(ctx, "wscale", None), ctx.dgrad_terms),
                             None, N, D, H, W, Cout, Cin, False, False,
                             mask=ymask, ascale=dscale, in_blocked=kind, stats_out=dstats)
-            sc2 = torch.zeros(2, dtype=torch.float32, device=x.device) if (_needs_range_scales() and ctx.needs_input_grad[0]) else None
             c123, dgamma, dbeta = _gn_bwd_coeffs(lambda flag: channel_stats(dxn, x, N, V, Cin, only_if=flag), gamma, mr,
-                                                 N, Cin, G, V, fold=(dstats, bhat, beta) if fold else None)
+                                                 N, Cin, G, V, fold=(dstats, bhat, beta) if fold else None,
+                                                 dgb=(dg0, db0) if f32g else None)
             if ctx.needs_input_grad[0] and dx_lazy:
                 assert x_from_relu and not dx_blocked
                 dx = dxn
@@ -586,13 +720,17 @@
     lib = _lib.load()
     terms = _TERMS[CONV_MODE]
     dev = skip.device
-    pk_s = pack_weight(weight[:, :Cs].contiguous(), False)
-    wsu = None
-    if terms == 2:
-        wsu = absmax_scale(weight[:, Cs:].contiguous()) * _const(dev, 0.125, 8.0)
-    pku = torch.empty(int(lib.kmh_conv3d_up2_pack_bytes(Cout, Cl, terms)), dtype=torch.uint8, device=dev)
-    check(lib.kmh_conv3d_up2_pack_weight(_p(weight), _p(pku), Cout, Cs + Cl, Cs, Cl, terms, _p(wsu), _stream()),
-          "kmh_conv3d_up2_pack_weight")
+    img = _bank_images(weight, Cs)
+    if img is not None:
+        pk_s, pku, wsu = img["fwd_s"], img["up"], img["wsu"]
+    else:
+        pk_s = pack_weight(weight[:, :Cs].contiguous(), False)
+        wsu = None
+        if terms == 2:
+            wsu = absmax_scale(weight[:, Cs:].contiguous()) * _const(dev, 0.125, 8.0)
+        pku = torch.empty(int(lib.kmh_conv3d_up2_pack_bytes(Cout, Cl, terms)), dtype=torch.uint8, device=dev)
+        check(lib.kmh_conv3d_up2_pack_weight(_p(weight), _p(pku), Cout, Cs + Cl, Cs, Cl, terms, _p(wsu), _stream()),
+              "kmh_conv3d_up2_pack_weight")
     part = _f32((N, D, H, W, Cout), dev)
     _conv_meta(N, D, H, W, Cl, Cout, taps=8)
     check(lib.kmh_conv3d_up2_fwd(_p(low), _p(scale), _p(shift), Cs + Cl, Cs, _p(pku), _p(part), N, D // 2, H // 2,
@@ -648,7 +786,10 @@
             check(lib.kmh_relu_mask(_p(dy), _p(y), dy.numel(), _p(dzm), _stream()), "kmh_relu_mask")
             dy = dzm
         dscale = grad_scale(dy) if _needs_range_scales() else None
-        bhat_s = torch.zeros((N, Cs), dtype=torch.float64, device=dy.device)
+        rs_, f32g = _needs_range_scales(), gamma is not None and gamma.dtype == torch.float32
+        bhat_s, amax_s, amax_l, dg0, db0 = _zeros(dy.device, ((N, Cs), torch.float64), ((2,), torch.float32) if rs_ else None,
+                                              ((2,), torch.float32) if rs_ else None, (gamma.shape, torch.float32) if f32g else None,
+                                              (gamma.shape, torch.float32) if f32g else None)
         dw_s = conv3_wgrad(skip, scale[:, :Cs].contiguous(), shift[:, :Cs].contiguous(), dy, N, D, H, W, Cs, Cout, False,
                            xscale=ctx.ascale, dscale=dscale, dz_blocked=blk, fold=(weight[:, :Cs].contiguous(), bhat_s))
         if Cout % 4 == 0 and not _off("KEYMORPH_NO_UPCONV_WGRAD"):
@@ -680,7 +821,7 @@
             xu = _f32((N, D, H, W, Cl), dy.device)
             check(lib.kmh_upcat_fwd(_p(skip), _p(low), _p(xu), N, D, H, W, 0, D // 2, H // 2, W // 2, Cl, _stream()),
                   "kmh_upcat_fwd")
-            bhat_l = torch.zeros((N, Cl), dtype=torch.float64, device=dy.device)
+            (bhat_l,) = _zeros(dy.device, ((N, Cl), torch.float64))
             dw_l = conv3_wgrad(xu, scale[:, Cs:].contiguous(), shift[:, Cs:].contiguous(), dy, N, D, H, W, Cl, Cout,
                                False, xscale=ctx.ascale, dscale=dscale, dz_blocked=blk,
                                fold=(weight[:, Cs:].contiguous(), bhat_l))
@@ -688,27 +829,27 @@
         dw = torch.cat([dw_s, dw_l], dim=1)
         bhat = torch.cat([bhat_s, bhat_l], dim=1)
         dst_s = torch.empty((N, Cs, 2), dtype=torch.float64, device=dy.device)
-        dxn_s = conv3_raw(dy, None, None, pack_weight(weight[:, :Cs].contiguous(), True), None, N, D, H, W, Cout, Cs,
+        img = _bank_images(weight, Cs)
+        pk_t = img["bwd_s"] if img is not None else pack_weight(weight[:, :Cs].contiguous(), True)
+        dxn_s = conv3_raw(dy, None, None, pk_t, None, N, D, H, W, Cout, Cs,
                           False, False, ascale=dscale, stats_out=dst_s, in_blocked=blk)
         dst_l = torch.empty((N, Cl, 2), dtype=torch.float64, device=dy.device)
         dsum_l = conv3_up2_dgrad(dy, weight, Cs, Cl, dscale, stats_out=dst_l, dz_blocked=blk)
         dstats = torch.cat([dst_s, dst_l], dim=1)
         ab = lambda flag: torch.cat([channel_stats(dxn_s, skip, N, V, Cs, only_if=flag),
                                      channel_stats(dsum_l, low, N, V // 8, Cl, only_if=flag)], dim=1)
-        c123, dgamma, dbeta = _gn_bwd_coeffs(ab, gamma, mr, N, C, G, V, fold=(dstats, bhat, beta))
+        c123, dgamma, dbeta = _gn_bwd_coeffs(ab, gamma, mr, N, C, G, V, fold=(dstats, bhat, beta), dgb=(dg0, db0) if f32g else None)
         c_s = c123[:, :Cs].contiguous()
         c_l = (c123[:, Cs:] * _const(dy.device, 1.0, 8.0, 8.0)).contiguous()
-        sc_s = torch.zeros(2, dtype=torch.float32, device=dy.device) if _needs_range_scales() else None
-        sc_l = torch.zeros(2, dtype=torch.float32, device=dy.device) if _needs_range_scales() else None
         dskip = dlow = None
         if ctx.needs_input_grad[0] and ctx.dskip_lazy:
             dskip = dxn_s
             attach(dskip, "lazy_gn", (c_s, skip))
             LAZY_STATS["handoffs"] += 1
         elif ctx.needs_input_grad[0]:
-            dskip = _gn_bwd_apply(dxn_s, skip, c_s, N, V, Cs, sc_s)
+            dskip = _gn_bwd_apply(dxn_s, skip, c_s, N, V, Cs, amax_s)
         if ctx.needs_input_grad[1]:
-            dlow = _gn_bwd_apply(dsum_l, low, c_l, N, V // 8, Cl, sc_l)
+            dlow = _gn_bwd_apply(dsum_l, low, c_l, N, V // 8, Cl, amax_l)
         return (dskip, dlow, dgamma, dbeta, dw) + (None,) * 4
 
 
@@ -1248,17 +1389,18 @@
         b = saved[3] if len(saved) > 3 else None
         N, D, H, W, Cin = feat.shape
         Cout = w.shape[0]
-        dpts = torch.zeros((N, Cout, 3), dtype=torch.float32, device=feat.device) if dpts is None else _prep(dpts)
+        bf_head = CONV_MODE != "f32" and Cin % 4 == 0
+        dpts0, dsc = _zeros(feat.device, ((N, Cout, 3), torch.float32) if dpts is None else None,
+                            ((2,), torch.float32) if (bf_head and _HEAD_TERMS[CONV_MODE] == 2 and ctx.needs_input_grad[0]) else None)
+        dpts = dpts0 if dpts is None else _prep(dpts)
         dpower = None if dpower is None else _prep(dpower)
         dfeat = torch.empty_like(feat) if ctx.needs_input_grad[0] else None
         need_w = ctx.needs_input_grad[1] or (b is not None and ctx.needs_input_grad[2])
         dw = torch.empty_like(w) if need_w else None
         db = _f32((Cout,), feat.device) if (need_w and b is not None) else None
-        if CONV_MODE != "f32" and Cin % 4 == 0:
+        if bf_head:
             terms = _HEAD_TERMS[CONV_MODE]
             ws = workspace(int(lib.kmh_headcom_bwd_bf_ws_bytes(N, D * H * W, Cin, Cout, terms)), feat.device, "head")
-            dsc = (torch.zeros(2, dtype=torch.float32, device=feat.device)
-                   if (terms == 2 and dfeat is not None) else None)
             check(lib.kmh_headcom_bwd_bf(_p(dpts), _p(dpower), _p(feat), _p(w), _p(b), _p(sums), _p(dfeat), _p(dw), _p(db), N, D, H,
                                          W, Cin, Cout, _t(terms), ctx.mask_dfeat, _p(ctx.hsc), _p(dsc), _p(ctx.hmask), _p(ws), _stream()),
                   "kmh_headcom_bwd_bf")
diff --git a/keymorph_amd/csrc/conv_bf.hip b/keymorph_amd/csrc/conv_bf.hip
--- a/keymorph_amd/csrc/conv_bf.hip
+++ b/keymorph_amd/csrc/conv_bf.hip
@@ -2,6 +2,7 @@
 #include <cstdio>
 #include <cstdlib>
 #include "conv_split.h"
+#include "pack_images.h"
 #include "stats_final.h"
 #include <type_traits>
 
@@ -13,43 +14,15 @@
 constexpr int BF_TPB = 256;
 
 constexpr int NSTEP_Z = 18;
+static_assert(NSTEP == kmh_pack::kSteps27 && NSTEP_Z == kmh_pack::kSteps36, "pack_images.h packs for these step counts");
 template <int TERMS>
 __global__ __launch_bounds__(256) void pack_weight_bf_kernel(const float* __restrict__ w, __bf16* __restrict__ out,
                                                              int Cout, int Cin, int CoutP, int nchunk,
                                                              int transposed, int zpair,
                                                              const float* __restrict__ wscale ) {
-  const int Co = transposed ? Cin : Cout, Ci = transposed ? Cout : Cin;
-  const int nstep = zpair ? NSTEP_Z : NSTEP;
-  const long long total = (long long)nchunk * nstep * 2 * CoutP * 8;
-  for (long long e = (long long)blockIdx.x * 256 + threadIdx.x; e < total; e += (long long)gridDim.x * 256) {
-    const int c = (int)(e & 7);
-    long long r = e >> 3;
-    const int col = (int)(r % CoutP); r /= CoutP;
-    const int h = (int)(r & 1); r >>= 1;
-    const int s = (int)(r % nstep);
-    const int chunk = (int)(r / nstep);
-    const int ci = chunk * 8 + c;
-    int tap = 2 * s + h, co = col;
-    bool ok = tap < 27;
-    if (zpair) {
-      const int kz = tap / 9 - (col >> 4);
-      co = col & 15;
-      ok = (col < 32) && kz >= 0 && kz <= 2;
-      tap = kz * 9 + tap % 9;
-    }
-    float v = 0.f;
-    if (ok && ci < Ci && co < Co)
-      v = transposed ? w[((long long)ci * Cin + co) * 27 + (26 - tap)] : w[((long long)co * Cin + ci) * 27 + tap];
-    float rem = wscale ? v * wscale[0] : v;
-#pragma unroll
-    for (int t = 0; t < TERMS; ++t) {
-      float back;
-      const unsigned short hb = to16<TERMS>(rem, back);
-      reinterpret_cast<unsigned short*>(out)[((((long long)chunk * TERMS + t) * nstep + s) * 2 + h) * CoutP * 8 +
-                                             (long long)col * 8 + c] = hb;
-      rem -= back;
-    }
-  }
+  const long long total = (long long)nchunk * (zpair ? NSTEP_Z : NSTEP) * 2 * CoutP * 8;
+  for (long long e = (long long)blockIdx.x * 256 + threadIdx.x; e < total; e += (long long)gridDim.x * 256)
+    kmh_pack::bf_elem<TERMS>(e, w, reinterpret_cast<unsigned short*>(out), Cout, Cin, Cin, 0, CoutP, transposed, zpair, wscale);
 }
 
 template <int NT, int TERMS, int MR, bool ZP = false, int ZT = 1>
diff --git a/keymorph_amd/csrc/conv_up2.hip b/keymorph_amd/csrc/conv_up2.hip
--- a/keymorph_amd/csrc/conv_up2.hip
+++ b/keymorph_amd/csrc/conv_up2.hip
@@ -1,5 +1,6 @@
 #include <cstdlib>
 #include "conv_split.h"
+#include "pack_images.h"
 #include "stats_final.h"
 
 namespace {
@@ -14,38 +15,8 @@
                                                              int Cout, int Ctot, int cofs, int Cl, int CoutP, int nchunk,
                                                              const float* __restrict__ wscale) {
   const long long total = (long long)nchunk * UP_NST * 2 * CoutP * 8;
-  for (long long e = (long long)blockIdx.x * 256 + threadIdx.x; e < total; e += (long long)gridDim.x * 256) {
-    const int c = (int)(e & 7);
-    long long r = e >> 3;
-    const int col = (int)(r % CoutP); r /= CoutP;
-    const int h = (int)(r & 1); r >>= 1;
-    const int su = (int)(r % UP_NST);
-    const int chunk = (int)(r / UP_NST);
-    const int ci = chunk * 8 + c, p = su >> 2, st = su & 3;
-    const int par[3] = {p >> 2, (p >> 1) & 1, p & 1}, j[3] = {st >> 1, st & 1, h};
-    int lo[3], hi[3];
-#pragma unroll
-    for (int a = 0; a < 3; ++a) {
-      lo[a] = par[a] == 0 ? (j[a] == 0 ? 0 : 1) : (j[a] == 0 ? 0 : 2);
-      hi[a] = par[a] == 0 ? (j[a] == 0 ? 0 : 2) : (j[a] == 0 ? 1 : 2);
-    }
-    float v = 0.f;
-    if (ci < Cl && col < Cout) {
-      const float* wr = w + ((long long)col * Ctot + cofs + ci) * 27;
-      for (int kz = lo[0]; kz <= hi[0]; ++kz)
-        for (int ky = lo[1]; ky <= hi[1]; ++ky)
-          for (int kx = lo[2]; kx <= hi[2]; ++kx) v += wr[kz * 9 + ky * 3 + kx];
-    }
-    float rem = wscale ? v * wscale[0] : v;
-#pragma unroll
-    for (int t = 0; t < TERMS; ++t) {
-      float back;
-      const unsigned short hb = to16<TERMS>(rem, back);
-      reinterpret_cast<unsigned short*>(out)[((((long long)chunk * TERMS + t) * UP_NST + su) * 2 + h) * CoutP * 8 +
-                                             (long long)col * 8 + c] = hb;
-      rem -= back;
-    }
-  }
+  for (long long e = (long long)blockIdx.x * 256 + threadIdx.x; e < total; e += (long long)gridDim.x * 256)
+    kmh_pack::up_elem<TERMS>(e, w, reinterpret_cast<unsigned short*>(out), Cout, Ctot, cofs, Cl, CoutP, wscale);
 }
 
 template <int TERMS, bool AMP = false>
@@ -194,6 +165,7 @@
 constexpr int DUX = 16, DUY = 4;
 constexpr int DHX = 2 * DUX + 2, DHY = 2 * DUY + 2, DPL = DHX * DHY * 4;
 constexpr int DUP_NST = 32;
+static_assert(UP_NST == kmh_pack::kStepsUp && DUP_NST == kmh_pack::kStepsUp, "pack_images.h packs for these step counts");
 constexpr int DUP_TPB = 256;
 
 template <int TERMS>
@@ -201,39 +173,8 @@
                                                               int Cout, int Ctot, int cofs, int Cl, int CiP, int nchunk,
                                                               const float* __restrict__ wscale) {
   const long long total = (long long)nchunk * DUP_NST * 2 * CiP * 8;
-  for (long long e = (long long)blockIdx.x * 256 + threadIdx.x; e < total; e += (long long)gridDim.x * 256) {
-    const int c = (int)(e & 7);
-    long long r = e >> 3;
-    const int col = (int)(r % CiP); r /= CiP;
-    const int h = (int)(r & 1); r >>= 1;
-    const int s = (int)(r % DUP_NST);
-    const int chunk = (int)(r / DUP_NST);
-    const int co = chunk * 8 + c;
-    const int idx[3] = {s >> 3, (s >> 1) & 3, 2 * (s & 1) + h};
-    int lo[3], hi[3];
-#pragma unroll
-    for (int a = 0; a < 3; ++a) {
-      const int par = (idx[a] + 1) & 1, j = idx[a] <= 1 ? 1 : 0;
-      lo[a] = par == 0 ? (j == 0 ? 0 : 1) : (j == 0 ? 0 : 2);
-      hi[a] = par == 0 ? (j == 0 ? 0 : 2) : (j == 0 ? 1 : 2);
-    }
-    float v = 0.f;
-    if (co < Cout && col < Cl) {
-      const float* wr = w + ((long long)co * Ctot + cofs + col) * 27;
-      for (int kz = lo[0]; kz <= hi[0]; ++kz)
-        for (int ky = lo[1]; ky <= hi[1]; ++ky)
-          for (int kx = lo[2]; kx <= hi[2]; ++kx) v += wr[kz * 9 + ky * 3 + kx];
-    }
-    float rem = wscale ? v * wscale[0] : v;
-#pragma unroll
-    for (int t = 0; t < TERMS; ++t) {
-      float back;
-      const unsigned short hb = to16<TERMS>(rem, back);
-      reinterpret_cast<unsigned short*>(out)[((((long long)chunk * TERMS + t) * DUP_NST + s) * 2 + h) * CiP * 8 +
-                                             (long long)col * 8 + c] = hb;
-      rem -= back;
-    }
-  }
+  for (long long e = (long long)blockIdx.x * 256 + threadIdx.x; e < total; e += (long long)gridDim.x * 256)
+    kmh_pack::upt_elem<TERMS>(e, w, reinterpret_cast<unsigned short*>(out), Cout, Ctot, cofs, Cl, CiP, wscale);
 }
 
 template <int TERMS, bool AMP = false>
diff --git a/keymorph_amd/csrc/firstlayer.hip b/keymorph_amd/csrc/firstlayer.hip
--- a/keymorph_amd/csrc/firstlayer.hip
+++ b/keymorph_amd/csrc/firstlayer.hip
@@ -568,6 +568,29 @@
   b = block_sum<double>(b, red);
   if (threadIdx.x == 0) { ab[0] = a; ab[1] = b; }
 }
+
+__global__ __launch_bounds__(256) void first_layer_fold_batch_kernel(const double* __restrict__ rs ,
+                                                                     const float* __restrict__ w, const float* __restrict__ scale,
+                                                                     const float* __restrict__ shift, int N, int Cout,
+                                                                     float* __restrict__ dw, double* __restrict__ ab ) {
+  __shared__ double red[4];
+  for (int n = 0; n < N; ++n) {
+    const double* rn = rs + (long long)n * Cout * 54;
+    const float sc = scale[n], sh = shift[n];
+    double a = 0, b = 0;
+    for (int e = threadIdx.x; e < Cout * 27; e += 256) {
+      const int co = e / 27, tap = e % 27;
+      const double R = rn[(co * 2 + 0) * 27 + tap], S = rn[(co * 2 + 1) * 27 + tap];
+      const float g = (float)((double)sc * R + (double)sh * S);
+      dw[e] = n ? dw[e] + g : g;
+      a += (double)w[e] * (double)S;
+      b += (double)w[e] * (double)R;
+    }
+    a = block_sum<double>(a, red);
+    b = block_sum<double>(b, red);
+    if (threadIdx.x == 0) { ab[2 * n] = a; ab[2 * n + 1] = b; }
+  }
+}
 }
 
 KMH_API int kmh_conv3d_first_layer_fold(const void* rs, int rs_f64, const float* w, const float* scale_n, const float* shift_n,
@@ -578,3 +601,10 @@
     first_layer_fold_kernel<float><<<1, 256, 0, (hipStream_t)stream>>>((const float*)rs, w, scale_n, shift_n, Cout, dw, ab_n, accumulate);
   return KMH_LAUNCH_CHECK();
 }
+
+KMH_API int kmh_conv3d_first_layer_fold_batch(const double* rs, const float* w, const float* scale, const float* shift, int N,
+                                              int Cout, float* dw, double* ab, void* stream) {
+  if (N < 1 || Cout < 1) return -22;
+  first_layer_fold_batch_kernel<<<1, 256, 0, (hipStream_t)stream>>>(rs, w, scale, shift, N, Cout, dw, ab);
+  return KMH_LAUNCH_CHECK();
+}
diff --git a/keymorph_amd/csrc/pack_images.h b/keymorph_amd/csrc/pack_images.h
--- /dev/null
+++ b/keymorph_amd/csrc/pack_images.h
@@ -0,0 +1,101 @@
+#pragma once
+#include "common.h"
+
+namespace kmh_pack {
+constexpr int kSteps27 = 14;
+constexpr int kSteps36 = 18;
+constexpr int kStepsUp = 32;
+
+template <int TERMS>
+__device__ __forceinline__ void store_terms(float v, const float* __restrict__ wscale, unsigned short* __restrict__ out,
+                                            long long base, long long term_stride) {
+  float rem = wscale ? v * wscale[0] : v;
+#pragma unroll
+  for (int t = 0; t < TERMS; ++t) {
+    float back;
+    const unsigned short hb = to16<TERMS>(rem, back);
+    out[base + t * term_stride] = hb;
+    rem -= back;
+  }
+}
+
+template <int TERMS>
+__device__ __forceinline__ void bf_elem(long long e, const float* __restrict__ w, unsigned short* __restrict__ out, int Cout,
+                                        int Cin, int Ctot, int cofs, int CoutP, int transposed, int zpair,
+                                        const float* __restrict__ wscale) {
+  const int Co = transposed ? Cin : Cout, Ci = transposed ? Cout : Cin;
+  const int nstep = zpair ? kSteps36 : kSteps27;
+  const int c = (int)(e & 7);
+  long long r = e >> 3;
+  const int col = (int)(r % CoutP); r /= CoutP;
+  const int h = (int)(r & 1); r >>= 1;
+  const int s = (int)(r % nstep);
+  const int chunk = (int)(r / nstep);
+  const int ci = chunk * 8 + c;
+  int tap = 2 * s + h, co = col;
+  bool ok = tap < 27;
+  if (zpair) {
+    const int kz = tap / 9 - (col >> 4);
+    co = col & 15;
+    ok = (col < 32) && kz >= 0 && kz <= 2;
+    tap = kz * 9 + tap % 9;
+  }
+  float v = 0.f;
+  if (ok && ci < Ci && co < Co)
+    v = transposed ? w[((long long)ci * Ctot + cofs + co) * 27 + (26 - tap)] : w[((long long)co * Ctot + cofs + ci) * 27 + tap];
+  store_terms<TERMS>(v, wscale, out, ((((long long)chunk * TERMS) * nstep + s) * 2 + h) * CoutP * 8 + (long long)col * 8 + c,
+                     (long long)nstep * 2 * CoutP * 8);
+}
+
+__device__ __forceinline__ void up_taps(int par, int j, int& lo, int& hi) {
+  lo = par == 0 ? (j == 0 ? 0 : 1) : (j == 0 ? 0 : 2);
+  hi = par == 0 ? (j == 0 ? 0 : 2) : (j == 0 ? 1 : 2);
+}
+__device__ __forceinline__ float up_sum(const float* __restrict__ wr, const int lo[3], const int hi[3]) {
+  float v = 0.f;
+  for (int kz = lo[0]; kz <= hi[0]; ++kz)
+    for (int ky = lo[1]; ky <= hi[1]; ++ky)
+      for (int kx = lo[2]; kx <= hi[2]; ++kx) v += wr[kz * 9 + ky * 3 + kx];
+  return v;
+}
+
+template <int TERMS>
+__device__ __forceinline__ void up_elem(long long e, const float* __restrict__ w, unsigned short* __restrict__ out, int Cout,
+                                        int Ctot, int cofs, int Cl, int CoutP, const float* __restrict__ wscale) {
+  const int c = (int)(e & 7);
+  long long r = e >> 3;
+  const int col = (int)(r % CoutP); r /= CoutP;
+  const int h = (int)(r & 1); r >>= 1;
+  const int su = (int)(r % kStepsUp);
+  const int chunk = (int)(r / kStepsUp);
+  const int ci = chunk * 8 + c, p = su >> 2, st = su & 3;
+  const int par[3] = {p >> 2, (p >> 1) & 1, p & 1}, j[3] = {st >> 1, st & 1, h};
+  int lo[3], hi[3];
+#pragma unroll
+  for (int a = 0; a < 3; ++a) up_taps(par[a], j[a], lo[a], hi[a]);
+  float v = 0.f;
+  if (ci < Cl && col < Cout) v = up_sum(w + ((long long)col * Ctot + cofs + ci) * 27, lo, hi);
+  store_terms<TERMS>(v, wscale, out, ((((long long)chunk * TERMS) * kStepsUp + su) * 2 + h) * CoutP * 8 + (long long)col * 8 + c,
+                     (long long)kStepsUp * 2 * CoutP * 8);
+}
+
+template <int TERMS>
+__device__ __forceinline__ void upt_elem(long long e, const float* __restrict__ w, unsigned short* __restrict__ out, int Cout,
+                                         int Ctot, int cofs, int Cl, int CiP, const float* __restrict__ wscale) {
+  const int c = (int)(e & 7);
+  long long r = e >> 3;
+  const int col = (int)(r % CiP); r /= CiP;
+  const int h = (int)(r & 1); r >>= 1;
+  const int s = (int)(r % kStepsUp);
+  const int chunk = (int)(r / kStepsUp);
+  const int co = chunk * 8 + c;
+  const int idx[3] = {s >> 3, (s >> 1) & 3, 2 * (s & 1) + h};
+  int lo[3], hi[3];
+#pragma unroll
+  for (int a = 0; a < 3; ++a) up_taps((idx[a] + 1) & 1, idx[a] <= 1 ? 1 : 0, lo[a], hi[a]);
+  float v = 0.f;
+  if (co < Cout && col < Cl) v = up_sum(w + ((long long)co * Ctot + cofs + col) * 27, lo, hi);
+  store_terms<TERMS>(v, wscale, out, ((((long long)chunk * TERMS) * kStepsUp + s) * 2 + h) * CiP * 8 + (long long)col * 8 + c,
+                     (long long)kStepsUp * 2 * CiP * 8);
+}
+}
diff --git a/keymorph_amd/csrc/weights.hip b/keymorph_amd/csrc/weights.hip
--- /dev/null
+++ b/keymorph_amd/csrc/weights.hip
@@ -0,0 +1,123 @@
+#include "absmax.h"
+#include "conv_split.h"
+#include "pack_images.h"
+
+struct KmhAbsmaxSeg {
+  const float* x;
+  long long n, row_len, row_stride, col_ofs;
+  float min_abs;
+  float mul, inv_mul;
+  int reserved;
+};
+
+struct KmhPackDesc {
+  const float* w;
+  void* out;
+  const float* wscale;
+  int kind;
+  int Cout, C, Ctot, cofs;
+  int pad;
+  int transposed, zpair;
+  int blk0, nblk;
+  long long total;
+};
+static_assert(sizeof(KmhAbsmaxSeg) == 56 && sizeof(KmhPackDesc) == 72, "the tables are written by backbone_ops.py");
+
+namespace {
+constexpr int kSegBlocks = 64;
+
+__global__ __launch_bounds__(256) void absmax_multi_partial_kernel(const KmhAbsmaxSeg* __restrict__ segs,
+                                                                   unsigned* __restrict__ acc ) {
+  const KmhAbsmaxSeg sg = segs[blockIdx.y];
+  const float* x = sg.x + sg.col_ofs;
+  const long long n = sg.n;
+  float m = 0.f;
+  if (sg.row_len >= n || sg.row_stride == sg.row_len) {
+    long long head = (long long)(((16 - (reinterpret_cast<unsigned long long>(x) & 15)) & 15) >> 2);
+    if (head > n) head = n;
+    const float* xb = x + head;
+    const long long nb = n - head, n4 = nb >> 2;
+    for (long long i = (long long)blockIdx.x * 256 + threadIdx.x; i < n4; i += (long long)gridDim.x * 256) {
+      const float4 v = reinterpret_cast<const float4*>(xb)[i];
+      m = fmaxf(fmaxf(m, fmaxf(fabsf(v.x), fabsf(v.y))), fmaxf(fabsf(v.z), fabsf(v.w)));
+    }
+    if (blockIdx.x == 0) {
+      for (long long i = threadIdx.x; i < head; i += 256) m = fmaxf(m, fabsf(x[i]));
+      for (long long i = (n4 << 2) + threadIdx.x; i < nb; i += 256) m = fmaxf(m, fabsf(xb[i]));
+    }
+  } else {
+    for (long long i = (long long)blockIdx.x * 256 + threadIdx.x; i < n; i += (long long)gridDim.x * 256) {
+      const long long r = i / sg.row_len;
+      m = fmaxf(m, fabsf(x[r * sg.row_stride + (i - r * sg.row_len)]));
+    }
+  }
+  kmh_absmax::publish(m, acc + 2 * blockIdx.y);
+}
+
+__global__ void absmax_multi_final_kernel(const KmhAbsmaxSeg* __restrict__ segs, int count, float* __restrict__ out) {
+  const int i = blockIdx.x * blockDim.x + threadIdx.x;
+  if (i >= count) return;
+  float s2[2];
+  range_scale(fmaxf(__uint_as_float(reinterpret_cast<const unsigned*>(out)[2 * i]), segs[i].min_abs), s2);
+  out[2 * i] = s2[0] * segs[i].mul;
+  out[2 * i + 1] = s2[1] * segs[i].inv_mul;
+}
+
+template <int TERMS>
+__global__ __launch_bounds__(256) void pack_multi_kernel(const KmhPackDesc* __restrict__ descs, int count) {
+  int i = 0;
+  while (i + 1 < count && (int)blockIdx.x >= descs[i + 1].blk0) ++i;
+  const KmhPackDesc d = descs[i];
+  unsigned short* out = reinterpret_cast<unsigned short*>(d.out);
+  const long long b = (long long)((int)blockIdx.x - d.blk0);
+  for (long long e = b * 256 + threadIdx.x; e < d.total; e += (long long)d.nblk * 256) {
+    if (d.kind == 0) kmh_pack::bf_elem<TERMS>(e, d.w, out, d.Cout, d.C, d.Ctot, d.cofs, d.pad, d.transposed, d.zpair, d.wscale);
+    else if (d.kind == 1) kmh_pack::up_elem<TERMS>(e, d.w, out, d.Cout, d.Ctot, d.cofs, d.C, d.pad, d.wscale);
+    else kmh_pack::upt_elem<TERMS>(e, d.w, out, d.Cout, d.Ctot, d.cofs, d.C, d.pad, d.wscale);
+  }
+}
+}
+
+KMH_API int kmh_absmax_scale_multi(const void* segs, int count, float* out, void* stream) {
+  if (count < 1 || !segs || !out) return -22;
+  hipStream_t s = (hipStream_t)stream;
+  hipError_t e = hipMemsetAsync(out, 0, (size_t)count * 2 * sizeof(float), s);
+  if (e != hipSuccess) return (int)e;
+  absmax_multi_partial_kernel<<<dim3(kSegBlocks, count), 256, 0, s>>>((const KmhAbsmaxSeg*)segs, reinterpret_cast<unsigned*>(out));
+  absmax_multi_final_kernel<<<ceil_div(count, 64), 64, 0, s>>>((const KmhAbsmaxSeg*)segs, count, out);
+  return KMH_LAUNCH_CHECK();
+}
+
+KMH_API int kmh_conv3d_pack_multi_geometry(int kind, int Cout, int C, int transposed, int* pad, int* zpair, long long* total,
+                                           int* nblk) {
+  long long t;
+  if (kind == 0) {
+    const int Co = transposed ? C : Cout, Ci = transposed ? Cout : C;
+    *zpair = Co <= 16;
+    *pad = cout_pad(Co);
+    t = (long long)((Ci + 7) / 8) * (*zpair ? kmh_pack::kSteps36 : kmh_pack::kSteps27) * 2 * *pad * 8;
+  } else if (kind == 1) {
+    if (C & 7) return -22;
+    *zpair = 0;
+    *pad = cout_pad(Cout);
+    t = (long long)(C / 8) * kmh_pack::kStepsUp * 2 * *pad * 8;
+  } else if (kind == 2) {
+    *zpair = 0;
+    *pad = (C + 127) & ~127;
+    t = (long long)((Cout + 7) / 8) * kmh_pack::kStepsUp * 2 * *pad * 8;
+  } else {
+    return -22;
+  }
+  *total = t;
+  *nblk = ceil_div(t, 256) > 2048 ? 2048 : ceil_div(t, 256);
+  return 0;
+}
+
+KMH_API int kmh_conv3d_pack_multi(const void* descs, int count, int total_blocks, int terms, void* stream) {
+  if (count < 1 || total_blocks < 1 || !descs) return -22;
+  hipStream_t s = (hipStream_t)stream;
+  if (terms == 2) pack_multi_kernel<2><<<total_blocks, 256, 0, s>>>((const KmhPackDesc*)descs, count);
+  else if (terms == 3) pack_multi_kernel<3><<<total_blocks, 256, 0, s>>>((const KmhPackDesc*)descs, count);
+  else return -22;
+  return KMH_LAUNCH_CHECK();
+}
diff --git a/keymorph_amd/parallel.py b/keymorph_amd/parallel.py
--- a/keymorph_amd/parallel.py
+++ b/keymorph_amd/parallel.py
@@ -136,6 +136,7 @@
         check(lib.kmh_adam_step(_p(self.flat.flat), _p(self.flat.gather()), _p(self.m), _p(self.v), self.flat.numel,
                                 self.lr, self.betas[0], self.betas[1], self.eps, self.t, grad_scale, _stream()),
               "kmh_adam_step")
+        torch.autograd.graph.increment_version(self.flat.params)
 
 
 def gather_group_points(local_points: torch.Tensor, num_subjects: int) -> torch.Tensor:
diff --git a/keymorph_amd/unet3d/model.py b/keymorph_amd/unet3d/model.py
--- a/keymorph_amd/unet3d/model.py
+++ b/keymorph_amd/unet3d/model.py
@@ -119,6 +119,7 @@
 
     def features(self, x, head_masks_gradient=False):
         last_pm = True if head_masks_gradient else None
+        self.weight_bank().ensure()
         x = B.to_ndhwc(x)
         feats = []
         L, nd = len(self.encoders), len(self.decoders)
@@ -158,6 +159,20 @@
             x = self._block(dec, skip, x, lazy, last_pm if j == nd - 1 else None)
         return x
 
+    def weight_bank(self):
+        bank = self.__dict__.get("_weight_bank")
+        if bank is None:
+            dec_c1 = {id(d.basic_module.SingleConv1): d.basic_module.SingleConv2.conv.out_channels for d in self.decoders}
+            specs = []
+            for m in self.modules():
+                if isinstance(m, SingleConv) and not (m.conv.in_channels == 1 and m.conv.out_channels <= 16):
+                    cs = dec_c1.get(id(m), 0)
+                    fused = cs and m.conv.out_channels > 16 and m.conv.out_channels % 4 == 0 and cs % 8 == 0 \
+                        and (m.conv.in_channels - cs) % 8 == 0
+                    specs.append((m.conv.weight, cs if fused else 0))
+            bank = self.__dict__["_weight_bank"] = B.WeightBank(specs)
+        return bank
+
     def _block(self, fn, *args, **kwargs):
         if self.use_checkpoint and torch.is_grad_enabled():
             from torch.utils import checkpoint
```

After: 15.58 (median of 6 runs). No clear change (+0.2%).
